# nnnagle/vq-vae

Measured on AMD Instinct MI355X. Metric: tiles/sec, higher is better.
Workload: dtype bf16

## Files before the change

### include/frl_hip.h

```cpp
#ifndef FRL_HIP_H
#define FRL_HIP_H

#include <stddef.h>
#include <stdint.h>

#ifdef __cplusplus
extern "C" {
#endif

typedef void* frl_stream_t;

enum { FRL_F32 = 0, FRL_BF16 = 1, FRL_F16 = 2  };
enum { FRL_ACT_NONE = 0, FRL_ACT_RELU = 1, FRL_ACT_SIGMOID = 2 };

int frl_version(void);
const char* frl_last_error(void);
int frl_device_arch(char* buf, int n);
int frl_kernel_timing_enable(int on);
int frl_kernel_timing_report(char* buf, int n);

size_t frl_pack_cache_table_bytes(void);
int frl_pack_cache_create(void* arena, size_t bytes);
int frl_pack_cache_destroy(int handle);
int frl_pack_cache_activate(int handle);
// ... 132 lines not shown
int frl_tcn_hot_fwd(const void* x, const void* drop_mask, const float* conv_w, const float* conv_b, const float* gn_w, const float* gn_b,
                    const float* gate_w, const float* gate_b, void* y, int64_t npix, int HW, int dilation, float eps, void* ws,
                    size_t ws_bytes, frl_stream_t stream);
int frl_tcn_hot_bwd_nodx_supported(int64_t npix, int HW);
int frl_tcn_hot_bwd(const void* x, const void* drop_mask, const void* dy, const float* conv_w, const float* conv_b, const float* gn_w,
                    const float* gn_b, const float* gate_w, const float* gate_b, void* dx, float* d_conv_w, float* d_conv_b,
                    float* d_gn_w, float* d_gn_b, float* d_gate_w, float* d_gate_b, int64_t npix, int HW, int dilation,
                    float eps, void* ws, size_t ws_bytes, frl_stream_t stream);
size_t frl_tcn_chain_fwd_workspace_bytes(void);
int frl_tcn_chain_static_tiles(int on);
int frl_tcn_chain_fwd(const void* x, const float* const* conv_w, const float* const* conv_b, const float* const* gn_w,
                      const float* const* gn_b, const float* const* gate_w, const float* const* gate_b, const float* head_w,
                      const float* head_b, void* y1, void* y2, void* y3, void* h, int64_t npix, int HW, int Ch, float eps, void* ws,
                      size_t ws_bytes, frl_stream_t stream);
int frl_tcn_chain_fwd_xt(const void* x, const float* const* conv_w, const float* const* conv_b, const float* const* gn_w,
                         const float* const* gn_b, const float* const* gate_w, const float* const* gate_b, const float* head_w,
                         const float* head_b, void* y1, void* y2, void* y3, void* h, void* xt, int64_t npix, int HW, int Ch, float eps,
                         void* ws, size_t ws_bytes, frl_stream_t stream);
int frl_tcn_hot_bwd_head_supported(int64_t npix, int HW, int Ch);
size_t frl_tcn_hot_bwd_head_workspace_bytes(int64_t npix);
int frl_tcn_hot_bwd_head(const void* x, const void* dh, const float* head_w, int Ch, const float* conv_w, const float* conv_b,
                         const float* gn_w, const float* gn_b, const float* gate_w, const float* gate_b, void* dx, float* d_conv_w,
                         float* d_conv_b, float* d_gn_w, float* d_gn_b, float* d_gate_w, float* d_gate_b, int64_t npix, int HW,
                         int dilation, float eps, void* ws, size_t ws_bytes, frl_stream_t stream);
int frl_tcn_hot_force_generic_tiles(int on);
int frl_tcn_hot_bwd4_share(int variant, int share);

size_t frl_adamw_workspace_bytes(void);
int frl_adamw_clip_step(const void* desc_host, int ntensors, const void* chunks, const int* chunk_tensor, int nchunks, float max_norm,
                        float lr, double beta1, double beta2, float eps, int step, float* norm_out, const float* ok, int* counters,
                        const float* lr_dev, int* tensor_steps, int nsteps, void* ws, size_t ws_bytes, frl_stream_t stream);
int frl_multi_tensor_scale_copy(const void* desc_host, int ntensors, const void* chunks, const int* chunk_tensor, int nchunks, float scale,
                                frl_stream_t stream);

int frl_film_modulate_fwd(const void* h, const void* gamma, const void* beta, void* out, int64_t B, int T, int64_t HW,
                          int C, int dtype, frl_stream_t stream);
int frl_film_modulate_bwd(const void* dout, const void* h, const void* gamma, void* dh, void* dgamma, void* dbeta,
                          int64_t B, int T, int64_t HW, int C, int dtype, frl_stream_t stream);
int frl_mean_time_fwd(const void* tile, void* out, int64_t B, int T, int64_t HWC, int dtype, frl_stream_t stream);
int frl_add(const void* a, const void* b, float scale_b, void* out, int64_t n, int dtype, frl_stream_t stream);

typedef struct FrlNormRec {
  float sub, div, mul, add, lo, hi;
  int flags;
  int pad;
} FrlNormRec;
int frl_normalize_tiles(const void* raw, int raw_dtype, const uint8_t* valid, const void* table, void* out, int out_dtype,
                        uint8_t* mask_out, int64_t rows, int F, frl_stream_t stream);
int frl_normalize_chunk_tiles(const void* chunk, int raw_dtype, int T, int CY, int CX, int F, const int32_t* desc, int ntiles,
                              int tile, const void* table, void* out, int out_dtype, uint8_t* mask_out, frl_stream_t stream);

int frl_host_parallel_copy(void* dst, const void* src, size_t nbytes, int nthreads);

size_t frl_mse_workspace_bytes(void);
int frl_mse_fwd(const void* pred, const void* target, const uint8_t* mask, int64_t P, int C, float* out, int dtype,
                void* ws, size_t ws_bytes, frl_stream_t stream);
int frl_mse_bwd(const void* pred, const void* target, const uint8_t* mask, const float* gscale, const float* stats,
                int64_t P, int C, void* dpred, int dtype, frl_stream_t stream);

int frl_decoder_mse_fused_supported(int Cz, int hidden, int F, int dtype);
size_t frl_decoder_mse_workspace_bytes(int64_t P, int Cz);
int frl_decoder_mse_fwd(const void* z, const float* w1, const float* b1, const float* w2, const float* b2, const void* target,
                        const uint8_t* mask, void* xhat, float* out, int64_t P, int Cz, void* ws, size_t ws_bytes,
                        frl_stream_t stream);
int frl_decoder_mse_bwd(const void* z, const float* w1, const float* b1, const float* w2, const float* b2, const void* target,
                        const uint8_t* mask, const float* gscale, const float* stats, void* dz, float* dw1, float* db1,
                        float* dw2, float* db2, int64_t P, int Cz, void* ws, size_t ws_bytes, frl_stream_t stream);
size_t frl_decoder_mse_onepass_bytes(int64_t P, int Cz);
int frl_decoder_mse_fwd_bwd(const void* z, const float* w1, const float* b1, const float* w2, const float* b2, const void* target,
                            const uint8_t* mask, const float* gscale, float* out, void* dz, void* buf, size_t buf_bytes, void* ctl,
                            int* nslab, int64_t P, int Cz, frl_stream_t stream);
int frl_decoder_mse_reduce(const void* buf, int nslab, float* dw1, float* db1, float* dw2, float* db2, int Cz, frl_stream_t stream);
int frl_decoder_mse_bwd_subgroups(int on);

size_t frl_vq_workspace_bytes(int64_t N, int K, int d);
int frl_vq_assign_fwd(const void* z, const float* E, int64_t N, int K, int d, int32_t* idx_out, void* zq_out,
                      float* stats_out, int32_t* counts_out, int dtype, void* ws, size_t ws_bytes, frl_stream_t stream);
size_t frl_vq_prepared_bytes(int K, int d);
int frl_vq_stream_tiles(int nt);
int frl_vq_prepare(const float* E, int64_t N, int K, int d, int dtype, void* prep, size_t prep_bytes, frl_stream_t stream);
int frl_vq_assign_fwd_prepared(const void* z, const float* E, void* prep , int64_t N, int K, int d,
                               int32_t* idx_out, void* zq_out, float* stats_out, int32_t* counts_out, int dtype, void* ws,
                               size_t ws_bytes, frl_stream_t stream);
int frl_vq_bwd(const void* g_out, const void* z, const void* zq , const float* E, const int32_t* idx, const int32_t* counts,
               const float* gscale, float beta, int64_t N, int K, int d, void* g_z_out, float* g_E_out, float* sums_out,
               int dtype, void* ws, size_t ws_bytes, frl_stream_t stream);
int frl_vq_ema_update(const float* sums, const int32_t* counts, int K, int d, float decay, float eps, float* ema_count,
                      float* ema_sum, float* E, const float* ok, frl_stream_t stream);
int frl_vq_revive_dead_codes(float* E, const int64_t* window_counts, int64_t min_count, const void* z, int64_t N, int K, int d,
                             uint64_t seed, float* m, float* v, int32_t* revived, int dtype, frl_stream_t stream);

int frl_gather_locations_fwd(const void* feat, int64_t sC, int64_t sH, int64_t sW, int C, int H, int W, const int64_t* coords, int64_t N,
                             void* out, int dtype, frl_stream_t stream);
int frl_segment_sum_rows(const float* vals, const int64_t* order, const int64_t* keys_sorted, int64_t M, int D, float* out, int64_t out_stride,
                         int accumulate, frl_stream_t stream);
int frl_infonce_fwd(const float* emb, int D, const int64_t* pairs, const float* weights, const unsigned char* is_pos, int64_t T,
                    const int64_t* seg, int64_t nseg, float temperature, int similarity, float* sims, float* logits, float* loss_a, float* coef,
                    float* loss, frl_stream_t stream);
int frl_infonce_pair_grads(const float* emb, int D, const int64_t* pairs, const float* sims, const float* coef, const float* gscale, int64_t T,
                           int64_t nseg, float temperature, int similarity, float* ga, float* gb, frl_stream_t stream);

size_t frl_vicreg_workspace_bytes(int64_t N, int D);
int frl_vicreg_fwd(const void* x, int64_t N, int D, int dtype, float variance_weight, float covariance_weight, float variance_target,
                   float eps, float* losses, float* cov, float* centre, void* ws, size_t ws_bytes, frl_stream_t stream);
int frl_vicreg_bwd(const void* x, const float* cov, const float* centre, const float* g3, int64_t N, int D, int dtype, float variance_weight,
                   float covariance_weight, float variance_target, float eps, void* dx, frl_stream_t stream);

int frl_soft_nbr_fwd(const float* d_ref, const float* d_learned, const unsigned char* mask, const float* weights, int64_t B, int M,
                     float inv_tau_ref, float inv_tau_learned, int min_valid, float* pairstat, float* coef, float* out2, double* stats,
                     frl_stream_t stream);
int frl_soft_nbr_bwd(const float* coef, const float* pairstat, const float* weights, const float* out2, const float* gup, int64_t B, int M,
                     float* grad, frl_stream_t stream);
int frl_soft_nbr_gathered_fwd(const float* ref, int C, const void* emb, int D, int emb_dtype, const int64_t* ref_rows_a, const int64_t* ref_rows_b,
                              const int64_t* emb_rows_a, const int64_t* emb_rows_b, const int64_t* lengths, const float* weights, int64_t B, int M,
                              int exclude_diagonal, float inv_tau_ref, float inv_tau_learned, int min_valid, float* pairstat, float* out2,
                              double* stats, frl_stream_t stream);
int frl_soft_nbr_gathered_bwd(const float* ref, int C, const void* emb, int D, int emb_dtype, const int64_t* ref_rows_a, const int64_t* ref_rows_b,
                              const int64_t* emb_rows_a, const int64_t* emb_rows_b, const int64_t* lengths, const float* weights, int64_t B, int M,
                              int exclude_diagonal, float inv_tau_ref, float inv_tau_learned, int min_valid, const float* pairstat,
                              const float* out2, const float* gup, float* grad_rows, frl_stream_t stream);

int frl_evt_soft_nbr_fwd(const void* emb, int emb_dtype, int64_t N, int D, const int32_t* idx, const float* S, const float* w, int K,
                         const int32_t* seg, const int32_t* seg_host, int nseg, float inv_tau_ref, float inv_tau_learned, int min_valid_anchors,
                         float* rowstat, float* segout, double* segstat, int32_t* index_flag, frl_stream_t stream);
int frl_evt_soft_nbr_bwd(const void* emb, int emb_dtype, int64_t N, int D, const int32_t* idx, const float* S, const float* w, int K,
                         const int32_t* seg, const int32_t* seg_host, int nseg, float inv_tau_ref, float inv_tau_learned, const float* rowstat,
                         const float* segout, const float* gup, const float* seg_weights, void* grad, frl_stream_t stream);

int frl_recovery_disc_fwd(const void* z, int dtype, const float* ysfc, int64_t N, int T, int D, float margin, float low_ysfc_max,
                          float high_ysfc_min, float* partial, float* out2, double* stats, frl_stream_t stream);
int frl_recovery_disc_bwd(const void* z, int dtype, const float* ysfc, int64_t N, int T, int D, float margin, float low_ysfc_max,
                          float high_ysfc_min, const float* out2, const float* gup, void* grad, frl_stream_t stream);
int frl_spread_rank_fwd(const float* d_i, const float* d_j, const unsigned char* mask, const float* ref_diff, int64_t B, int M, float margin,
                        float delta, float* pairstat, float* out2, double* stats, frl_stream_t stream);
int frl_spread_rank_bwd(const unsigned char* mask, const float* pairstat, const float* ref_diff, const float* gup, int64_t B, int M,
                        float margin, float delta, float* grad_i, float* grad_j, frl_stream_t stream);
int frl_spread_rank_gathered_fwd(const void* emb, int D, int emb_dtype, const int64_t* rows_i, const int64_t* rows_j, const int64_t* lengths,
                                 const float* ref_diff, int64_t B, int M, float margin, float delta, float* pairstat, float* out2,
                                 double* stats, frl_stream_t stream);
int frl_spread_rank_gathered_bwd(const void* emb, int D, int emb_dtype, const int64_t* rows_i, const int64_t* rows_j, const int64_t* lengths,
                                 const float* ref_diff, int64_t B, int M, float margin, float delta, const float* pairstat, const float* gup,
                                 float* grad_rows, frl_stream_t stream);

int frl_decode_codes(const int32_t* idx, const void* table, void* out, int64_t P, int K, int F, int dtype, int32_t* index_flag,
                     frl_stream_t stream);

size_t frl_mutual_knn_max_points(int D);
int frl_mutual_knn(const float* feat, int N, int D, const int32_t* patch_id, const float* coords, float pos_min_spatial, int k,
                   int32_t* knn_idx, uint8_t* mutual, frl_stream_t stream);

size_t frl_phase_pairs_max_points(int D);
int frl_phase_pairs(const float* spec, const float* ysfc, int N, int D, int T, const int32_t* seg_host, const int32_t* seg, int S, int k,
                    int min_overlap, int min_pairs, float sigma, uint64_t* masks, int32_t* knn_idx, int32_t* overlap, uint8_t* keep,
                    uint8_t* keep_overlap, float* weight, float* dist, uint8_t* anchor_ok, int32_t* counters, int32_t* flag,
                    frl_stream_t stream);

int frl_spatial_pairs_max_hw(void);
int frl_spatial_pack_mask(const uint8_t* mask, int S, int H, int W, uint32_t* bits, frl_stream_t stream);
int frl_spatial_knn(const uint32_t* bits, int S, int H, int W, const int32_t* anchors, int N, const int32_t* seg_host, const int32_t* seg,
                    const int32_t* offsets, int k, int32_t* pos_rc, uint8_t* pos_valid, int32_t* counters, int32_t* flag, frl_stream_t stream);
int frl_spatial_negatives(const uint32_t* bits, int S, int H, int W, const int32_t* anchors, int N, const int32_t* seg_host, const int32_t* seg,
                          int lo, int hi, int n_per_anchor, const int32_t* draws, int32_t* neg_rc, int32_t* neg_count, int32_t* counters,
                          int32_t* flag, frl_stream_t stream);
int frl_spatial_pair_index(int S, int H, int W, const int32_t* anchors, int N, const int32_t* seg_host, const int32_t* seg, const int32_t* pos_rc,
                           const uint8_t* pos_valid, int k, const int32_t* neg_rc, const int32_t* neg_count, int n_per_anchor, const float* feat,
                           int C, float tau, float min_w, uint32_t* bitmap, int32_t* wordpre, int32_t* unique_seg, int32_t* unique_rc,
                           int32_t* anchor_idx, int32_t* pos_idx, int32_t* neg_idx, float* pos_w, float* pos_d, float* neg_w, float* neg_d,
                           frl_stream_t stream);

// ... 68 lines not shown
```

### vq-vae_amd/csrc/frl_epi.hpp

```cpp
#pragma once
#include <stdint.h>
#include <hip/hip_runtime.h>

struct ThEpi {
  float *dWc, *dWg, *dbc, *dbg, *dgam, *dbet;
  __device__ void operator()(int64_t i, float s) const {
    if (i < 3 * 4096) {
      const int k = (int)(i / 4096), co = (int)((i % 4096) / 64), ci = (int)(i % 64);
      dWc[(co * 64 + ci) * 3 + k] = s;
    } else if (i < 4 * 4096) {
      dWg[i - 3 * 4096] = s;
    } else {
      const int j = (int)(i - 4 * 4096);
      if (j < 64) dbc[j] = s; else if (j < 128) dbg[j - 64] = s; else if (j < 192) dgam[j - 128] = s; else dbet[j - 192] = s;
    }
  }
};

struct C3Epi {
  int OCT, Cin9, oc_base, Cout; float* dW; float* dB;
  __device__ void operator()(int64_t i, float s) const {
    if (i < (int64_t)OCT * Cin9) {
      const int Cin = Cin9 / 9;
      const int tap = (int)(i / ((int64_t)OCT * Cin)), rem = (int)(i % ((int64_t)OCT * Cin));
      const int ocl = rem / Cin, ic = rem % Cin;
      if (oc_base + ocl < Cout) dW[(int64_t)(oc_base + ocl) * Cin9 + ic * 9 + tap] = s;
    } else if (dB != nullptr) {
      const int ocl = (int)(i - (int64_t)OCT * Cin9);
      if (oc_base + ocl < Cout) dB[oc_base + ocl] = s;
    }
  }
};

struct DecEpi {
  float *dW2, *dW1, *db2, *db1; int Cz, CZP, F, Hd;
  __device__ void operator()(int64_t i, float s) const {
    if (i < F * Hd) { dW2[i] = s; return; }
    i -= F * Hd;
    if (i < Hd * CZP) { const int hh = (int)(i / CZP), c = (int)(i % CZP); if (c < Cz) dW1[hh * Cz + c] = s; return; }
    i -= Hd * CZP;
    if (i < F) db2[i] = s; else db1[i - F] = s;
  }
};

struct EncEpi {
  float *dw2, *dw1, *db2, *dg2, *db1, *dg1;
  __device__ void operator()(int64_t i, float s) const {
    if (i < 64 * 128) { dw2[i] = s; return; }
    i -= 64 * 128;
    if (i < 128 * 64) { dw1[i] = s; return; }
    i -= 128 * 64;
    if (i < 64) db2[i] = s;
    else if (i < 128) dg2[i - 64] = s;
    else if (i < 256) db1[i - 128] = s;
    else dg1[i - 256] = s;
  }
};

struct FilmEpi {
  float *dw1g, *dw1b, *dw2g, *dw2b, *db1g, *db1b, *db2g, *db2b;
  __device__ void operator()(int64_t i, float s) const {
    if (i < 2048) { dw1g[i] = s; return; }
    if (i < 4096) { dw1b[i - 2048] = s; return; }
    if (i < 4480) { dw2g[i - 4096] = s; return; }
    if (i < 4864) { dw2b[i - 4480] = s; return; }
    if (i < 4896) { db1g[i - 4864] = s; return; }
    if (i < 4928) { db1b[i - 4896] = s; return; }
    if (i < 4940) { db2g[i - 4928] = s; return; }
    db2b[i - 4940] = s;
  }
};

struct ShEpi {
  float *dwb, *dwa, *dbb, *dba; int NB, NA, HID;
  __device__ void operator()(int64_t i, float s) const {
    if (i < NB * HID) { dwb[i] = s; return; }
    i -= NB * HID;
    if (i < NA * HID) { dwa[i] = s; return; }
    i -= NA * HID;
    if (i < NB) dbb[i] = s; else dba[i - NB] = s;
  }
};

struct WgradEpi {
  float* dW; int64_t dso, dsi; float* dB; int Cout, Cin, accumulate_bias;
  __device__ void operator()(int64_t i, float s) const {
    if (i < (int64_t)Cout * Cin) {
      const int oc = (int)(i / Cin), ic = (int)(i % Cin);
      dW[oc * dso + ic * dsi] = s;
    } else if (dB != nullptr) {
      const int oc = (int)(i - (int64_t)Cout * Cin);
      if (accumulate_bias) dB[oc] += s; else dB[oc] = s;
    }
  }
};

struct CodeEpi {
  const float* E; const int32_t* counts; const float* gscale; float ce_base; int d, bf; float* gE; float* sums_out;
  __device__ void operator()(int64_t i, float s) const {
    if (sums_out) sums_out[i] = s;
    if (gE) {
      const float ce = ce_base * (gscale ? gscale[1] : 1.f);
      const float ev = bf ? (float)(__bf16)E[i] : E[i];
      gE[i] = ce * ((float)counts[i / d] * ev - s);
    }
  }
};

struct CopyEpi {
  float* dst;
  __device__ void operator()(int64_t i, float s) const { dst[i] = s; }
};

template <class Epi> struct FrlEpiKind { static constexpr int id = 0; };
template <> struct FrlEpiKind<ThEpi> { static constexpr int id = 1; };
template <> struct FrlEpiKind<C3Epi> { static constexpr int id = 2; };
template <> struct FrlEpiKind<DecEpi> { static constexpr int id = 3; };
template <> struct FrlEpiKind<EncEpi> { static constexpr int id = 4; };
template <> struct FrlEpiKind<FilmEpi> { static constexpr int id = 5; };
template <> struct FrlEpiKind<ShEpi> { static constexpr int id = 6; };
template <> struct FrlEpiKind<WgradEpi> { static constexpr int id = 7; };
template <> struct FrlEpiKind<CodeEpi> { static constexpr int id = 8; };
```

### vq-vae_amd/csrc/frl_pack.hpp

```cpp
#pragma once
#include <hip/hip_runtime.h>
#include <stdint.h>
#include <stddef.h>

enum { FRL_PACK_PW = 0, FRL_PACK_C3 = 1, FRL_PACK_PW_REP = 2, FRL_PACK_PW_K4 = 3 };

struct FrlPackJob {
  const float* W;
  char* dst;
  long long so, si;
  int kind, dtype, NF;
  int Cout, Cin, MB;
  int tap_rev, nfrag;
};

static inline FrlPackJob frl_pack_job_pw(const float* W, size_t dst_off, int dtype, int NF, int Cout, int Cin, int MB, long long so, long long si) {
  FrlPackJob j;
  j.W = W; j.dst = (char*)dst_off; j.so = so; j.si = si; j.kind = FRL_PACK_PW; j.dtype = dtype; j.NF = NF;
  j.Cout = Cout; j.Cin = Cin; j.MB = MB; j.tap_rev = 0; j.nfrag = MB * NF * 64;
  return j;
}
static inline FrlPackJob frl_pack_job_c3(const float* W, size_t dst_off, int dtype, int NF, int Cout, int Cin, long long so, long long si, int tap_rev,
                                         int nfrag) {
  FrlPackJob j;
  j.W = W; j.dst = (char*)dst_off; j.so = so; j.si = si; j.kind = FRL_PACK_C3; j.dtype = dtype; j.NF = NF;
  j.Cout = Cout; j.Cin = Cin; j.MB = (Cout + 15) >> 4; j.tap_rev = tap_rev; j.nfrag = nfrag;
  return j;
}

void* frl_pack_cached(const FrlPackJob* jobs, int njobs, size_t bytes, bool* hit);
```

### vq-vae_amd/csrc/pack_cache.hip

```cpp
#include "frl_common.hpp"
#include "frl_host.hpp"
#include "frl_pack.hpp"
#include <map>
#include <mutex>
#include <string.h>
#include <vector>

#define PK_FRAGS_PER_BLOCK 512

__device__ __forceinline__ void pk_frag_pw(const FrlPackJob& j, int i) {
  const int lane = i & 63, fs = i >> 6;
  const int s = fs % j.NF, mb = fs / j.NF;
  const int r = lane & 15, kc = lane >> 4;
  const int qo = 4 * j.MB;
  const int oc = j.kind == FRL_PACK_PW_REP ? 4 * mb + (r & 3) : qo * (r >> 2) + 4 * mb + (r & 3);
  if (j.dtype == FRL_BF16) {
    const int q = j.NF * 8;
    bf16x8 v;
#pragma unroll
    for (int e = 0; e < 8; ++e) {
      const int ic = j.kind == FRL_PACK_PW_K4 ? (e < 4 ? 4 * kc + e : j.Cin) : q * kc + 8 * s + e;
      v[e] = (oc < j.Cout && ic < j.Cin) ? (bf16)j.W[oc * j.so + ic * j.si] : (bf16)0.f;
    }
    reinterpret_cast<bf16x8*>(j.dst)[i] = v;
  } else {
    const int q = j.NF;
    const int ic = q * kc + s;
    reinterpret_cast<float*>(j.dst)[i] = (oc < j.Cout && ic < j.Cin) ? j.W[oc * j.so + ic * j.si] : 0.f;
  }
}

__device__ __forceinline__ void pk_frag_c3(const FrlPackJob& j, int g) {
  const int FE = j.dtype == FRL_BF16 ? 8 : 1;
  const int q = j.NF * FE, CK = 4 * q;
  const int MB = (j.Cout + 15) >> 4, qo = 4 * MB;
  const int nck = (j.Cin + CK - 1) / CK;
  const int per_block = 9 * 4 * j.NF * 64;
  const int blk = g / per_block, i = g % per_block;
  const int oc0 = (blk / nck) * 4, ck = (blk % nck) * CK;
  const int ln = i & 63, fs = i >> 6;
  const int s = fs % j.NF, m = (fs / j.NF) & 3, tap = fs / (j.NF * 4);
  const int r = ln & 15, kq = ln >> 4;
  const int oc = qo * (r >> 2) + 4 * (oc0 + m) + (r & 3);
  const int tsrc = j.tap_rev ? 8 - tap : tap;
  const bool mok = (oc0 + m) < MB;
  if (j.dtype == FRL_BF16) {
    bf16x8 v;
#pragma unroll
    for (int e = 0; e < 8; ++e) {
      const int ic = ck + q * kq + 8 * s + e;
      v[e] = (mok && oc < j.Cout && ic < j.Cin) ? (bf16)j.W[oc * j.so + ic * j.si + tsrc] : (bf16)0.f;
    }
    reinterpret_cast<bf16x8*>(j.dst)[g] = v;
  } else {
    const int ic = ck + q * kq + s;
    reinterpret_cast<float*>(j.dst)[g] = (mok && oc < j.Cout && ic < j.Cin) ? j.W[oc * j.so + ic * j.si + tsrc] : 0.f;
  }
}

__global__ __launch_bounds__(256) void frl_pack_jobs_kernel(const FrlPackJob* __restrict__ jobs, const int2* __restrict__ blocks) {
  const int2 bk = blocks[blockIdx.x];
  const FrlPackJob j = jobs[bk.x];
  const int end = (bk.y + PK_FRAGS_PER_BLOCK) < j.nfrag ? (bk.y + PK_FRAGS_PER_BLOCK) : j.nfrag;
  for (int i = bk.y + threadIdx.x; i < end; i += 256) {
    if (j.kind == FRL_PACK_C3) pk_frag_c3(j, i); else pk_frag_pw(j, i);
  }
}

namespace {
struct Key {
  unsigned char bytes[8 * 72];
  size_t n;
  bool operator<(const Key& o) const { return n != o.n ? n < o.n : memcmp(bytes, o.bytes, n) < 0; }
};
struct Cache {
  char* arena = nullptr;
  size_t bytes = 0, used = 0, table_bytes = 0;
  std::map<Key, char*> images;
  std::vector<FrlPackJob> jobs;
  std::vector<int2> blocks;
  bool dirty = false;
};
std::mutex g_mu;
std::map<int, Cache> g_caches;
int g_next = 1;
int g_active = 0;
constexpr size_t PK_MAX_JOBS = 2048, PK_MAX_BLOCKS = 16384;
}

void* frl_pack_cached(const FrlPackJob* jobs, int njobs, size_t bytes, bool* hit) {
  *hit = false;
  if (g_active == 0 || njobs <= 0 || njobs > 8) return nullptr;
  std::lock_guard<std::mutex> lk(g_mu);
  auto it = g_caches.find(g_active);
  if (it == g_caches.end()) return nullptr;
  Cache& c = it->second;
  Key k;
  memset(&k, 0, sizeof(k));
  k.n = (size_t)njobs * sizeof(FrlPackJob);
  memcpy(k.bytes, jobs, k.n);
  auto im = c.images.find(k);
  if (im != c.images.end()) { *hit = true; return im->second; }
  const size_t need = (bytes + 255) / 256 * 256;
  int nblk = 0;
  for (int i = 0; i < njobs; ++i) nblk += (jobs[i].nfrag + PK_FRAGS_PER_BLOCK - 1) / PK_FRAGS_PER_BLOCK;
  if (c.used + need > c.bytes || c.jobs.size() + njobs > PK_MAX_JOBS || c.blocks.size() + nblk > PK_MAX_BLOCKS) return nullptr;
  char* img = c.arena + c.used;
  c.used += need;
  for (int i = 0; i < njobs; ++i) {
    FrlPackJob j = jobs[i];
    j.dst = img + (size_t)j.dst;
    const int ji = (int)c.jobs.size();
    c.jobs.push_back(j);
    for (int f = 0; f < j.nfrag; f += PK_FRAGS_PER_BLOCK) c.blocks.push_back(int2{ji, f});
  }
  c.images[k] = img;
  c.dirty = true;
  return img;
}

extern "C" {

size_t frl_pack_cache_table_bytes(void) { return PK_MAX_JOBS * sizeof(FrlPackJob) + PK_MAX_BLOCKS * sizeof(int2); }

int frl_pack_cache_create(void* arena, size_t bytes) {
  const size_t tb = (frl_pack_cache_table_bytes() + 255) / 256 * 256;
  if (arena == nullptr || bytes <= tb + 4096) return frl_fail(-4, "pack_cache_create: arena too small");
  std::lock_guard<std::mutex> lk(g_mu);
  Cache c;
  c.arena = (char*)arena;
  c.bytes = bytes;
  c.table_bytes = tb;
  c.used = tb;
  const int h = g_next++;
  g_caches[h] = c;
  return h;
}

int frl_pack_cache_destroy(int handle) {
  std::lock_guard<std::mutex> lk(g_mu);
  if (g_active == handle) g_active = 0;
  g_caches.erase(handle);
  return 0;
}

int frl_pack_cache_activate(int handle) {
  std::lock_guard<std::mutex> lk(g_mu);
  const int was = g_active;
  g_active = (handle != 0 && g_caches.count(handle)) ? handle : 0;
  return was;
}

int frl_pack_cache_images(int handle) {
  std::lock_guard<std::mutex> lk(g_mu);
  auto it = g_caches.find(handle);
  return it == g_caches.end() ? -1 : (int)it->second.images.size();
}

int frl_pack_cache_refresh(int handle, hipStream_t stream) {
  std::lock_guard<std::mutex> lk(g_mu);
  auto it = g_caches.find(handle);
  if (it == g_caches.end()) return frl_fail(-2, "pack_cache_refresh: unknown handle");
  Cache& c = it->second;
  if (c.jobs.empty()) return 0;
  FrlPackJob* jd = (FrlPackJob*)c.arena;
  int2* bd = (int2*)(c.arena + PK_MAX_JOBS * sizeof(FrlPackJob));
  if (c.dirty) {
    hipStreamCaptureStatus cs = hipStreamCaptureStatusNone;
    (void)hipStreamIsCapturing(stream, &cs);
    if (cs != hipStreamCaptureStatusNone) return frl_fail(-5, "pack_cache_refresh: images were registered during a stream capture (run the step eagerly first)");
    FRL_HIP(hipMemcpyAsync(jd, c.jobs.data(), c.jobs.size() * sizeof(FrlPackJob), hipMemcpyHostToDevice, stream));
    FRL_HIP(hipMemcpyAsync(bd, c.blocks.data(), c.blocks.size() * sizeof(int2), hipMemcpyHostToDevice, stream));
    FRL_HIP(hipStreamSynchronize(stream));
    c.dirty = false;
  }
  FRL_LAUNCH(frl_pack_jobs_kernel, dim3((unsigned)c.blocks.size()), dim3(256), 0, stream, (const FrlPackJob*)jd, (const int2*)bd);
  return frl_check_launch("pack_cache_refresh");
}

}
```

### vq-vae_amd/csrc/vq.hip

```cpp
#include "frl_common.hpp"
#include "frl_host.hpp"
#include "vq_common.hpp"
#include "vq_prepare.hpp"
#include "vq_assign_chunked.hpp"
#include "vq_assign_resident.hpp"
#include "vq_assign_stream.hpp"
#include "vq_bwd.hpp"
#include <stdlib.h>

static int vq_chunk(int K, int d_pad, size_t esize) {
  const size_t cap = 64 * 1024;
  int kc = VQ_MAX_CHUNK;
  while (kc > 16 && (size_t)kc * d_pad * esize > cap) kc >>= 1;
  const int kpad = (K + 15) / 16 * 16;
  if (kc > kpad) kc = kpad;
  return kc;
}
static int vq_waves(int64_t N, int d) { return (d <= 64 && N >= (int64_t)256 * 8 * 2 * 16) ? 8 : 4; }
static int vq_grid(int64_t N, int d) {
  const int nw = vq_waves(N, d), NT = nw == 8 ? 2 : 4;
  const int64_t nb = (N + nw * NT * 16 - 1) / (nw * NT * 16);
  const int cap = 512;
  return (int)(nb < cap ? (nb < 1 ? 1 : nb) : cap);
}
#define VQ_FIX_WAVES 1024
#define VQ_BWD_WGS 256

struct VqPrep { size_t ctl, en, pack, total; int Kc, kpad, npk; };
template <typename T, int NF>
static VqPrep vq_prep_layout(int64_t N, int K, int d) {
  VqPrep P;
  const int d_pad = NF * DT<T>::FE * 4;
  P.Kc = vq_chunk(K, d_pad, sizeof(T));
  P.kpad = (K + P.Kc - 1) / P.Kc * P.Kc;
  P.npk = (P.kpad / 16) * NF * 64;
  P.ctl = 0;
  P.en = (sizeof(VqCtl) + (size_t)K * 4 + 255) / 256 * 256;
  P.pack = P.en + ((size_t)P.kpad * 4 + 255) / 256 * 256;
  P.total = P.pack + (size_t)P.npk * sizeof(typename DT<T>::frag_t);
  return P;
}
static size_t vq_prep_bytes_max(int K) {
  return (sizeof(VqCtl) + (size_t)K * 4 + 255) / 256 * 256 + ((size_t)(K + VQ_MAX_CHUNK) * 4 + 255) / 256 * 256 +
         (size_t)((K + 15) / 16 + 64) * 16 * 128 * 4;
}

struct VqLayout { size_t hdr, counts_fix, partial, amb, amb_lim, prep, total; int grid; };
static VqLayout vq_layout(int64_t N, int K, int d) {
  VqLayout L;
  L.grid = vq_grid(N, d);
  size_t o = 0;
  L.hdr = o; o += 256;
  L.counts_fix = o; o += ((size_t)K * 4 + 255) / 256 * 256;
  L.partial = o; o += ((size_t)L.grid * 16 * 4 + 255) / 256 * 256;
  L.amb = o; o += ((size_t)N * 4 + 255) / 256 * 256;
  L.amb_lim = o; o += ((size_t)N * 4 + 255) / 256 * 256;
  L.prep = o; o += vq_prep_bytes_max(K);
  L.total = o;
  return L;
}

template <typename T, int NF>
static int launch_vq_prepare(const float* E, int64_t N, int K, int d, char* prep, hipStream_t st) {
  typedef typename DT<T>::frag_t frag_t;
  const VqPrep P = vq_prep_layout<T, NF>(N, K, d);
  const int npack_blocks = (P.npk + 255) / 256;
  const int kz = P.kpad > 64 ? P.kpad : 64;
  FRL_LAUNCH((vq_prepare_kernel<T, NF>), dim3(npack_blocks + (kz + 255) / 256), dim3(256), 0, st, E, K, d, (float*)(prep + P.en), P.kpad,
             (frag_t*)(prep + P.pack), P.npk, npack_blocks, (int*)(prep + P.ctl));
  return frl_check_launch("vq_prepare");
}

static int g_vq_stream_tiles = -1;
static int vq_stream_tiles();
#ifndef VQ_STREAM_DEFAULT
#define VQ_STREAM_DEFAULT 2
#endif
static int vq_stream_tiles() {
  if (g_vq_stream_tiles >= 0) return g_vq_stream_tiles;
  static const int env = [] { const char* e = getenv("FRL_VQ_STREAM"); return e ? atoi(e) : VQ_STREAM_DEFAULT; }();
  return env;
}
#ifndef VQ_RES_NT
#define VQ_RES_NT 4
#endif
template <typename... P, typename... A>
static int vq_launch_assign(void (*kern)(P...), int grid, int threads, size_t lds, hipStream_t st, A... args) {
  if (lds > 64 * 1024) FRL_HIP(hipFuncSetAttribute((const void*)kern, hipFuncAttributeMaxDynamicSharedMemorySize, (int)lds));
  FRL_LAUNCH_AS("vq_assign_kernel", kern, dim3(grid), dim3(threads), lds, st, args...);
  return 0;
}
template <typename T, int NF>
static int launch_vq(const void* z, const float* E, char* prep, int64_t N, int K, int d, int32_t* idx, void* zq, float* stats,
                     int32_t* counts, char* ws, hipStream_t st) {
  typedef typename DT<T>::frag_t frag_t;
  const VqLayout L = vq_layout(N, K, d);
  const VqPrep P = vq_prep_layout<T, NF>(N, K, d);
  const int nw = vq_waves(N, d);
  const int Kc = P.Kc;
  VqHeader* hdr = (VqHeader*)(ws + L.hdr);
  const bool resident = P.kpad == Kc;
  if (!resident) FRL_HIP(hipMemsetAsync(ws, 0, L.partial, st));
  if (prep == nullptr) {
    const int rc = launch_vq_prepare<T, NF>(E, N, K, d, ws + L.prep, st);
    if (rc) return rc;
    prep = ws + L.prep;
  }
  const float* en = (const float*)(prep + P.en);
  const frag_t* pk = (const frag_t*)(prep + P.pack);
  if constexpr (sizeof(T) == 2 && NF == 2) {
    const int stream_nt = vq_stream_tiles();
    int nt = stream_nt >= 4 ? 4 : (stream_nt >= 2 ? 2 : 1);
    while (nt > 1 && N % (VQS_NW * nt * 16) != 0) nt >>= 1;
    const int batch = VQS_NW * nt * 16;
    if (resident && stream_nt > 0 && d == 64 && (Kc & 15) == 0 && N % batch == 0 && N < ((int64_t)1 << 32)) {
      const int64_t nb = (N + batch - 1) / batch;
      const int grid_s = (int)(nb < 256 ? nb : 256);
      const size_t lds = (size_t)(Kc / 16) * NF * 64 * sizeof(frag_t) + (size_t)Kc * 4 + (size_t)((K + 3) & ~3) * 4 + 64 * 4 +
                         (size_t)VQ_FAST_ROWS * 16 + (size_t)VQS_NW * VQS_CAP * 8 + (size_t)VQS_CAND * 4 +
                         (size_t)VQS_NW * (VQS_CAP + 16) * VQS_ZP * sizeof(T);
      if (lds > 160 * 1024) return frl_fail(-3, "vq_assign: LDS budget exceeded");
      const auto kern = nt == 4 ? vq_assign_stream_kernel<4> : nt == 2 ? vq_assign_stream_kernel<2> : vq_assign_stream_kernel<1>;
      const int rc = vq_launch_assign(kern, grid_s, 64 * VQS_NW, lds, st, (const bf16*)z, en, N, K, Kc, idx, (bf16*)zq, (float*)(ws + L.partial),
                                      (const bf16x8*)pk, (VqCtl*)(prep + P.ctl), counts, stats, (unsigned*)(ws + L.amb), (float*)(ws + L.amb_lim));
      return rc ? rc : frl_check_launch("vq_assign");
    }
  }
  if (resident) {
    const int nwr = (nw == 8 && NF <= (sizeof(T) == 2 ? 2 : 4)) ? 8 : 4;
    const int batch = nwr * VQ_RES_NT * 16;
    const int64_t nb = (N + batch - 1) / batch;
    const int grid_r = (int)(nb < L.grid ? nb : L.grid);
    size_t lds = (size_t)(Kc / 16) * NF * 64 * sizeof(frag_t) + (size_t)Kc * 4 + (size_t)((K + 1) & ~1) * 4 + (size_t)VQ_FAST_ROWS * 12 +
                 (size_t)2 * batch * 4 + (size_t)nwr * 64 * 4 + 32 * 4 + (size_t)VQ_PZ_CAP * d * sizeof(T);
    const size_t fold = (size_t)2 * nwr * 64 * sizeof(double);
    if (lds < fold) lds = fold;
    if (lds > 160 * 1024) return frl_fail(-3, "vq_assign: LDS budget exceeded");
    auto kern = vq_assign_resident_kernel<T, NF, VQ_RES_NT, 4>;
    if constexpr (NF <= (sizeof(T) == 2 ? 2 : 4)) {
      if (nwr == 8) kern = vq_assign_resident_kernel<T, NF, VQ_RES_NT, 8>;
    }
    const int rc = vq_launch_assign(kern, grid_r, 64 * nwr, lds, st, (const T*)z, E, en, N, K, d, Kc, idx, (T*)zq, (float*)(ws + L.partial), pk,
                                    (VqCtl*)(prep + P.ctl), counts, stats);
    return rc ? rc : frl_check_launch("vq_assign");
  }
  const int Kc2 = Kc >= 32 ? Kc / 2 : Kc;
  const size_t lds = 2 * ((size_t)(Kc2 / 16) * NF * 64 * sizeof(frag_t) + (size_t)Kc2 * 4) + 64 + (K <= 2048 ? (size_t)K * 4 : 0);
  if (((Kc2 / 16) * NF * 64 * sizeof(frag_t)) % 1024 != 0 || (Kc2 & 63) != 0) return frl_fail(-3, "vq_assign: chunk is not a whole number of DMA pieces");
  const auto kern = nw == 8 ? vq_assign_kernel<T, NF, 2, 8> : vq_assign_kernel<T, NF, 4, 4>;
  const int rc = vq_launch_assign(kern, L.grid, 64 * nw, lds, st, (const T*)z, E, en, N, K, d, Kc2, idx, (T*)zq, (float*)(ws + L.partial),
                                  (int32_t*)(ws + L.counts_fix), hdr, (int32_t*)(ws + L.amb), (float*)(ws + L.amb_lim), pk);
  if (rc) return rc;
  FRL_LAUNCH_AS("vq_fixup_tile_kernel", (vq_fixup_tile_kernel<T, NF>), dim3(1024), dim3(64 * VQ_FIXT_WAVES), 0, st, (const T*)z, E, en, pk, K, P.kpad, d,
                (const int32_t*)(ws + L.amb), (const float*)(ws + L.amb_lim), hdr, idx, (T*)zq, (int32_t*)(ws + L.counts_fix));
  FRL_LAUNCH(vq_finalize_kernel, dim3(1), dim3(256), 0, st, (const float*)(ws + L.partial), L.grid * nw, (const VqHeader*)hdr,
             (const int32_t*)(ws + L.counts_fix), counts, K, N, d, stats);
  return frl_check_launch("vq_assign");
}

static int vq_bwd_chunk(int K, int d) {
  int kc = K;
  while ((size_t)kc * d * 4 > 96 * 1024 && kc > 1) kc = (kc + 1) / 2;
  return kc;
}

extern "C" {

int frl_vq_stream_tiles(int nt) {
  const int prev = g_vq_stream_tiles;
  g_vq_stream_tiles = nt < 0 ? -1 : nt;
  return prev;
}

size_t frl_vq_workspace_bytes(int64_t N, int K, int d) {
  const VqLayout L = vq_layout(N, K, d);
  const size_t bwd = (size_t)VQ_BWD_WGS * K * d * 4 + (size_t)K * d * 4;
  return L.total > bwd ? L.total : bwd;
}

#define VQ_DISPATCH(dtype, d, CALL)                                              \
  do {                                                                          \
    if ((dtype) == FRL_F32) {                                                   \
      if ((d) <= 16) return CALL(float, 4);                                     \
      if ((d) <= 32) return CALL(float, 8);                                     \
      if ((d) <= 64) return CALL(float, 16);                                    \
      return CALL(float, 32);                                                   \
    } else if ((dtype) == FRL_BF16) {                                           \
      if ((d) <= 32) return CALL(bf16, 1);                                      \
      if ((d) <= 64) return CALL(bf16, 2);                                      \
      return CALL(bf16, 4);                                                     \
    }                                                                           \
    return frl_fail(-2, "vq: bad dtype");                                       \
  } while (0)

size_t frl_vq_prepared_bytes(int K, int d) { return (K > 0 && d > 0 && d <= 128) ? vq_prep_bytes_max(K) : 0; }

int frl_vq_prepare(const float* E, int64_t N, int K, int d, int dtype, void* prep, size_t prep_bytes, hipStream_t stream) {
  if (N <= 0 || K <= 0 || d <= 0) return frl_fail(-2, "vq_prepare: empty input");
  if (d > 128) return frl_fail(-2, "vq_prepare: d > 128 unsupported");
  if (prep == nullptr || prep_bytes < frl_vq_prepared_bytes(K, d)) return frl_fail(-4, "vq_prepare: buffer too small");
#define VQ_CALL_PREP(T_, NF_) launch_vq_prepare<T_, NF_>(E, N, K, d, (char*)prep, stream)
  VQ_DISPATCH(dtype, d, VQ_CALL_PREP);
#undef VQ_CALL_PREP
}

int frl_vq_assign_fwd_prepared(const void* z, const float* E, void* prep, int64_t N, int K, int d, int32_t* idx_out, void* zq_out,
                               float* stats_out, int32_t* counts_out, int dtype, void* ws, size_t ws_bytes, hipStream_t stream) {
  if (N <= 0 || K <= 0 || d <= 0) return frl_fail(-2, "vq_assign: empty input");
  if (d > 128) return frl_fail(-2, "vq_assign: d > 128 unsupported");
  if (ws_bytes < frl_vq_workspace_bytes(N, K, d)) return frl_fail(-4, "vq_assign: workspace too small");
#define VQ_CALL_FWD(T_, NF_) launch_vq<T_, NF_>(z, E, (char*)prep, N, K, d, idx_out, zq_out, stats_out, counts_out, (char*)ws, stream)
  VQ_DISPATCH(dtype, d, VQ_CALL_FWD);
#undef VQ_CALL_FWD
}

int frl_vq_assign_fwd(const void* z, const float* E, int64_t N, int K, int d, int32_t* idx_out, void* zq_out,
                      float* stats_out, int32_t* counts_out, int dtype, void* ws, size_t ws_bytes, hipStream_t stream) {
  return frl_vq_assign_fwd_prepared(z, E, nullptr, N, K, d, idx_out, zq_out, stats_out, counts_out, dtype, ws, ws_bytes, stream);
}

int frl_vq_bwd(const void* g_out, const void* z, const void* zq, const float* E, const int32_t* idx, const int32_t* counts,
               const float* gscale, float beta, int64_t N, int K, int d, void* g_z_out, float* g_E_out,
               float* sums_out, int dtype, void* ws, size_t ws_bytes, hipStream_t stream) {
  if (N <= 0 || K <= 0 || d <= 0) return frl_fail(-2, "vq_bwd: empty input");
  if (dtype != FRL_F32 && dtype != FRL_BF16) return frl_fail(-2, "vq_bwd: bad dtype");
  if (dtype == FRL_BF16 && d > 128) return frl_fail(-2, "vq_bwd: d > 128 unsupported in bf16");
  if (ws_bytes < frl_vq_workspace_bytes(N, K, d)) return frl_fail(-4, "vq_bwd: workspace too small");
  const int Kc = vq_bwd_chunk(K, d);
  const size_t lds = (size_t)Kc * d * 4;
  if (dtype == FRL_F32 && lds > 96 * 1024) return frl_fail(-2, "vq_bwd: one code row exceeds the LDS chunk");
  const int64_t rows = (N + VQ_BWD_WGS - 1) / VQ_BWD_WGS;
  const float cz = beta * 2.f / ((float)N * (float)d), ce = 2.f / ((float)N * (float)d);
  float* slab = (float*)ws;
  if (dtype == FRL_F32) {
    auto kern = vq_bwd_kernel<float>;
    if (lds > 64 * 1024) FRL_HIP(hipFuncSetAttribute((const void*)kern, hipFuncAttributeMaxDynamicSharedMemorySize, (int)lds));
    FRL_LAUNCH_AS("vq_bwd_kernel", kern, dim3(VQ_BWD_WGS), dim3(256), lds, stream, (const float*)g_out, (const float*)z, E, idx, gscale,
                       cz, N, K, d, Kc, rows, (float*)g_z_out, slab);
    launch_slab_reduce_deferrable<float, CodeEpi>((const float*)slab, VQ_BWD_WGS, (int64_t)K * d, CodeEpi{E, counts, gscale, ce, d, 0, g_E_out, sums_out}, stream, sums_out == nullptr);
  } else if (dtype == FRL_BF16) {
    const int64_t rows64 = (rows + 63) / 64 * 64;
    if (d <= 32) {
      FRL_LAUNCH((vq_bwd_mfma_kernel<4, 2, 8>), dim3(VQ_BWD_WGS), dim3(512), (size_t)64 * 40 * 2 + 256, stream, (const bf16*)g_out, (const bf16*)z, (const bf16*)zq, E, idx,
                 gscale, cz, N, K, d, rows64, (bf16*)g_z_out, slab);
    } else if (d <= 64) {
      FRL_LAUNCH((vq_bwd_mfma_kernel<4, 4, 8>), dim3(VQ_BWD_WGS), dim3(512), (size_t)64 * 72 * 2 + 256, stream, (const bf16*)g_out, (const bf16*)z, (const bf16*)zq, E, idx,
                 gscale, cz, N, K, d, rows64, (bf16*)g_z_out, slab);
    } else {
      FRL_LAUNCH((vq_bwd_mfma_kernel<2, 8, 8>), dim3(VQ_BWD_WGS), dim3(512), (size_t)64 * 136 * 2 + 256, stream, (const bf16*)g_out, (const bf16*)z, (const bf16*)zq, E, idx,
                 gscale, cz, N, K, d, rows64, (bf16*)g_z_out, slab);
    }
    launch_slab_reduce_deferrable<float, CodeEpi>((const float*)slab, VQ_BWD_WGS, (int64_t)K * d, CodeEpi{E, counts, gscale, ce, d, 1, g_E_out, sums_out}, stream, sums_out == nullptr);
  } else return frl_fail(-2, "vq_bwd: bad dtype");
  return frl_check_launch("vq_bwd");
}

int frl_vq_ema_update(const float* sums, const int32_t* counts, int K, int d, float decay, float eps, float* ema_count,
                      float* ema_sum, float* E, const float* ok, hipStream_t stream) {
  FRL_LAUNCH(vq_ema_kernel, dim3(1), dim3(256), 0, stream, sums, counts, K, d, decay, eps, ema_count, ema_sum, E, ok);
  return frl_check_launch("vq_ema_update");
}

int frl_vq_revive_dead_codes(float* E, const int64_t* window_counts, int64_t min_count, const void* z, int64_t N, int K, int d,
                             uint64_t seed, float* m, float* v, int32_t* revived, int dtype, hipStream_t stream) {
  if (K <= 0 || d <= 0) return frl_fail(-2, "vq_revive_dead_codes: bad codebook shape");
  if (N <= 0) return frl_fail(-2, "vq_revive_dead_codes: no candidate rows");
  if (dtype == FRL_F32)
    FRL_LAUNCH((vq_revive_kernel<float>), dim3(K), dim3(64), 0, stream, E, (const long long*)window_counts, (long long)min_count,
               (const float*)z, (long long)N, K, d, (unsigned long long)seed, m, v, revived);
  else if (dtype == FRL_BF16)
    FRL_LAUNCH((vq_revive_kernel<bf16>), dim3(K), dim3(64), 0, stream, E, (const long long*)window_counts, (long long)min_count,
               (const bf16*)z, (long long)N, K, d, (unsigned long long)seed, m, v, revived);
  else return frl_fail(-2, "vq_revive_dead_codes: dtype must be FRL_F32 or FRL_BF16");
  return frl_check_launch("vq_revive_dead_codes");
}

}
```

### vq-vae_amd/csrc/vq_assign_chunked.hpp

```cpp
#pragma once
#include "vq_common.hpp"

template <typename T, int NF, int NT, int NW>
__global__ __launch_bounds__(NW * 64, (NW == 8 ? 4 : 2)) void vq_assign_kernel(
    const T* __restrict__ Z, const float* __restrict__ E, const float* __restrict__ en_g, int64_t N, int K, int d, int Kc,
    int32_t* __restrict__ idx_out, T* __restrict__ zq_out, float* __restrict__ partial , int32_t* __restrict__ counts_acc,
    VqHeader* __restrict__ hdr_w, int32_t* __restrict__ amb_list, float* __restrict__ amb_lim, const typename DT<T>::frag_t* __restrict__ pk) {
  typedef typename DT<T>::frag_t frag_t;
  constexpr int FE = DT<T>::FE;
  constexpr int q = NF * FE;
  extern __shared__ __attribute__((aligned(16))) char smem[];
  const int chunk_bytes = (Kc / 16) * NF * 64 * (int)sizeof(frag_t);
  const int buf_bytes = chunk_bytes + Kc * 4;
  float* cbw = reinterpret_cast<float*>(smem + 2 * buf_bytes);
  int* hist = reinterpret_cast<int*>(smem + 2 * buf_bytes + 64);
  const bool lds_hist = K <= 2048;
  const int tid = threadIdx.x, lane = tid & 63;
  const int wave = __builtin_amdgcn_readfirstlane(tid >> 6);
  const int vx = lane & 15, kc = lane >> 4;
  const int nchunks = (K + Kc - 1) / Kc;
  const bool fast = (d == 4 * q);
  float enmax;
  {
    float m = 0.f;
// ... 150 lines not shown
          } else {
#pragma unroll
            for (int s = 0; s < NF * FE; ++s) {
              if (q * kc + s < d) {
                const float ev = to_f32(from_f32<T>(er[s]));
                zo[s] = from_f32<T>(ev);
                const float df = lq_get<T, NF>(zt[t], s / FE, s % FE) - ev;
                sq_acc = fmaf(df, df, sq_acc);
              }
            }
          }
          if (kc == 0) atomicAdd(lds_hist ? &hist[code] : &counts_acc[code], 1);
        }
      }
    }
  }
  const float ws_ = wave_sum(sq_acc);
  if (lane == 0) partial[blockIdx.x * NW + wave] = ws_;
  if (lds_hist) {
    __syncthreads();
    vq_flush_hist<NW>(hist, counts_acc, K, tid);
  }
}

#define VQ_FIXT_WAVES 8
template <typename T, int NF>
__global__ __launch_bounds__(64 * VQ_FIXT_WAVES) void vq_fixup_tile_kernel(const T* __restrict__ Z, const float* __restrict__ E, const float* __restrict__ en_g,
                                                            const typename DT<T>::frag_t* __restrict__ pk, int K, int kpad, int d,
                                                            const int32_t* __restrict__ amb_list, const float* __restrict__ amb_lim,
                                                            VqHeader* __restrict__ hdr, int32_t* __restrict__ idx_out, T* __restrict__ zq_out,
                                                            int32_t* __restrict__ counts_fix) {
  constexpr int FE = DT<T>::FE;
  constexpr int q = NF * FE;
  __shared__ double mrg_d[VQ_FIXT_WAVES][16];
  __shared__ int mrg_k[VQ_FIXT_WAVES][16];
  __shared__ unsigned long long bins[VQ_SQ_BINS];
  __shared__ float row_sq[16];
  if (threadIdx.x < VQ_SQ_BINS) bins[threadIdx.x] = 0ull;
  const int lane = threadIdx.x & 63, wave = threadIdx.x >> 6;
  const int vx = lane & 15, kc = lane >> 4;
  const bool fast = (d == 4 * q);
  const int namb = hdr->namb;
  const int ntile = (namb + 15) >> 4, nmb = kpad >> 4;
  const int mb0 = (wave * nmb) / VQ_FIXT_WAVES, mb1 = ((wave + 1) * nmb) / VQ_FIXT_WAVES;
  for (int tile = blockIdx.x; tile < ntile; tile += gridDim.x) {
    const int li = tile * 16 + vx;
    const bool valid = li < namb;
    const int64_t row = amb_list[valid ? li : tile * 16];
    const float lm = amb_lim[valid ? li : tile * 16];
    LQTile<T, NF> zr;
    lq_load<T, NF>(zr, Z, row, d, kc, fast);
    const VqBest own = vq_resolve_inlane<T, NF>(zr, pk, en_g, mb0, mb1, K, lane, valid, lm, [&](int p0, int p1, double& d0, double& d1) {
      vq_exact_pair<T, 1>(Z, E, row, p0, p1, d, d0, d1);
    });
    double bestd = own.d;
    int bk = own.k;
    if (kc == 0) { mrg_d[wave][vx] = bestd; mrg_k[wave][vx] = bk; }
    __syncthreads();
    if (wave == 0) {
      bestd = mrg_d[0][vx]; bk = mrg_k[0][vx];
#pragma unroll
      for (int w = 1; w < VQ_FIXT_WAVES; ++w) {
        const double ob = mrg_d[w][vx];
        const int okk = mrg_k[w][vx];
        if (ob < bestd || (ob == bestd && okk < bk)) { bestd = ob; bk = okk; }
      }
      if ((unsigned)bk >= (unsigned)K) bk = 0;
      float rs = 0.f;
      if (valid) vq_write_row<T, NF>(zr, E, zq_out, row, bk, d, kc, rs);
      rs += __shfl_xor(rs, 16, 64);
      rs += __shfl_xor(rs, 32, 64);
      if (valid && kc == 0) { idx_out[row] = bk; atomicAdd(&counts_fix[bk], 1); }
      if (kc == 0) row_sq[vx] = valid ? rs : -1.f;
    }
    __syncthreads();
    if (wave == 1 && lane < 16 && !(row_sq[lane] == -1.f)) vq_sq_bins_add(bins, &hdr->sq_fix, row_sq[lane]);
  }
  __syncthreads();
  if (threadIdx.x < VQ_SQ_BINS && bins[threadIdx.x] != 0ull) atomicAdd(&hdr->sq_bins[threadIdx.x], bins[threadIdx.x]);
}

__global__ __launch_bounds__(256) void vq_finalize_kernel(const float* __restrict__ partial, int npartial, const VqHeader* __restrict__ hdr,
                                                          const int32_t* __restrict__ counts_acc, int32_t* __restrict__ counts, int K, int64_t N,
                                                          int d, float* __restrict__ stats) {
  __shared__ double red[256];
  double s = 0.0;
  for (int i = threadIdx.x; i < npartial; i += 256) s += (double)partial[i];
  red[threadIdx.x] = s;
  __syncthreads();
  for (int o = 128; o > 0; o >>= 1) { if (threadIdx.x < o) red[threadIdx.x] += red[threadIdx.x + o]; __syncthreads(); }
  const double sq = red[0] + (vq_sq_bins_value(hdr->sq_bins) + hdr->sq_fix);
  __syncthreads();
  double h = 0.0;
  for (int k = threadIdx.x; k < K; k += 256) {
    const int cnt = counts_acc[k];
    counts[k] = cnt;
    const double p = (double)cnt / (double)N;
    h += p * log(p + 1e-10);
  }
  red[threadIdx.x] = h;
  __syncthreads();
  for (int o = 128; o > 0; o >>= 1) { if (threadIdx.x < o) red[threadIdx.x] += red[threadIdx.x + o]; __syncthreads(); }
  if (threadIdx.x == 0) {
    stats[0] = (float)sq;
    stats[1] = (float)exp(-red[0]);
    stats[2] = (float)hdr->namb;
    stats[3] = (float)(sq / ((double)N * (double)d));
  }
}
```

### vq-vae_amd/csrc/vq_assign_resident.hpp

```cpp
#pragma once
#include "vq_common.hpp"

#define VQ_PZ_CAP 16

template <typename T, int NF, int NT, int NW>
__global__ __launch_bounds__(NW * 64, (NW == 8 ? 4 : 1)) void vq_assign_resident_kernel(
    const T* __restrict__ Z, const float* __restrict__ E, const float* __restrict__ en_g, int64_t N, int K, int d, int Kc,
    int32_t* __restrict__ idx_out, T* __restrict__ zq_out, float* __restrict__ partial ,
    const typename DT<T>::frag_t* __restrict__ pk, VqCtl* __restrict__ ctl, int32_t* __restrict__ counts_out, float* __restrict__ stats_out) {
  typedef typename DT<T>::frag_t frag_t;
  constexpr int FE = DT<T>::FE;
  constexpr int q = NF * FE;
  constexpr int BATCH = NW * NT * 16;
  constexpr int CAND_CAP = NW * 64;
  extern __shared__ __attribute__((aligned(16))) char smem[];
  frag_t* wl = reinterpret_cast<frag_t*>(smem);
  float* enl = reinterpret_cast<float*>(smem + (size_t)(Kc / 16) * NF * 64 * sizeof(frag_t));
  int* hist = reinterpret_cast<int*>(enl + Kc);
  unsigned long long* best = reinterpret_cast<unsigned long long*>(hist + ((K + 1) & ~1));
  int* bestk = reinterpret_cast<int*>(best + VQ_FAST_ROWS);
  int* park = bestk + VQ_FAST_ROWS;
  int* cand = park + 2 * BATCH;
  int* misc = cand + CAND_CAP;
  T* park_z = reinterpret_cast<T*>(misc + 32);
  int32_t* counts_acc = reinterpret_cast<int32_t*>(ctl + 1);
  const int tid = threadIdx.x, lane = tid & 63, wave = tid >> 6;
  const int vx = lane & 15, kc = lane >> 4;
  const bool fast = (d == 4 * q);
  const int nmb = Kc / 16;
#ifdef VQ_STAMPS
  __shared__ unsigned long long vq_ts[16][8];
  if (tid < 128) (&vq_ts[0][0])[tid] = 0ull;
  unsigned long long t_prev = __builtin_amdgcn_s_memtime();
  const unsigned long long t_begin = t_prev;
  const unsigned long long w_begin = wall_clock64();
#endif

  const int64_t nbatch = (N + BATCH - 1) / BATCH;
  LQTile<T, NF> zt[NT];
  auto load_batch = [&](int64_t b, int tid_) {
    const int64_t r0 = b * BATCH + (int64_t)(tid_ >> 6) * (NT * 16);
#pragma unroll
    for (int t = 0; t < NT; ++t) {
      int64_t row = r0 + t * 16 + (tid_ & 15);
      if (row >= N) row = N - 1;
      lq_load<T, NF>(zt[t], Z, row, d, (tid_ >> 4) & 3, fast);
    }
  };
  if ((int64_t)blockIdx.x < nbatch) load_batch(blockIdx.x, tid);
  copy_frags_lds<T>(wl, pk, nmb * NF * 64, tid, NW * 64);
  float enmax;
  {
    float m = 0.f;
    for (int i = tid; i < Kc; i += NW * 64) {
      const float v = i < K ? en_g[i] : 3.0e38f;
      enl[i] = v;
      if (i < K) m = fmaxf(m, v);
    }
#pragma unroll
    for (int off = 1; off < 64; off <<= 1) m = fmaxf(m, __shfl_xor(m, off, 64));
    if (lane == 0) misc[18 + wave] = __float_as_int(m);
  }
  for (int k = tid; k < K; k += NW * 64) hist[k] = 0;
  if (tid < VQ_FAST_ROWS) { best[tid] = ~0ull; bestk[tid] = 0x7fffffff; }
  if (tid == 0) misc[16] = 0;
  __syncthreads();
  {
    float m = 0.f;
#pragma unroll
    for (int w = 0; w < NW; ++w) m = fmaxf(m, __int_as_float(misc[18 + w]));
    enmax = m;
  }
  const float err_rel = (float)(4 * q + 8) * 1.1920929e-7f;
  const float thr_rel = (3.0517578125e-5f + 2.f * err_rel) * 1.001953125f;
  const float enroot = sqrtf(enmax);
  float sq_acc = 0.f;
  int n_resolved = 0;
  VQ_ST(2);

  for (int64_t batch = blockIdx.x; batch < nbatch; batch += gridDim.x) {
    const int64_t base = batch * BATCH;
    const int64_t v0 = base + (int64_t)wave * (NT * 16);
    if (batch != (int64_t)blockIdx.x) {
      int tidl = tid;
      asm volatile("" : "+v"(tidl));
      load_batch(batch, tidl);
    }
    float thr[NT];
    unsigned g1[NT], g2[NT];
    int gc[NT];
#pragma unroll
    for (int t = 0; t < NT; ++t) {
// ... 202 lines not shown
        }
        VQ_LDS_BARRIER();
        if (c < ncand && bits == best[li]) __hip_atomic_fetch_min(&bestk[li], code, __ATOMIC_RELAXED, __HIP_MEMORY_SCOPE_WORKGROUP);
        VQ_LDS_BARRIER();
        const int j = tidr & 15;
        for (int li2 = tidr >> 4; li2 < n; li2 += NW * 4) {
          int bk = bestk[li2];
          if ((unsigned)bk >= (unsigned)K) bk = 0;
          const int64_t row = base + park[2 * li2];
          for (int ch = j; ch < d; ch += 16) {
            float ev, zv;
            bool done_ = false;
            if constexpr (FE == 8) {
              if (zlds) {
                ev = -0.5f * (float)reinterpret_cast<const bf16x8*>(wl)[((bk >> 4) * NF + ((ch % q) >> 3)) * 64 + (bk & 15) + 16 * (ch / q)][ch & 7];
                zv = (float)reinterpret_cast<const bf16*>(park_z)[li2 * d + ch];
                done_ = true;
              }
            }
            if (!done_) {
              ev = to_f32(from_f32<T>(E[(int64_t)bk * d + ch]));
              zv = to_f32(Z[row * (int64_t)d + ch]);
            }
            zq_out[row * (int64_t)d + ch] = from_f32<T>(ev);
            const float df = zv - ev;
            sq_acc = fmaf(df, df, sq_acc);
          }
          if (j == 0) { idx_out[row] = bk; atomicAdd(&hist[bk], 1); }
        }
        VQ_LDS_BARRIER();
        if (tidr < VQ_FAST_ROWS && tidr < n) {
          int m1 = -1;
          asm volatile("" : "+v"(m1));
          best[tidr] = ((unsigned long long)(unsigned)m1 << 32) | (unsigned)m1;
          bestk[tidr] = 0x7fffffff;
        }
      }
    }
    if (!all_waves) {
      for (int t0 = wave * 16; t0 < n; t0 += NW * 16) {
        const int li = t0 + vx;
        const bool valid = li < n;
        const int64_t row = base + park[2 * (valid ? li : t0)];
        const float lm = __int_as_float(park[2 * (valid ? li : t0) + 1]);
        LQTile<T, NF> zr;
        lq_load<T, NF>(zr, Z, row, d, kc, fast);
        int bk = vq_resolve_inlane<T, NF>(zr, wl, enl, 0, nmb, K, lane, valid, lm, [&](int p0, int p1, double& d0, double& d1) {
          vq_exact_pair<T, 1>(Z, E, row, p0, p1, d, d0, d1);
        }).k;
        if ((unsigned)bk >= (unsigned)K) bk = 0;
        if (valid) {
          vq_write_row<T, NF>(zr, E, zq_out, row, bk, d, kc, sq_acc);
          if (kc == 0) { idx_out[row] = bk; atomicAdd(&hist[bk], 1); }
        }
      }
    }
    n_resolved += n;
    VQ_LDS_BARRIER();
    if (tid == 0) misc[16] = 0;
    VQ_ST(5);
  }
  int tidt = tid;
  asm volatile("" : "+v"(tidt));
  const float ws_ = wave_sum(sq_acc);
  if ((tidt & 63) == 0) partial[blockIdx.x * NW + (tidt >> 6)] = ws_;
  __syncthreads();
  vq_flush_hist<NW>(hist, counts_acc, K, tidt);
  if (tidt == 0 && n_resolved) atomicAdd(&ctl->namb, n_resolved);
  asm volatile("s_waitcnt vmcnt(0)" ::: "memory");
  __syncthreads();
  if (tidt == 0) {
    __builtin_amdgcn_fence(__ATOMIC_RELEASE, "agent");
    asm volatile("s_waitcnt vmcnt(0)" ::: "memory");
    const int ticket = __hip_atomic_fetch_add(&ctl->done, 1, __ATOMIC_RELAXED, __HIP_MEMORY_SCOPE_AGENT);
    misc[17] = (ticket == (int)gridDim.x - 1) ? 1 : 0;
    if (ticket == (int)gridDim.x - 1) {
      __builtin_amdgcn_fence(__ATOMIC_ACQUIRE, "agent");
      asm volatile("s_waitcnt vmcnt(0)" ::: "memory");
    }
  }
  __syncthreads();
  const bool last = misc[17] != 0;
  __syncthreads();
  if (last) vq_fold_stats<NW>(reinterpret_cast<double*>(smem), tidt, tidt & 63, tidt >> 6, partial, (int)gridDim.x * NW, ctl, K, N, d, counts_out, stats_out);
#ifdef VQ_STAMPS
  VQ_ST(6);
  __syncthreads();
  if (tid < 128) vq_dbg[(size_t)blockIdx.x * 128 + tid] = (&vq_ts[0][0])[tid];
  if (tid == 0) { vq_dbg[(size_t)gridDim.x * 128 + 2 * blockIdx.x] = __builtin_amdgcn_s_memtime() - t_begin; vq_dbg[(size_t)gridDim.x * 128 + 2 * blockIdx.x + 1] = wall_clock64() - w_begin; }
#endif
}
```

### vq-vae_amd/csrc/vq_assign_stream.hpp

```cpp
#pragma once
#include "vq_common.hpp"

#define VQS_NW 16
#define VQS_ZP 72
#define VQS_GRP 16

template <int NT, bool FULL>
__device__ __forceinline__ void vqs_score_group(const bf16x8* __restrict__ wl, const float* __restrict__ enl, int lane, int kc, int mb0, int cnt,
                                                const LQTile<bf16, 2> (&z)[NT], unsigned (&c1)[NT], unsigned (&c2)[NT]) {
  const unsigned maskv = ~VQ_IDX_MASK;
  const bf16x8* __restrict__ wb = wl + mb0 * 2 * 64 + lane;
  const float* __restrict__ eb = enl + mb0 * 16 + 4 * kc;
  auto block = [&](int mb, int j) {
    (void)mb;
    const f32x4 en4 = *reinterpret_cast<const f32x4*>(eb + j * 16);
    const bf16x8 a0 = wb[j * 2 * 64], a1 = wb[j * 2 * 64 + 64];
#pragma unroll
    for (int t = 0; t < NT; ++t) {
      f32x4 acc = mfma16(a0, z[t].f[0], en4);
      acc = mfma16(a1, z[t].f[1], acc);
#pragma unroll
      for (int r = 0; r < 4; r += 2) {
        const unsigned k0 = (__float_as_uint(acc[r]) & maskv) | (unsigned)(4 * j + r);
        const unsigned k1 = (__float_as_uint(acc[r + 1]) & maskv) | (unsigned)(4 * j + r + 1);
        unsigned m;
        asm("v_med3_f32 %0, %1, %2, %3" : "=v"(m) : "v"(c1[t]), "v"(k0), "v"(k1));
        asm("v_min_f32 %0, %1, %2" : "=v"(c2[t]) : "v"(c2[t]), "v"(m));
        asm("v_min3_f32 %0, %1, %2, %3" : "=v"(c1[t]) : "v"(c1[t]), "v"(k0), "v"(k1));
      }
    }
  };
  if constexpr (FULL) {
#pragma unroll
    for (int j = 0; j < VQS_GRP; ++j) block(mb0 + j, j);
  } else {
    for (int j = 0; j < cnt; ++j) block(mb0 + j, j);
  }
}

__device__ __forceinline__ void vqs_load_row(LQTile<bf16, 2>& t, const bf16* p) {
  asm volatile("global_load_dwordx4 %0, %1, off" : "=v"(t.f[0]) : "v"(p) : "memory");
  asm volatile("global_load_dwordx4 %0, %1, off offset:16" : "=v"(t.f[1]) : "v"(p) : "memory");
}
template <int NT, int CNT>
__device__ __forceinline__ void vqs_wait(LQTile<bf16, 2> (&b)[NT]) {
  asm volatile("s_waitcnt vmcnt(%2)" : "+v"(b[0].f[0]), "+v"(b[0].f[1]) : "n"(CNT) : "memory");
#pragma unroll
  for (int t = 1; t < NT; ++t) asm volatile("" : "+v"(b[t].f[0]), "+v"(b[t].f[1]) : : "memory");
}

__device__ __forceinline__ int vqs_resolve_inlane(const LQTile<bf16, 2>& zt, const bf16* __restrict__ zrow, const bf16x8* __restrict__ wl,
                                                  const float* __restrict__ enl, int nmb, int K, int lane, int kc, bool mine, float lm) {
  double bestd = 1.0e300;
  int bk = 0x7fffffff, p0 = -1, p1 = -1;
  auto flush = [&]() {
    if (p0 >= 0) {
      const double d0 = vq_exact_lds<2>(zrow, wl, p0, 64);
      if (d0 < bestd || (d0 == bestd && p0 < bk)) { bestd = d0; bk = p0; }
      if (p1 >= 0) {
        const double d1 = vq_exact_lds<2>(zrow, wl, p1, 64);
        if (d1 < bestd || (d1 == bestd && p1 < bk)) { bestd = d1; bk = p1; }
      }
    }
    p0 = p1 = -1;
  };
  for (int mb = 0; mb < nmb; ++mb) {
    f32x4 acc = *reinterpret_cast<const f32x4*>(enl + mb * 16 + 4 * kc);
    acc = mfma16(wl[(mb * 2 + 0) * 64 + lane], zt.f[0], acc);
    acc = mfma16(wl[(mb * 2 + 1) * 64 + lane], zt.f[1], acc);
#pragma unroll
    for (int r = 0; r < 4; ++r) {
      const int cd = mb * 16 + 4 * kc + r;
      const bool hit = mine && acc[r] <= lm && cd < K;
      if (__builtin_amdgcn_ballot_w64(hit && p1 >= 0) != 0ull) flush();
      if (hit) { if (p0 < 0) p0 = cd; else p1 = cd; }
    }
  }
  flush();
#pragma unroll
  for (int off = 16; off <= 32; off <<= 1) {
    const double ob = __shfl_xor(bestd, off, 64);
    const int okk = __shfl_xor(bk, off, 64);
    if (ob < bestd || (ob == bestd && okk < bk)) { bestd = ob; bk = okk; }
  }
  if ((unsigned)bk >= (unsigned)K) bk = 0;
  return bk;
}

#define VQS_CAP 8
#define VQS_CAND (VQS_NW * 64)
#ifdef VQS_NT_STORES
#define VQS_STORE(p, v) __builtin_nontemporal_store((v), (p))
#else
#define VQS_STORE(p, v) (*(p) = (v))
#endif
template <int NT>
__global__ __launch_bounds__(VQS_NW * 64, 1) void vq_assign_stream_kernel(
    const bf16* __restrict__ Z, const float* __restrict__ en_g, int64_t N, int K, int Kc, int32_t* __restrict__ idx_out,
    bf16* __restrict__ zq_out, float* __restrict__ partial , const bf16x8* __restrict__ pk, VqCtl* __restrict__ ctl,
    int32_t* __restrict__ counts_out, float* __restrict__ stats_out, unsigned* __restrict__ ovf_row , float* __restrict__ ovf_lim ) {
  constexpr int NF = 2, q = 16, d = 64, NW = VQS_NW;
  constexpr int BATCH = NW * NT * 16;
  static_assert(NW * VQS_CAP <= VQ_FAST_ROWS, "parked rows of a workgroup");
  extern __shared__ __attribute__((aligned(16))) char smem[];
  bf16x8* wl = reinterpret_cast<bf16x8*>(smem);
  float* enl = reinterpret_cast<float*>(smem + (size_t)(Kc / 16) * NF * 64 * sizeof(bf16x8));
  int* hist = reinterpret_cast<int*>(enl + Kc);
  int* misc = hist + ((K + 3) & ~3);
  unsigned long long* best = reinterpret_cast<unsigned long long*>(misc + 64);
  int* bestk = reinterpret_cast<int*>(best + VQ_FAST_ROWS);
  int* plist = bestk + VQ_FAST_ROWS;
  unsigned* prow = reinterpret_cast<unsigned*>(plist + VQ_FAST_ROWS);
  float* plim = reinterpret_cast<float*>(prow + NW * VQS_CAP);
  int* cand = reinterpret_cast<int*>(plim + NW * VQS_CAP);
  bf16* zdef = reinterpret_cast<bf16*>(cand + VQS_CAND);
  bf16* zpark = zdef + NW * VQS_CAP * VQS_ZP;
  int32_t* counts_acc = reinterpret_cast<int32_t*>(ctl + 1);
  const int tid = threadIdx.x, lane = tid & 63, wave = tid >> 6;
  const int vx = lane & 15, kc = lane >> 4;
  const int nmb = Kc / 16;
  const int64_t nbatch = N / BATCH;
#ifdef VQ_STAMPS
  __shared__ unsigned long long vq_ts[16][8];
  if (tid < 128) (&vq_ts[0][0])[tid] = 0ull;
  unsigned long long t_prev = __builtin_amdgcn_s_memtime();
  const unsigned long long t_begin = t_prev;
  const unsigned long long w_begin = wall_clock64();
#endif
  LQTile<bf16, NF> bufA[NT], bufB[NT];
  auto load_batch = [&](LQTile<bf16, NF> (&dst)[NT], int64_t b, bool real = true) {
    const int64_t r0 = b * BATCH + (int64_t)wave * (NT * 16);
#pragma unroll
    for (int t = 0; t < NT; ++t) vqs_load_row(dst[t], Z + (r0 + (real ? t * 16 + vx : 0)) * d + q * kc);
  };
  load_batch(bufA, blockIdx.x);
  const float env = tid < K ? en_g[tid] : 3.0e38f;
  for (int i0 = 0; i0 < nmb * NF * 64; i0 += 4 * NW * 64) {
    bf16x8 tmp[4];
#pragma unroll
    for (int u = 0; u < 4; ++u) { const int i = i0 + u * NW * 64 + tid; if (i < nmb * NF * 64) tmp[u] = pk[i]; }
#pragma unroll
    for (int u = 0; u < 4; ++u) { const int i = i0 + u * NW * 64 + tid; if (i < nmb * NF * 64) wl[i] = tmp[u]; }
  }
  float enmax;
  {
    float m = 0.f;
    if (tid < Kc) {
      enl[tid] = env;
      if (tid < K) m = env;
    }
#pragma unroll
    for (int off = 1; off < 64; off <<= 1) m = fmaxf(m, __shfl_xor(m, off, 64));
    if (lane == 0) misc[18 + wave] = __float_as_int(m);
  }
  for (int k = tid; k < K; k += NW * 64) hist[k] = 0;
  if (tid < VQ_FAST_ROWS) { best[tid] = ~0ull; bestk[tid] = 0x7fffffff; }
  if (tid < 2) misc[tid] = 0;
  __syncthreads();
  {
    float m = 0.f;
#pragma unroll
    for (int w = 0; w < NW; ++w) m = fmaxf(m, __int_as_float(misc[18 + w]));
    enmax = m;
  }
  const VqThr th = vq_thresholds(q, enmax);
  float sq_acc = 0.f;
  int n_resolved = 0, cnt_w = 0, ovf_cnt = 0;
  auto ovf_slot = [&](int k) -> int64_t {
    return ((int64_t)blockIdx.x + (int64_t)(k / (NT * 16)) * gridDim.x) * BATCH + (int64_t)wave * (NT * 16) + (k % (NT * 16));
  };
  bf16* zp = zpark + wave * 16 * VQS_ZP;
  int nstep = 0;
  VQ_ST(2);

  auto step = [&](LQTile<bf16, NF> (&cur)[NT], LQTile<bf16, NF> (&nxt)[NT], int64_t batch) {
    const int64_t v0 = batch * BATCH + (int64_t)wave * (NT * 16);
    { if (nstep == 0) __builtin_amdgcn_s_setprio(3); else if (nstep == 1) __builtin_amdgcn_s_setprio(2); else if (nstep == 2) __builtin_amdgcn_s_setprio(1); else __builtin_amdgcn_s_setprio(0); }
    ++nstep;
    vqs_wait<NT, 3 * NT>(cur);
    VQ_ST(0);
    const bool has_next = batch + (int64_t)gridDim.x < nbatch;
    load_batch(nxt, has_next ? batch + gridDim.x : batch, has_next);
    float thr[NT];
// ... 157 lines not shown
      for (int t0 = wave * 16; t0 < npark; t0 += NW * 16) {
        const int li = t0 + vx;
        const bool valid = li < npark;
        const int e = plist[valid ? li : t0];
        LQTile<bf16, NF> zr;
        zr.f[0] = *reinterpret_cast<const bf16x8*>(zdef + e * VQS_ZP + q * kc);
        zr.f[1] = *reinterpret_cast<const bf16x8*>(zdef + e * VQS_ZP + q * kc + 8);
        const int bk = vqs_resolve_inlane(zr, zdef + e * VQS_ZP, wl, enl, nmb, K, lane, kc, valid, plim[e]);
        if (valid) {
          const int64_t row = (int64_t)prow[e];
          bf16* zo = zq_out + row * (int64_t)d + q * kc;
#pragma unroll
          for (int s = 0; s < NF; ++s) {
            const bf16x8 pv = wl[((bk >> 4) * NF + s) * 64 + (bk & 15) + 16 * kc];
            bf16x8 ev;
#pragma unroll
            for (int e2 = 0; e2 < 8; ++e2) {
              const float f = -0.5f * (float)pv[e2];
              ev[e2] = (bf16)f;
              const float df = (float)zr.f[s][e2] - f;
              sq_acc = fmaf(df, df, sq_acc);
            }
            *reinterpret_cast<bf16x8*>(zo + 8 * s) = ev;
          }
          if (kc == 0) { idx_out[row] = bk; atomicAdd(&hist[bk], 1); }
        }
      }
    }
  }
  for (int t0 = 0; t0 < ovf_cnt; t0 += 16) {
    const int kq = t0 + vx;
    const bool valid = kq < ovf_cnt;
    const int64_t sl_ = ovf_slot(valid ? kq : t0);
    const int64_t row = (int64_t)__hip_atomic_load(&ovf_row[sl_], __ATOMIC_RELAXED, __HIP_MEMORY_SCOPE_AGENT);
    const float lm = __hip_atomic_load(&ovf_lim[sl_], __ATOMIC_RELAXED, __HIP_MEMORY_SCOPE_AGENT);
    LQTile<bf16, NF> zr;
    zr.f[0] = *reinterpret_cast<const bf16x8*>(Z + row * d + q * kc);
    zr.f[1] = *reinterpret_cast<const bf16x8*>(Z + row * d + q * kc + 8);
    *reinterpret_cast<bf16x8*>(zp + vx * VQS_ZP + q * kc) = zr.f[0];
    *reinterpret_cast<bf16x8*>(zp + vx * VQS_ZP + q * kc + 8) = zr.f[1];
    asm volatile("s_waitcnt lgkmcnt(0)" ::: "memory");
    const int bk = vqs_resolve_inlane(zr, zp + vx * VQS_ZP, wl, enl, nmb, K, lane, kc, valid, lm);
    if (valid) {
      bf16* zo = zq_out + row * (int64_t)d + q * kc;
#pragma unroll
      for (int s = 0; s < NF; ++s) {
        const bf16x8 pv = wl[((bk >> 4) * NF + s) * 64 + (bk & 15) + 16 * kc];
        bf16x8 ev;
#pragma unroll
        for (int e2 = 0; e2 < 8; ++e2) {
          const float f = -0.5f * (float)pv[e2];
          ev[e2] = (bf16)f;
          const float df = (float)zr.f[s][e2] - f;
          sq_acc = fmaf(df, df, sq_acc);
        }
        *reinterpret_cast<bf16x8*>(zo + 8 * s) = ev;
      }
      if (kc == 0) { idx_out[row] = bk; atomicAdd(&hist[bk], 1); }
    }
    asm volatile("s_waitcnt lgkmcnt(0)" ::: "memory");
  }
  VQ_ST(5);
  const float ws_ = wave_sum(sq_acc);
  if (lane == 0) {
    __hip_atomic_store(&partial[blockIdx.x * NW + wave], ws_, __ATOMIC_RELAXED, __HIP_MEMORY_SCOPE_AGENT);
    if (n_resolved) atomicAdd(&misc[0], n_resolved);
  }
  __syncthreads();
  vq_flush_hist<NW>(hist, counts_acc, K, tid);
  if (tid == 0 && misc[0]) atomicAdd(&ctl->namb, misc[0]);
  asm volatile("s_waitcnt vmcnt(0)" ::: "memory");
  __syncthreads();
  if (tid == 0) {
    const int ticket = __hip_atomic_fetch_add(&ctl->done, 1, __ATOMIC_RELAXED, __HIP_MEMORY_SCOPE_AGENT);
    misc[17] = (ticket == (int)gridDim.x - 1) ? 1 : 0;
    if (ticket == (int)gridDim.x - 1) {
      __builtin_amdgcn_fence(__ATOMIC_ACQUIRE, "agent");
      asm volatile("s_waitcnt vmcnt(0)" ::: "memory");
    }
  }
  __syncthreads();
  const bool last = misc[17] != 0;
  __syncthreads();
  if (last) vq_fold_stats<NW>(reinterpret_cast<double*>(smem), tid, lane, wave, partial, (int)gridDim.x * NW, ctl, K, N, d, counts_out, stats_out);
#ifdef VQ_STAMPS
  VQ_ST(6);
  __syncthreads();
  if (tid < 128) vq_dbg[(size_t)blockIdx.x * 128 + tid] = (&vq_ts[0][0])[tid];
  if (tid == 0) { vq_dbg[(size_t)gridDim.x * 128 + 2 * blockIdx.x] = __builtin_amdgcn_s_memtime() - t_begin; vq_dbg[(size_t)gridDim.x * 128 + 2 * blockIdx.x + 1] = wall_clock64() - w_begin; }
#endif
}
```

### vq-vae_amd/csrc/vq_common.hpp

```cpp
#pragma once
#include "frl_common.hpp"
#include "frl_reduce.hpp"
#include <math.h>

#define VQ_IDX_BITS 7
#define VQ_IDX_MASK 127u
#define VQ_MAX_CHUNK 512
#define VQ_FAST_ROWS 128

#define VQ_SQ_BINS 9
struct VqHeader {
  unsigned enmax_bits;
  int namb;
  double sq_fix;
  int done;
  int pad;
  unsigned long long sq_bins[VQ_SQ_BINS];
};
static_assert(sizeof(VqHeader) <= 256, "the workspace keeps 256 bytes for the header");
struct VqCtl { int done; int namb; int pad[62]; };

#ifdef VQ_STAMPS
__device__ unsigned long long* vq_dbg;
#define VQ_ST(i) do { const unsigned long long t_now = __builtin_amdgcn_s_memtime(); if (lane == 0) vq_ts[wave][i] += t_now - t_prev; t_prev = t_now; } while (0)
// ... 72 lines not shown
  const float err_rel = (float)(4 * q + 8) * 1.1920929e-7f;
  const float thr_rel = (3.0517578125e-5f + 2.f * err_rel) * 1.001953125f;
  return VqThr{thr_rel, sqrtf(enmax)};
}
template <typename T, int NF>
__device__ __forceinline__ float vq_row_threshold(const LQTile<T, NF>& z, VqThr th) {
  float zn = 0.f;
#pragma unroll
  for (int s = 0; s < NF; ++s)
#pragma unroll
    for (int e = 0; e < DT<T>::FE; ++e) { const float v = lq_get<T, NF>(z, s, e); zn = fmaf(v, v, zn); }
  zn += __shfl_xor(zn, 16, 64);
  zn += __shfl_xor(zn, 32, 64);
  const float sroot = sqrtf(zn) + th.enroot;
  return sroot * sroot * th.thr_rel + 1e-37f;
}

template <typename T, int NF>
__device__ __forceinline__ void vq_write_row(const LQTile<T, NF>& z, const float* E, T* zq_out, int64_t row, int code,
                                             int d, int kc, float& sq_acc) {
  constexpr int FE = DT<T>::FE, q = NF * FE;
  const float* er = E + (int64_t)code * d + q * kc;
  T* zo = zq_out + row * (int64_t)d + q * kc;
#pragma unroll
  for (int s = 0; s < NF * FE; ++s) {
    if (q * kc + s < d) {
      const float ev = to_f32(from_f32<T>(er[s]));
      zo[s] = from_f32<T>(ev);
      const float df = lq_get<T, NF>(z, s / FE, s % FE) - ev;
      sq_acc = fmaf(df, df, sq_acc);
    }
  }
}

struct VqBest { double d; int k; };
template <typename T, int NF, typename Exact>
__device__ __forceinline__ VqBest vq_resolve_inlane(const LQTile<T, NF>& z, const typename DT<T>::frag_t* __restrict__ frags,
                                                    const float* __restrict__ norms, int mb0, int mb1, int K, int lane, bool mine, float lm,
                                                    Exact exact) {
  const int kc = lane >> 4;
  double bestd = 1.0e300;
  int bk = 0x7fffffff, p0 = -1, p1 = -1;
  auto flush = [&]() {
    if (p0 >= 0) {
      double d0, d1;
      exact(p0, p1, d0, d1);
      if (d0 < bestd || (d0 == bestd && p0 < bk)) { bestd = d0; bk = p0; }
      if (p1 >= 0 && (d1 < bestd || (d1 == bestd && p1 < bk))) { bestd = d1; bk = p1; }
    }
    p0 = p1 = -1;
  };
  for (int mb = mb0; mb < mb1; ++mb) {
    f32x4 acc = *reinterpret_cast<const f32x4*>(norms + mb * 16 + 4 * kc);
#pragma unroll
    for (int s = 0; s < NF; ++s) acc = mfma16(frags[(size_t)(mb * NF + s) * 64 + lane], z.f[s], acc);
#pragma unroll
    for (int r = 0; r < 4; ++r) {
      const int code = mb * 16 + 4 * kc + r;
      const bool hit = mine && acc[r] <= lm && code < K;
      if (__builtin_amdgcn_ballot_w64(hit && p1 >= 0) != 0ull) flush();
      if (hit) { if (p0 < 0) p0 = code; else p1 = code; }
    }
  }
  flush();
#pragma unroll
  for (int off = 16; off <= 32; off <<= 1) {
    const double ob = __shfl_xor(bestd, off, 64);
    const int okk = __shfl_xor(bk, off, 64);
    if (ob < bestd || (ob == bestd && okk < bk)) { bestd = ob; bk = okk; }
  }
  return VqBest{bestd, bk};
}

template <int NW>
__device__ __forceinline__ void vq_flush_hist(const int* __restrict__ hist, int32_t* __restrict__ counts_acc, int K, int tid) {
  for (int k = tid; k < K; k += NW * 64) {
    const int h = hist[k];
    if (h) atomicAdd(&counts_acc[k], h);
  }
}

template <int NW>
__device__ __forceinline__ void vq_fold_stats(double* red, int tid, int lane, int wave, const float* partial, int npartial, VqCtl* ctl, int K, int64_t N, int d,
                                              int32_t* __restrict__ counts_out, float* __restrict__ stats_out) {
  int32_t* counts_acc = reinterpret_cast<int32_t*>(ctl + 1);
  double sp = 0.0;
  for (int i = tid; i < npartial; i += NW * 64) sp += (double)__hip_atomic_load(&partial[i], __ATOMIC_RELAXED, __HIP_MEMORY_SCOPE_AGENT);
  double hp = 0.0;
  for (int k = tid; k < K; k += NW * 64) {
    const int c = __hip_atomic_load(&counts_acc[k], __ATOMIC_RELAXED, __HIP_MEMORY_SCOPE_AGENT);
    counts_out[k] = c;
    __hip_atomic_store(&counts_acc[k], 0, __ATOMIC_RELAXED, __HIP_MEMORY_SCOPE_AGENT);
    const double p = (double)c / (double)N;
    hp += p * log(p + 1e-10);
  }
  sp = wave_sum_d(sp);
  hp = wave_sum_d(hp);
  if (lane == 0) { red[wave] = sp; red[NW + wave] = hp; }
  __syncthreads();
  if (tid == 0) {
    for (int w = 1; w < NW; ++w) { red[0] += red[w]; red[NW] += red[NW + w]; }
    stats_out[0] = (float)red[0];
    stats_out[1] = (float)exp(-red[NW]);
    stats_out[2] = (float)__hip_atomic_load(&ctl->namb, __ATOMIC_RELAXED, __HIP_MEMORY_SCOPE_AGENT);
    stats_out[3] = (float)(red[0] / ((double)N * (double)d));
    __hip_atomic_store(&ctl->namb, 0, __ATOMIC_RELAXED, __HIP_MEMORY_SCOPE_AGENT);
    __hip_atomic_store(&ctl->done, 0, __ATOMIC_RELAXED, __HIP_MEMORY_SCOPE_AGENT);
  }
}

__device__ __forceinline__ void vq_sq_bins_add(unsigned long long* bins, double* nonfinite, float v) {
  const unsigned u = __float_as_uint(v);
  const unsigned ex = (u >> 23) & 0xffu;
  if (ex == 0xffu || (u >> 31)) { atomicAdd(nonfinite, (double)v); return; }
  const unsigned m = ex ? ((u & 0x7fffffu) | 0x800000u) : (u & 0x7fffffu);
  if (m == 0u) return;
  const unsigned e = ex ? ex - 1u : 0u;
  const unsigned long long w = (unsigned long long)m << (e & 31u);
  atomicAdd(&bins[e >> 5], w & 0xffffffffull);
  if (w >> 32) atomicAdd(&bins[(e >> 5) + 1], w >> 32);
}
__device__ __forceinline__ double vq_sq_bins_value(const unsigned long long* bins) {
  double s = 0.0;
#pragma unroll
  for (int b = VQ_SQ_BINS - 1; b >= 0; --b) s = s * 4294967296.0 + (double)bins[b];
  return s * 0x1p-149;
}
```

### vq-vae_amd/csrc/vq_prepare.hpp

```cpp
#pragma once
#include "vq_common.hpp"

template <typename T, int NF>
__global__ void vq_prepare_kernel(const float* __restrict__ E, int K, int d, float* __restrict__ en, int kpad,
                                  typename DT<T>::frag_t* __restrict__ pk, int total, int npack_blocks, int* __restrict__ ctl) {
  constexpr int FE = DT<T>::FE;
  constexpr int q = NF * FE;
  if ((int)blockIdx.x >= npack_blocks) {
    const int k = ((int)blockIdx.x - npack_blocks) * blockDim.x + threadIdx.x;
    if (k >= kpad) return;
    if (k < 64) ctl[k] = 0;
    if (k < K) ctl[64 + k] = 0;
    float s = 3.0e38f;
    if (k < K) {
      s = 0.f;
      for (int j = 0; j < d; ++j) {
        const float v = to_f32(from_f32<T>(E[(int64_t)k * d + j]));
        s = fmaf(v, v, s);
      }
    }
    en[k] = s;
    return;
  }
  const int i = blockIdx.x * blockDim.x + threadIdx.x;
  if (i >= total) return;
  const int ln = i & 63, fs = i >> 6;
  const int s = fs % NF, mb = fs / NF;
  const int code = mb * 16 + (ln & 15), kq = ln >> 4;
  if constexpr (FE == 8) {
    bf16x8 v;
#pragma unroll
    for (int e = 0; e < 8; ++e) {
      const int ch = q * kq + 8 * s + e;
      v[e] = (code < K && ch < d) ? (bf16)(-2.f * (float)(bf16)E[(int64_t)code * d + ch]) : (bf16)0.f;
    }
    pk[i] = v;
  } else {
    const int ch = q * kq + s;
    pk[i] = (code < K && ch < d) ? -2.f * E[(int64_t)code * d + ch] : 0.f;
  }
}
```

### vq-vae_amd/frl_hip/_lib.py

```python
from __future__ import annotations

import ctypes
import os
from ctypes import c_char_p, c_float, c_int, c_int64, c_size_t, c_void_p

_HERE = os.path.dirname(os.path.abspath(__file__))
LIB_PATH = os.path.join(_HERE, "libfrlhip_%s.so" % os.environ["FRL_HIP_LIB_TAG"] if os.environ.get("FRL_HIP_LIB_TAG") else "libfrlhip.so")

F32, BF16, F16 = 0, 1, 2
ACT_NONE, ACT_RELU, ACT_SIGMOID = 0, 1, 2

_lib = None


class FrlHipError(RuntimeError):
    pass


P, I, L, F, S, D = c_void_p, c_int, c_int64, c_float, c_size_t, ctypes.c_double
SIGNATURES = {
    "frl_version": (c_int, []),
    "frl_last_error": (c_char_p, []),
    "frl_device_arch": (c_int, [c_char_p, I]),
    "frl_kernel_timing_enable": (c_int, [I]),
    "frl_kernel_timing_report": (c_int, [c_char_p, I]),
    "frl_pack_cache_table_bytes": (S, []),
    "frl_pack_cache_create": (c_int, [P, S]),
    "frl_pack_cache_destroy": (c_int, [I]),
    "frl_pack_cache_activate": (c_int, [I]),
    "frl_pack_cache_images": (c_int, [I]),
    "frl_pack_cache_refresh": (c_int, [I, P]),
    "frl_conv_workspace_bytes": (S, [I, I, I]),
    "frl_conv1x1_fwd": (c_int, [P, P, P, P, L, I, I, I, I, P, S, P]),
    "frl_conv1x1_bwd_data": (c_int, [P, P, I, P, P, L, I, I, I, P, S, P]),
    "frl_conv1x1_bwd_data_add": (c_int, [P, P, I, P, P, P, L, I, I, I, P, S, P]),
    "frl_wgrad_set_max_workgroups": (c_int, [I]),
    "frl_wgrad_thin": (c_int, [I]),
    "frl_conv3x3_wgrad_force_generic": (c_int, [I]),
    "frl_conv3x3_tile32": (c_int, [I]),
    "frl_conv1x1_bwd_weight_workspace_bytes": (S, [L, I, I]),
    "frl_conv1x1_bwd_weight": (c_int, [P, P, I, P, P, P, L, I, I, I, P, S, P]),
    "frl_conv_tap_bwd_weight": (c_int, [P, P, I, P, P, L, L, P, L, I, I, I, I, I, I, P, S, I, P]),
    "frl_vq_workspace_bytes": (S, [L, I, I]),
    "frl_vq_assign_fwd": (c_int, [P, P, L, I, I, P, P, P, P, I, P, S, P]),
    "frl_vq_prepared_bytes": (S, [I, I]),
    "frl_vq_prepare": (c_int, [P, L, I, I, I, P, S, P]),
    "frl_vq_stream_tiles": (c_int, [I]),
    "frl_vq_assign_fwd_prepared": (c_int, [P, P, P, L, I, I, P, P, P, P, I, P, S, P]),
    "frl_vq_bwd": (c_int, [P, P, P, P, P, P, P, F, L, I, I, P, P, P, I, P, S, P]),
    "frl_vq_ema_update": (c_int, [P, P, I, I, F, F, P, P, P, P, P]),
    "frl_vq_revive_dead_codes": (c_int, [P, P, L, P, L, I, I, ctypes.c_uint64, P, P, P, I, P]),
    "frl_groupnorm_fwd": (c_int, [P, P, P, P, P, P, I, I, I, I, F, I, I, P]),
    "frl_groupnorm_bwd_workspace_bytes": (S, [I, I, I]),
    "frl_groupnorm_bwd": (c_int, [P, P, P, P, P, P, P, P, P, I, I, I, I, I, I, P, S, P]),
    "frl_scalar_combine": (c_int, [P, P, I, P, P, P]),
    "frl_scalar_fanout": (c_int, [P, P, I, P, P]),
    "frl_scalar_combine_dev": (c_int, [P, P, P, I, P, P, P]),
    "frl_scalar_combine_aux": (c_int, [P, P, P, P, I, P, P, P, P]),
    "frl_scalar_fanout_dev": (c_int, [P, P, P, I, P, P]),
    "frl_scalar_fanout_guard": (c_int, [P, P, P, P, I, P, P, P]),
    "frl_encoder2_supported": (c_int, [I, I, I, I, I, I, I]),
    "frl_encoder2_workspace_bytes": (S, [I]),
    "frl_encoder2_fwd": (c_int, [P, P, P, P, P, P, P, P, P, I, I, F, P, S, P]),
    "frl_encoder2_bwd": (c_int, [P, P, P, P, P, P, P, P, P, P, P, P, P, P, P, I, I, P, S, P]),
    "frl_decoder_mse_fused_supported": (c_int, [I, I, I, I]),
    "frl_decoder_mse_workspace_bytes": (S, [L, I]),
    "frl_decoder_mse_fwd": (c_int, [P, P, P, P, P, P, P, P, P, L, I, P, S, P]),
    "frl_decoder_mse_bwd": (c_int, [P, P, P, P, P, P, P, P, P, P, P, P, P, P, L, I, P, S, P]),
    "frl_decoder_mse_onepass_bytes": (S, [L, I]),
    "frl_decoder_mse_fwd_bwd": (c_int, [P, P, P, P, P, P, P, P, P, P, P, S, P, P, L, I, P]),
    "frl_decoder_mse_reduce": (c_int, [P, I, P, P, P, P, I, P]),
    "frl_mse_workspace_bytes": (S, []),
    "frl_mse_fwd": (c_int, [P, P, P, L, I, P, I, P, S, P]),
    "frl_mse_bwd": (c_int, [P, P, P, P, P, L, I, P, I, P]),
    "frl_film_modulate_fwd": (c_int, [P, P, P, P, L, I, L, I, I, P]),
    "frl_film_modulate_bwd": (c_int, [P, P, P, P, P, P, L, I, L, I, I, P]),
    "frl_film_fused_supported": (c_int, [I, I, I, I]),
    "frl_film_fused_workspace_bytes": (S, []),
    "frl_film_fused_fwd": (c_int, [P] * 13 + [I, I, I, P, S, P]),
    "frl_film_fused_bwd": (c_int, [P] * 20 + [I, I, I, P, S, P]),
    "frl_gate_blend_fwd": (c_int, [P, P, P, F, P, P, L, I, P]),
    "frl_gate_blend_bwd": (c_int, [P, P, P, P, F, P, P, L, I, P]),
    "frl_mean_time_fwd": (c_int, [P, P, L, I, L, I, P]),
    "frl_add": (c_int, [P, P, F, P, L, I, P]),
    "frl_normalize_tiles": (c_int, [P, I, P, P, P, I, P, L, I, P]),
    "frl_gather_locations_fwd": (c_int, [P, L, L, L, I, I, I, P, L, P, I, P]),
    "frl_segment_sum_rows": (c_int, [P, P, P, L, I, P, L, I, P]),
    "frl_infonce_fwd": (c_int, [P, I, P, P, P, L, P, L, F, I, P, P, P, P, P, P]),
    "frl_infonce_pair_grads": (c_int, [P, I, P, P, P, P, L, L, F, I, P, P, P]),
    "frl_mutual_knn_max_points": (S, [I]),
    "frl_mutual_knn": (c_int, [P, I, I, P, P, F, I, P, P, P]),
    "frl_phase_pairs_max_points": (S, [I]),
    "frl_phase_pairs": (c_int, [P, P, I, I, I, P, P, I, I, I, I, F] + [P] * 11),
    "frl_spatial_pairs_max_hw": (c_int, []),
    "frl_spatial_pack_mask": (c_int, [P, I, I, I, P, P]),
    "frl_spatial_knn": (c_int, [P, I, I, I, P, I, P, P, P, I, P, P, P, P, P]),
    "frl_spatial_negatives": (c_int, [P, I, I, I, P, I, P, P, I, I, I, P, P, P, P, P, P]),
    "frl_spatial_pair_index": (c_int, [I, I, I, P, I, P, P, P, P, I, P, P, I, P, I, F, F] + [P] * 12),
    "frl_anchor_grid_max": (c_int, [I, I, I, I, I]),
    "frl_anchor_grid": (c_int, [P, I, I, I, I, I, I, P, I, P, P, P, P]),
    "frl_anchor_supplement": (c_int, [P, I, I, I, P, P, I, P, P, P, P, P, P]),
    "frl_anchor_inverse_frequency": (c_int, [P, P, I, I, I, P, I, P, P, P]),
    "frl_spectral_negatives": (c_int, [P, L, I, P, I, I, P, L, F, F, P, P, P, P, P]),
    "frl_pair_sims_workspace_bytes": (S, [L]),
    "frl_pair_sims": (c_int, [P, L, I, P, L, P, P, P, P, S, P]),
    "frl_type_baseline_workspace_bytes": (S, [I, I]),
    "frl_type_baseline": (c_int, [P, P, I, I, I, I, I, P, P, P, P, S, P]),
    "frl_leakage_workspace_bytes": (S, [L, I, I]),
    "frl_leakage_fwd": (c_int, [P, I, P, I, L, I, I, P, P, P, P, S, P]),
    "frl_leakage_bwd": (c_int, [P, I, P, P, P, P, L, I, I, P, I, P]),
    "frl_gmm_workspace_bytes": (S, [L, I, I, I]),
    "frl_gmm_pivot": (c_int, [P, L, I, P, P, S, P]),
    "frl_gmm_em_step": (c_int, [P, P, L, I, I, P, P, P, P, I, I, P, P, S, P]),
    "frl_gmm_m_step": (c_int, [L, I, I, P, P, P, P, P, D, D, I, P, I, P, I, P, S, P]),
    "frl_gmm_score": (c_int, [P, L, I, I, P, P, P, P, P, P, P, P]),
    "frl_phase_summary": (c_int, [P, P, L, I, I, F, F, P, P, P]),
    "frl_probe_workspace_bytes": (S, [I, I, I]),
    "frl_probe_pivot": (c_int, [P, I, I, P, I, I, P, I, I, P, I, I, L, P, P, S, P]),
    "frl_probe_accumulate": (c_int, [P, I, I, P, I, I, P, I, I, P, I, I, L, P, I, P, P, P, S, P]),
    "frl_probe_evaluate": (c_int, [P, I, I, P, I, I, P, I, I, P, I, I, L, P, P, P, I, P, P, P, P, S, P]),
    "frl_strata_workspace_bytes": (S, [I, I, I, I]),
    "frl_strata_contingency": (c_int, [P, I, P, I, P, I, P, I, I, I, L, I, I, P, P, P, P]),
    "frl_strata_moments": (c_int, [P, P, I, P, I, P, I, I, I, I, I, L, I, P, I, I, P, P, P, P, P, P, S, P]),
    "frl_quantile_workspace_bytes": (S, [I, I, I]),
    "frl_quantile_append": (c_int, [P, P, I, P, I, P, I, P, I, I, I, L, I, I, I, P, P, L, P, P, P, P, P, P]),
    "frl_quantile_select": (c_int, [P, P, L, P, P, P, L, I, I, P, I, I, P, P, P, P, P, S, P]),
    "frl_host_parallel_copy": (c_int, [P, P, S, I]),
    "frl_normalize_chunk_tiles": (c_int, [P, I, I, I, I, I, P, I, I, P, P, I, P, P]),
    "frl_conv3x3_fwd": (c_int, [P, P, P, P, I, I, I, I, I, I, I, P, S, P]),
    "frl_conv3x3_fwd_gate_blend": (c_int, [P, P, P, P, P, P, P, I, I, I, I, I, I, P, S, P]),
    "frl_conv3x3_bwd_data": (c_int, [P, P, I, P, P, I, I, I, I, I, I, P, S, P]),
    "frl_conv3x3_bwd_data_fused": (c_int, [P, P, I, P, P, P, P, P, I, I, I, I, I, I, P, S, P]),
# ... 89 lines not shown
```

### vq-vae_amd/frl_hip/functional.py

```python
from __future__ import annotations

from typing import Optional

import torch
from torch.autograd import Function
from torch.autograd.function import once_differentiable

from . import ops
from .ops import ACT_NONE, ACT_RELU, ACT_SIGMOID


def _c(t: Optional[torch.Tensor]):
    return None if t is None else (t if t.is_contiguous() else t.contiguous())


def _wanted(ctx, first: int, grads):
    out = []
    for i, g in enumerate(grads):
        if g is not None and not ctx.needs_input_grad[first + i]:
            ops.discard(g)
            g = None
        out.append(g)
    return tuple(out)


class Conv1x1Fn(Function):

    @staticmethod
    def forward(ctx, x, w, bias, act):
        y = ops.conv1x1_fwd(x, w, bias, act)
        ctx.act = act
        ctx.has_bias = bias is not None
        ctx.save_for_backward(x, w, y if act != ACT_NONE else None)
        return y

    @staticmethod
    @once_differentiable
    def backward(ctx, dy):
        x, w, y = ctx.saved_tensors
        dy = _c(dy)
        dx = ops.conv1x1_bwd_data(dy, w, y, ctx.act) if ctx.needs_input_grad[0] else None
        dw = db = None
        if ctx.needs_input_grad[1] or (ctx.has_bias and ctx.needs_input_grad[2]):
            dw, db = ops.conv1x1_bwd_weight(dy, x, y, ctx.act, want_bias=ctx.has_bias and ctx.needs_input_grad[2])
            dw, = _wanted(ctx, 1, (dw.reshape(w.shape),))
        return dx, dw, db, None


class Conv3x3Fn(Function):

    @staticmethod
    def forward(ctx, x, w, bias, act):
        y = ops.conv3x3_fwd(x, w, bias, act)
        ctx.act = act
        ctx.has_bias = bias is not None
        ctx.save_for_backward(x, w, y if act != ACT_NONE else None)
        return y

    @staticmethod
    @once_differentiable
    def backward(ctx, dy):
        x, w, y = ctx.saved_tensors
        dy = _c(dy)
        dx = ops.conv3x3_bwd_data(dy, w, y, ctx.act) if ctx.needs_input_grad[0] else None
        dw = db = None
        if ctx.needs_input_grad[1] or (ctx.has_bias and ctx.needs_input_grad[2]):
            dw, db = ops.conv3x3_bwd_weight(dy, x, y, ctx.act, want_bias=ctx.has_bias and ctx.needs_input_grad[2])
            dw, = _wanted(ctx, 1, (dw,))
        return dx, dw, db, None


class GroupNormFn(Function):

    @staticmethod
    def forward(ctx, x, gamma, beta, groups, eps, relu):
        y, mean, rstd = ops.groupnorm_fwd(x, gamma, beta, groups, eps, relu)
        ctx.groups, ctx.relu = groups, relu
        ctx.save_for_backward(x, gamma, beta, mean, rstd)
        return y

    @staticmethod
    @once_differentiable
    def backward(ctx, dy):
        x, gamma, beta, mean, rstd = ctx.saved_tensors
        dx, dg, db = ops.groupnorm_bwd(_c(dy), x, gamma, beta, mean, rstd, ctx.groups, ctx.relu)
        return _wanted(ctx, 0, (dx, dg, db)) + (None, None, None)


class Encoder2Fn(Function):

    @staticmethod
    def forward(ctx, x, w1, g1, b1, w2, g2, b2, eps):
        z, stats = ops.encoder2_fwd(x, w1, g1, b1, w2, g2, b2, eps)
        ctx.save_for_backward(x, w1, g1, b1, w2, g2, b2, stats)
        return z

    @staticmethod
    @once_differentiable
    def backward(ctx, dz):
        x, w1, g1, b1, w2, g2, b2, stats = ctx.saved_tensors
        grads = ops.encoder2_bwd(x, _c(dz), w1, g1, b1, w2, g2, b2, stats)
        return (None,) + _wanted(ctx, 1, grads) + (None,)


class ScalarCombineFn(Function):

    @staticmethod
    def forward(ctx, coefs, mults, aux_coefs, promises, *terms):
        res = ops.scalar_combine([t.detach() for t in terms], coefs, mults, aux_coefs)
        ctx.coefs = tuple(float(c) for c in coefs)
        ctx.mults = mults
        ctx.promises = promises
        ctx.mark_non_differentiable(*res[1:])
        return res if aux_coefs is not None else res + (None,)

    @staticmethod
    @once_differentiable
    def backward(ctx, g, g_ok, g_aux):
        gg = ops.scalar_fanout(g.reshape(1).float().contiguous(), ctx.coefs, ctx.mults, ctx.promises)
        return (None, None, None, None) + tuple(gg[i] for i in range(len(ctx.coefs)))


def scalar_combine(terms, coefs, mults=None, aux_coefs=None):
    fits = all(torch.is_tensor(t) and t.is_cuda and t.dtype == torch.float32 and t.numel() == 1 for t in terms) and 1 <= len(terms) <= 8
    if not fits:
        tot = None
        for i, (t, c) in enumerate(zip(terms, coefs)):
            v = t if c == 1.0 else c * t
            if mults is not None and mults[i] is not None:
                v = v * mults[i].reshape(()).to(v.device)
            tot = v if tot is None else tot + v
        if aux_coefs is None:
            return tot, None
        aux = sum(float(c) * t.detach() for t, c in zip(terms, aux_coefs))
        return tot, None, aux
    promises = []
    for t in terms:
        pr = getattr(t, "_frl_promise", None)
        promises.append(None if pr is None else pr[0])
        if pr is not None:
            pr[1]["guarded"] = True
    loss, ok, aux = ScalarCombineFn.apply(tuple(coefs), None if mults is None else tuple(mults), None if aux_coefs is None else tuple(aux_coefs),
                                          tuple(promises) if any(p is not None for p in promises) else None, *[t.reshape(()) for t in terms])
    return (loss, ok) if aux_coefs is None else (loss, ok, aux)


class SobelFn(Function):
    @staticmethod
    def forward(ctx, x):
        return ops.sobel_fwd(x)

    @staticmethod
    @once_differentiable
    def backward(ctx, dg):
        return ops.sobel_bwd(_c(dg))


class EdgeSmoothFn(Function):

    @staticmethod
    def forward(ctx, x, a_logit, b_logit, rank, dil):
        sm, res, a_soft, b_soft = ops.edge_smooth_fwd(x, a_logit, b_logit, rank, dil)
        ctx.rank, ctx.dil = rank, dil
        ctx.save_for_backward(x, a_soft, b_soft)
        return sm, res

    @staticmethod
    @once_differentiable
    def backward(ctx, d_sm, d_res):
        x, a_soft, b_soft = ctx.saved_tensors
        d_sm, d_res = _c(d_sm), _c(d_res)
        d_tot = ops.add(d_sm, d_res, -1.0)
        dx, da, db = ops.edge_smooth_bwd(d_tot, x, a_soft, b_soft, ctx.rank, ctx.dil, dx_add=d_res)
        return dx, da, db, None, None


class GateBlendFn(Function):

    @staticmethod
    def forward(ctx, smoothed, residual, gate_raw, min_gate):
        out, gate = ops.gate_blend_fwd(smoothed, residual, gate_raw, min_gate)
        ctx.min_gate = min_gate
        ctx.set_materialize_grads(False)
        ctx.save_for_backward(residual, gate_raw)
        return out, gate

    @staticmethod
    @once_differentiable
    def backward(ctx, dout, dgate):
        residual, gate_raw = ctx.saved_tensors
        if dout is None:
            dout = torch.zeros_like(residual)
        dout = _c(dout)
        dres, dgraw = ops.gate_blend_bwd(dout, _c(dgate), residual, gate_raw, ctx.min_gate)
        return dout if ctx.needs_input_grad[0] else None, dres, dgraw, None


class SpatialSmoothFn(Function):

    @staticmethod
    def forward(ctx, x, w_mb, b_mb, w_a, b_a, w_b, b_b, w_g0, b_g0, w_g2, b_g2, rank, dil, min_gate):
# ... 81 lines not shown
        ctx.cfg = (dilation, groups, eps)
        ctx.drop_mask = drop_mask
        ctx.save_for_backward(x, conv_w, conv_b, gn_w, gn_b, gate_w, gate_b, proj_w, proj_b)
        return y

    @staticmethod
    @once_differentiable
    def backward(ctx, dy):
        x, conv_w, conv_b, gn_w, gn_b, gate_w, gate_b, proj_w, proj_b = ctx.saved_tensors
        dilation, groups, eps = ctx.cfg
        pw = None if proj_w is None else proj_w.reshape(proj_w.shape[0], proj_w.shape[1])
        g = ops.tcn_block_bwd(x, _c(dy), conv_w, conv_b, gn_w, gn_b, gate_w, gate_b, pw, proj_b, dilation, groups, eps,
                              drop_mask=ctx.drop_mask, want_dx=ctx.needs_input_grad[0])
        dpw = g["proj_w"].reshape(proj_w.shape) if proj_w is not None else None
        return (g["dx"] if ctx.needs_input_grad[0] else None,) + _wanted(ctx, 1, (g["conv_w"], g["conv_b"], g["gn_w"], g["gn_b"], g["gate_w"],
                                                                                g["gate_b"], dpw, g.get("proj_b"))) + (None, None, None, None)


class TcnChainHeadFn(Function):

    @staticmethod
    def forward(ctx, x, *args):
        params, (head_w, head_b, groups, eps) = args[:18], args[18:22]
        want_xtype = len(args) > 22 and bool(args[22])
        blocks = [tuple(params[6 * i:6 * i + 6]) + (d, groups, False) for i, d in enumerate((1, 2, 4))]
        y1, y2, y3, h, *xt = ops.tcn_chain_fwd(x, blocks, head_w, head_b, eps, want_xtype=want_xtype)
        ctx.cfg = (groups, eps)
        ctx.n_tail = len(args) - 20
        ctx.save_for_backward(x, y1, y2, y3, head_w, *params)
        if want_xtype:
            ctx.mark_non_differentiable(xt[0])
            ctx.set_materialize_grads(False)
            return h, xt[0]
        return h

    @staticmethod
    @once_differentiable
    def backward(ctx, dh, _dxt=None):
        if dh is None:
            return (None,) * (21 + ctx.n_tail)
        x, y1, y2, y3, head_w, *params = ctx.saved_tensors
        groups, eps = ctx.cfg
        dh = _c(dh)
        w2 = head_w.reshape(head_w.shape[0], head_w.shape[1])
        dw_h = db_h = None
        if ctx.needs_input_grad[19] or ctx.needs_input_grad[20]:
            dw_h, db_h = ops.conv1x1_bwd_weight(dh, y3, None, ACT_NONE, want_bias=ctx.needs_input_grad[20])
            dw_h, = _wanted(ctx, 19, (dw_h.reshape(head_w.shape),))
        head_in_kernel = groups == 8 and ops.tcn_block_bwd_head_supported(y2, dh, w2, 4)
        dy = None if head_in_kernel else ops.conv1x1_bwd_data(dh, w2, None, ACT_NONE)
        grads = [None] * 18
        for i, (xin, dil) in reversed(list(enumerate(zip((x, y1, y2), (1, 2, 4))))):
            cw, cb, gw, gb, tw, tb = params[6 * i:6 * i + 6]
            if i == 2 and head_in_kernel:
                g = ops.tcn_block_bwd_head(xin, dh, w2, cw, cb, gw, gb, tw, tb, dil, eps)
            else:
                g = ops.tcn_block_bwd(xin, dy, cw, cb, gw, gb, tw, tb, None, None, dil, groups, eps, want_dx=(i > 0 or ctx.needs_input_grad[0]))
            grads[6 * i:6 * i + 6] = [g["conv_w"], g["conv_b"], g["gn_w"], g["gn_b"], g["gate_w"], g["gate_b"]]
            dy = g["dx"]
        return (dy if ctx.needs_input_grad[0] else None,) + _wanted(ctx, 1, grads) + (dw_h, db_h) + (None,) * ctx.n_tail


class FilmFn(Function):

    @staticmethod
    def forward(ctx, h, gamma, beta):
        ctx.save_for_backward(h, gamma)
        return ops.film_modulate_fwd(h, gamma, beta)

    @staticmethod
    @once_differentiable
    def backward(ctx, dout):
        h, gamma = ctx.saved_tensors
        return ops.film_modulate_bwd(_c(dout), h, gamma)


class FilmFusedFn(Function):

    @staticmethod
    def forward(ctx, h, z_type, *params):
        z, gamma, beta = ops.film_fused_fwd(z_type, h, params)
        ctx.save_for_backward(h, z_type, *params)
        ctx.mark_non_differentiable(gamma, beta)
        return z, gamma, beta

    @staticmethod
    @once_differentiable
    def backward(ctx, dz, _dg, _db):
        h, z_type, *params = ctx.saved_tensors
        dh, grads = ops.film_fused_bwd(z_type, h, _c(dz), params)
        return (dh if ctx.needs_input_grad[0] else None, None) + _wanted(ctx, 2, grads)


class ChannelScaleFn(Function):

    @staticmethod
    def forward(ctx, x, scale):
        b, c = scale.shape
        ctx.save_for_backward(scale)
        zero = torch.zeros_like(scale)
        ctx.zero = zero
        return ops.film_modulate_fwd(x.reshape(b, -1, 1, c), scale.reshape(b, 1, c), zero.reshape(b, 1, c)).reshape(x.shape)

    @staticmethod
    @once_differentiable
    def backward(ctx, dy):
        (scale,) = ctx.saved_tensors
        b, c = scale.shape
        dy = _c(dy)
        return ops.film_modulate_fwd(dy.reshape(b, -1, 1, c), scale.reshape(b, 1, c), ctx.zero.reshape(b, 1, c)).reshape(dy.shape), None


class VQFn(Function):

    @staticmethod
    def forward(ctx, z, codebook, prep=None):
        idx, zq, stats, counts = ops.vq_assign(z, codebook, prep)
        d = z.shape[-1]
        n = z.numel() // d
        ctx.set_materialize_grads(False)
        ctx.save_for_backward(z, codebook, idx, counts, zq)
        st = stats.clone()
        ctx.mark_non_differentiable(idx, counts, stats)
        return zq, st[3], st.narrow(0, 3, 1).reshape(()), st[1], idx, counts, stats

    @staticmethod
    @once_differentiable
    def backward(ctx, g_zq, g_cb, g_cm, g_perp, g_idx, g_counts, g_stats):
        z, codebook, idx, counts, zq = ctx.saved_tensors
        if g_cm is not None and g_cb is not None:
            gs = torch.stack([g_cm.reshape(()).float(), g_cb.reshape(()).float()])
        else:
            gs = torch.zeros(2, dtype=torch.float32, device=z.device)
            if g_cm is not None:
                gs[0] = g_cm
            if g_cb is not None:
                gs[1] = g_cb
        gz, ge, _ = ops.vq_bwd(_c(g_zq), z, codebook, idx, counts, gs, 1.0,
                               want_gz=ctx.needs_input_grad[0], want_ge=ctx.needs_input_grad[1], zq=zq)
        return gz, ge, None


class MseFn(Function):

    @staticmethod
    def forward(ctx, pred, target, mask):
        stats = ops.mse_fwd(pred, target, mask)
        ctx.save_for_backward(pred, target, mask, stats)
        return stats[0].clone()

    @staticmethod
    @once_differentiable
    def backward(ctx, g):
        pred, target, mask, stats = ctx.saved_tensors
        return ops.mse_bwd(pred, target, mask, g.reshape(1).float().contiguous(), stats), None, None


class DecoderMseFn(Function):

    @staticmethod
    def forward(ctx, z, w1, b1, w2, b2, target, mask, want_xhat, onepass=None):
        ctx.set_materialize_grads(False)
        ctx.onepass = onepass
        if onepass is not None:
            stats, dz, slabs = ops.decoder_mse_fwd_bwd(z, w1, b1, w2, b2, target, mask, onepass[0])
            ctx.held = (dz, slabs)
            ctx.save_for_backward(w1, b1, w2, b2)
            return stats.narrow(0, 0, 1).reshape(()), None
        stats, xhat = ops.decoder_mse_fwd(z, w1, b1, w2, b2, target, mask, want_xhat)
        ctx.save_for_backward(z, w1, b1, w2, b2, target, mask, stats)
        if xhat is not None:
            ctx.mark_non_differentiable(xhat)
        return stats.narrow(0, 0, 1).reshape(()), xhat

    @staticmethod
    @once_differentiable
    def backward(ctx, g, g_xhat):
        if ctx.onepass is not None:
            held, ctx.held = ctx.held, None
            if held is None:
                raise RuntimeError("decoder_mse: the gradients of a one-pass loss (grad_scale=) are handed out once; a second backward "
                                   "through it needs the two-kernel path (grad_scale=None)")
            if g is None:
                return (None,) * 9
            grad_scale, state = ctx.onepass
            if not state["guarded"]:
                ops.scalar_fanout(g.reshape(1).float().contiguous(), (1.0,), None, (grad_scale,))
            dz, slabs = held
            w1, b1, w2, b2 = ctx.saved_tensors
            gw = (None,) * 4
            if any(ctx.needs_input_grad[1:5]):
                dw1, db1, dw2, db2 = ops.decoder_mse_reduce(slabs, w1, b1, w2, b2)
                gw = _wanted(ctx, 1, (dw1.reshape(w1.shape), db1, dw2.reshape(w2.shape), db2))
            del held, slabs
            return (dz if ctx.needs_input_grad[0] else None,) + gw + (None, None, None, None)
        z, w1, b1, w2, b2, target, mask, stats = ctx.saved_tensors
        if g is None:
            return (None,) * 9
        dz, dw1, db1, dw2, db2 = ops.decoder_mse_bwd(z, w1, b1, w2, b2, target, mask, g.reshape(1).float().contiguous(), stats)
        return _wanted(ctx, 0, (dz, dw1.reshape(w1.shape), db1, dw2.reshape(w2.shape), db2)) + (None, None, None, None)


def decoder_mse(z, w1, b1, w2, b2, target, mask=None, want_xhat=False, grad_scale=None):
    if mask is not None:
        mask = mask.reshape(-1).to(torch.uint8).contiguous()
    if (grad_scale is not None and not want_xhat and torch.is_grad_enabled()
            and any(torch.is_tensor(t) and t.requires_grad for t in (z, w1, b1, w2, b2))):
        state = {"guarded": False}
        loss, xhat = DecoderMseFn.apply(z, w1, b1, w2, b2, target, mask, False, (grad_scale, state))
        loss._frl_promise = (grad_scale, state)
        return loss, xhat
    return DecoderMseFn.apply(z, w1, b1, w2, b2, target, mask, want_xhat)
# ... 23 lines not shown
```

### vq-vae_amd/frl_hip/models/vqvae.py

```python
from __future__ import annotations

from typing import Dict, Optional

import torch
import torch.distributed as dist
import torch.nn as nn

from .. import functional as Fh
from .. import ops
from ..losses.variance_covariance import variance_covariance_loss
from .blocks import Conv2DHead
from .representation import RepresentationModel


class VectorQuantizer(nn.Module):

    def __init__(self, codebook_size: int = 256, emb_dim: int = 64, beta: float = 0.25, quantizer: str = "st",
                 ema_decay: float = 0.99, ema_eps: float = 1e-5):
        super().__init__()
        if quantizer not in ("st", "ema"):
            raise ValueError("quantizer must be 'st' or 'ema' (scripts/train_vqvae.py:412)")
        self.codebook_size, self.emb_dim, self.beta = codebook_size, emb_dim, beta
        self.quantizer, self.ema_decay, self.ema_eps = quantizer, ema_decay, ema_eps
        self.codebook = nn.Parameter(torch.empty(codebook_size, emb_dim).uniform_(-1.0 / codebook_size, 1.0 / codebook_size),
# ... 20 lines not shown
        self.last_counts = counts
        self.last_stats = stats
        if self.quantizer == "ema":
            vq_loss = Fh.scalar_combine([l_cm], [self.beta])[0]
            if self.training:
                with torch.no_grad():
                    _, _, sums = ops.vq_bwd(None, z_rows.detach(), self.codebook.detach(), idx, counts, None, 0.0,
                                            want_gz=False, want_ge=False, want_sums=True)
                self._pending_ema = (sums, counts)
                if not self.defer_ema:
                    self.apply_ema()
        elif raw_terms:
            vq_loss = ((l_cb, 1.0), (l_cm, float(self.beta)))
        else:
            vq_loss = Fh.scalar_combine([l_cb, l_cm], [1.0, self.beta])[0]
        return zq, vq_loss, perp, idx

    @torch.no_grad()
    def apply_ema(self, ok: Optional[torch.Tensor] = None) -> None:
        if self._pending_ema is None:
            return
        sums, counts = self._pending_ema
        self._pending_ema = None
        if dist.is_available() and dist.is_initialized() and dist.get_world_size() > 1:
            counts = counts.clone()
            dist.all_reduce(sums)
            dist.all_reduce(counts)
        ops.vq_ema_update(sums, counts, self.ema_count, self.ema_sum, self.codebook.data, self.ema_decay, self.ema_eps, ok)
        if self._prepared is not None:
            self._prepared = ((None, None, self._prepared[0][2]), self._prepared[1])
        if self.defer_ema:
            torch.autograd.graph.increment_version(self.codebook)

    def drop_ema(self) -> None:
        self._pending_ema = None


class VQVAE(RepresentationModel):

    def __init__(self, in_features: Optional[int] = None, codebook_size: int = 256, emb_dim: int = 64, beta: float = 0.25,
                 hidden: int = 128, quantizer: str = "st", ema_decay: float = 0.99, ema_eps: float = 1e-5,
                 phase: bool = True, phase_codebook_size: int = 0, lambda_recon: float = 1.0, lambda_vq: float = 1.0,
                 cont_dim: Optional[int] = None, cat_vocab_sizes=None, naip_bands: Optional[int] = None, cat_emb_dim: int = 8,
                 lambda_vcr: float = 0.0, vcr_variance_weight: float = 1.0, vcr_covariance_weight: float = 1.0,
                 vcr_variance_target: float = 1.0, **repr_kwargs):
        if cont_dim is not None:
            if in_features is not None and int(in_features) != int(cont_dim):
                raise ValueError(f"cont_dim ({cont_dim}) and in_features ({in_features}) name the same axis and disagree")
            in_features = int(cont_dim)
        if in_features is None:
            in_features = 64
        if cat_vocab_sizes:
            raise ValueError("cat_vocab_sizes is not empty: categorical inputs are not part of the (time, y, x, feature) tile VQ-VAE "
                             f"(got {sorted(dict(cat_vocab_sizes))}); pass an empty mapping")
        self_legacy = dict(cat_vocab_sizes=dict(cat_vocab_sizes or {}), naip_bands=None if naip_bands is None else int(naip_bands),
                           cat_emb_dim=int(cat_emb_dim))
        repr_kwargs.setdefault("z_type_dim", emb_dim)
        if repr_kwargs["z_type_dim"] != emb_dim:
            raise ValueError("emb_dim must equal z_type_dim (the quantizer acts on z_type)")
        if "type_encoder_channels" not in repr_kwargs and emb_dim != 64:
            repr_kwargs["type_encoder_channels"] = (128, emb_dim)
        super().__init__(type_in_channels=in_features, phase_in_channels=in_features, **repr_kwargs)
        self.in_features, self.phase, self.lambda_recon, self.lambda_vq = in_features, phase, lambda_recon, lambda_vq
        self.cont_dim, self.legacy_inputs = in_features, self_legacy
        if lambda_vcr < 0:
            raise ValueError("lambda_vcr must be >= 0")
        self.lambda_vcr = float(lambda_vcr)
        self.vcr_variance_weight, self.vcr_covariance_weight = float(vcr_variance_weight), float(vcr_covariance_weight)
        self.vcr_variance_target = float(vcr_variance_target)
        self.quant = VectorQuantizer(codebook_size, emb_dim, beta, quantizer, ema_decay, ema_eps)
        self.decoder_type = Conv2DHead(emb_dim, [hidden], in_features)
        if phase:
            self.decoder_phase = Conv2DHead(self.z_phase_dim, [hidden], in_features)
            if phase_codebook_size:
                self.quant_phase = VectorQuantizer(phase_codebook_size, self.z_phase_dim, beta, quantizer, ema_decay, ema_eps)
        self.lambda_vq_dev: Optional[torch.Tensor] = None
        self.codebook_manager = None
        self._manager_takes_rows = False
        self.defer_codebook_hooks = False
        self._pending_manager = None
        self.fused_decoder = True
        self.onepass_decoder = True
        self.chain_xtype = True
        self._grad_scale_dev = {}
        self.concurrent_phase = True
        self._side_stream = None

    def phase_stream(self, device):
        if self._side_stream is None:
            self._side_stream = torch.cuda.Stream(device=device)
        return self._side_stream

    def attach_codebook_manager(self, manager) -> None:
        import inspect
        self.codebook_manager = manager
        upd = getattr(manager, "update", None)
        self._manager_takes_rows = upd is not None and len(inspect.signature(upd).parameters) >= 2

    def _grad_scale(self, device) -> torch.Tensor:
        key = (str(device), float(self.lambda_recon))
        t = self._grad_scale_dev.get(key)
        if t is None:
            t = self._grad_scale_dev[key] = torch.full((1,), float(self.lambda_recon), dtype=torch.float32, device=device)
        return t

    def _vcr_term(self, z: torch.Tensor):
        total, _, _ = variance_covariance_loss(z.reshape(-1, z.shape[-1]), self.vcr_variance_weight, self.vcr_covariance_weight,
                                               self.vcr_variance_target)
        return (total, self.lambda_vcr)

    def _decode_loss(self, dec: Conv2DHead, z: torch.Tensor, target: torch.Tensor, mask, want_recon: bool, onepass: bool = False):
        l0, l2 = dec.layers[0], dec.layers[-1]
        if (len(dec.layers) == 3 and self.fused_decoder
                and ops.decoder_mse_supported(z.shape[-1], l0.out_channels, l2.out_channels, z)):
            w1 = l0.weight.reshape(l0.out_channels, l0.in_channels)
            w2 = l2.weight.reshape(l2.out_channels, l2.in_channels)
            gs = self._grad_scale(z.device) if (onepass and self.onepass_decoder and not want_recon) else None
            return Fh.decoder_mse(z, w1, l0.bias, w2, l2.bias, target, mask, want_recon, grad_scale=gs)
        xhat = dec(z)
        return Fh.mse_loss(xhat, target, mask), xhat

    def _phase_branch(self, tile, z_type_detached, mask, return_recon, onepass: bool = False, h=None) -> Dict[str, torch.Tensor]:
        b, t, hh, ww, f = tile.shape
        out: Dict[str, torch.Tensor] = {}
        z_phase = self.forward_phase_nhwc(tile, z_type_detached, h=h)
        zp_in = z_phase
        terms = []
        if hasattr(self, "quant_phase"):
            zpq, pvq, pperp, pidx = self.quant_phase(z_phase.reshape(-1, z_phase.shape[-1]))
            zp_in = zpq.reshape(z_phase.shape)
            terms.append(self._vq_term(pvq))
            out.update(idx_phase=pidx, vq_loss_phase=pvq, perplexity_phase=pperp)
        if mask is None or mask.dim() == 4:
            pmask = mask
        else:
            pmask = mask.unsqueeze(1).expand(b, t, hh, ww).contiguous()
        l_phase, xhat_phase = self._decode_loss(self.decoder_phase, zp_in, tile, pmask, return_recon, onepass)
        terms.append((l_phase, self.lambda_recon))
        if self.lambda_vcr > 0 and self.training:
            terms.append(self._vcr_term(z_phase))
            out["vcr_loss_phase"] = terms[-1][0].detach()
        out.update(z_phase=z_phase, l_phase=l_phase, loss_terms=terms)
        if xhat_phase is not None:
            out["xhat_phase"] = xhat_phase
        return out

    def forward_tiles(self, tile: torch.Tensor, mask: Optional[torch.Tensor] = None,
                      return_recon: bool = False, differentiable_vq_loss: bool = False) -> Dict[str, torch.Tensor]:
        self._require_gpu(tile)
        tile = self._rows(tile)
        b, t, hh, ww, f = tile.shape
        concurrent = self.phase and self.concurrent_phase and tile.is_cuda
        pre = None
        if self.phase and self.chain_xtype and tile.is_cuda and not differentiable_vq_loss:
            if concurrent:
                main, side = torch.cuda.current_stream(), self.phase_stream(tile.device)
                side.wait_stream(main)
                tile.record_stream(side)
                with torch.cuda.stream(side):
                    pre = self.phase_chain_xtype(tile)
                if pre is not None:
                    main.wait_stream(side)
                    pre[1].record_stream(main)
            else:
                pre = self.phase_chain_xtype(tile)
        if pre is not None:
# ... 183 lines not shown
```

### vq-vae_amd/frl_hip/ops.py

```python
from __future__ import annotations

import ctypes
from typing import Optional, Tuple

import torch

from . import _lib
from ._lib import ACT_NONE, ACT_RELU, ACT_SIGMOID, BF16, F32, check

_WS = {}

_TIMING = {"on": False, "events": {}}


def set_timing(on: bool) -> None:
    _TIMING["on"] = bool(on)
    _TIMING["events"] = {}


def timing_summary():
    torch.cuda.synchronize()
    return {k: (len(v), sum(a.elapsed_time(b) for a, b in v)) for k, v in _TIMING["events"].items()}


def kernel_timing(on: bool) -> None:
    _lib.load().frl_kernel_timing_enable(1 if on else 0)


def kernel_timing_report():
    buf = ctypes.create_string_buffer(1 << 16)
    _lib.load().frl_kernel_timing_report(buf, len(buf))
    out = {}
    for line in buf.value.decode().splitlines():
        name, calls, ms = line.rsplit("\t", 2)
        out[name] = (int(calls), float(ms))
    return out


_INDEX_FLAG = {}


def sanitize_indices(idx: torch.Tensor, n: int, what: str) -> torch.Tensor:
    import os
    bad = ((idx < -n) | (idx >= n)).any()
    flag = _INDEX_FLAG.get(idx.device)
    if flag is None:
        flag = _INDEX_FLAG[idx.device] = torch.zeros(1, dtype=torch.int32, device=idx.device)
    flag |= bad.to(torch.int32)
    if os.environ.get("FRL_HIP_CHECK_INDICES", "0") == "1" and bool(bad.item()):
        raise IndexError(f"{what}: index out of range for {n} rows")
    return torch.where(idx < 0, idx + n, idx).clamp_(0, max(n - 1, 0))


def index_errors(device=None, reset: bool = True) -> bool:
    hit = False
    for dev, flag in _INDEX_FLAG.items():
        if device is None or torch.device(device) == dev:
            hit |= bool(flag.item())
            if reset:
                flag.zero_()
    return hit


class PackCache:

    def __init__(self, device, nbytes: int = 64 << 20):
        lib = _lib.load()
        self.arena = torch.empty(int(nbytes) + lib.frl_pack_cache_table_bytes(), dtype=torch.uint8, device=device)
        self.handle = lib.frl_pack_cache_create(ctypes.c_void_p(self.arena.data_ptr()), self.arena.numel())
        if self.handle <= 0:
            check(self.handle, "frl_pack_cache_create")
        self._prev = 0

    def __enter__(self):
        self._prev = _lib.load().frl_pack_cache_activate(self.handle)
        return self

    def __exit__(self, *a):
        _lib.load().frl_pack_cache_activate(self._prev)
        return False

    def refresh(self) -> None:
        check(_lib.load().frl_pack_cache_refresh(self.handle, _stream()), "frl_pack_cache_refresh")

    @property
    def images(self) -> int:
        return _lib.load().frl_pack_cache_images(self.handle)

    def close(self) -> None:
        if self.handle > 0:
            _lib.load().frl_pack_cache_destroy(self.handle)
            self.handle = 0

    def __del__(self):
        try:
            self.close()
        except Exception:
            pass


class span:

    def __init__(self, name):
        self.name = name

    def __enter__(self):
        if _TIMING["on"]:
            self.e0, self.e1 = torch.cuda.Event(enable_timing=True), torch.cuda.Event(enable_timing=True)
            self.e0.record()
        return self

    def __exit__(self, *a):
        if _TIMING["on"]:
            self.e1.record()
            _TIMING["events"].setdefault(self.name, []).append((self.e0, self.e1))
        return False


def _timed(name):
    def deco(fn):
        def wrapper(*a, **kw):
            if not _TIMING["on"]:
                return fn(*a, **kw)
            e0, e1 = torch.cuda.Event(enable_timing=True), torch.cuda.Event(enable_timing=True)
            e0.record()
            out = fn(*a, **kw)
            e1.record()
            _TIMING["events"].setdefault(name, []).append((e0, e1))
            return out
        wrapper.__name__ = fn.__name__
        wrapper.__doc__ = fn.__doc__
        return wrapper
    return deco


def _dt(t: torch.Tensor) -> int:
    if t.dtype == torch.float32:
        return F32
    if t.dtype == torch.bfloat16:
        return BF16
    raise TypeError(f"frl_hip supports float32 and bfloat16 activations, got {t.dtype}")


def _p(t: Optional[torch.Tensor]):
    return ctypes.c_void_p(0 if t is None else t.data_ptr())


def _stream():
    return ctypes.c_void_p(torch.cuda.current_stream().cuda_stream)


def _chk_rows(t: torch.Tensor, c: int, name: str):
    if not t.is_cuda:
        raise _lib.FrlHipError(f"{name}: tensor must live on the GPU (no CPU fallback)")
    if not t.is_contiguous() or t.shape[-1] != c:
        raise ValueError(f"{name}: expected contiguous [..., {c}] rows, got {tuple(t.shape)} stride {t.stride()}")


def _chk_like(t: torch.Tensor, ref: torch.Tensor, name: str):
    if t.shape != ref.shape or t.dtype != ref.dtype or t.device != ref.device or not t.is_contiguous():
        raise ValueError(f"{name}: expected a contiguous {tuple(ref.shape)} {ref.dtype} tensor on {ref.device}, got "
                         f"{tuple(t.shape)} {t.dtype} stride {t.stride()}")


def _f32(t: Optional[torch.Tensor], name: str):
    if t is None:
# ... 119 lines not shown
    ws = _WS.get(key)
    if ws is None or ws.numel() < nbytes:
        ws = torch.empty(max(nbytes, 1 << 20), dtype=torch.uint8, device=device)
        _WS[key] = ws
    return ws


@_timed("conv1x1_fwd")
def conv1x1_fwd(x: torch.Tensor, w: torch.Tensor, bias: Optional[torch.Tensor], act: int = ACT_NONE) -> torch.Tensor:
    cout, cin = w.shape[0], w.shape[1]
    _chk_rows(x, cin, "conv1x1_fwd.x")
    w = _f32(w.reshape(cout, cin), "w")
    y = torch.empty(x.shape[:-1] + (cout,), dtype=x.dtype, device=x.device)
    p = x.numel() // cin
    lib = _lib.load()
    ws = workspace(lib.frl_conv_workspace_bytes(cin, cout, 1), x.device)
    check(lib.frl_conv1x1_fwd(_p(x), _p(w), _p(_f32(bias, "bias")), _p(y), p, cin, cout, act, _dt(x), _p(ws), ws.numel(),
                              _stream()), "frl_conv1x1_fwd")
    return y


@_timed("conv1x1_bwd_data")
def conv1x1_bwd_data(dy: torch.Tensor, w: torch.Tensor, y: Optional[torch.Tensor] = None, act: int = ACT_NONE,
                     add: Optional[torch.Tensor] = None) -> torch.Tensor:
    cout, cin = w.shape[0], w.shape[1]
    _chk_rows(dy, cout, "conv1x1_bwd_data.dy")
    w = _f32(w.reshape(cout, cin), "w")
    dx = torch.empty(dy.shape[:-1] + (cin,), dtype=dy.dtype, device=dy.device)
    p = dy.numel() // cout
    lib = _lib.load()
    ws = workspace(lib.frl_conv_workspace_bytes(cin, cout, 1), dy.device)
    if add is not None:
        _chk_like(add, dx, "conv1x1_bwd_data.add")
        check(lib.frl_conv1x1_bwd_data_add(_p(dy), _p(y), act, _p(w), _p(dx), _p(add), p, cin, cout, _dt(dy), _p(ws), ws.numel(),
                                           _stream()), "frl_conv1x1_bwd_data_add")
        return dx
    check(lib.frl_conv1x1_bwd_data(_p(dy), _p(y), act, _p(w), _p(dx), p, cin, cout, _dt(dy), _p(ws), ws.numel(), _stream()),
          "frl_conv1x1_bwd_data")
    return dx


def _conv1x1_bwd_weight_impl(dy: torch.Tensor, x: torch.Tensor, y: Optional[torch.Tensor] = None, act: int = ACT_NONE,
                       want_bias: bool = True, scalar_frags: bool = False) -> Tuple[torch.Tensor, Optional[torch.Tensor]]:
    cout, cin = dy.shape[-1], x.shape[-1]
    _chk_rows(dy, cout, "bwd_weight.dy")
    _chk_rows(x, cin, "bwd_weight.x")
    p = dy.numel() // cout
    lib = _lib.load()
    nbytes = lib.frl_conv1x1_bwd_weight_workspace_bytes(p, cin, cout)
    ws = workspace(nbytes, dy.device)
    dw = grad_empty((cout, cin), dy.device)
    db = grad_empty((cout,), dy.device) if want_bias else None
    check(lib.frl_conv_tap_bwd_weight(_p(dy), _p(y), act, _p(x), _p(dw), cin, 1, _p(db), p, cin, cout, 1, 1, 0,
                                      _dt(dy), _p(ws), ws.numel(), 1 if scalar_frags else 0, _stream()),
          "frl_conv_tap_bwd_weight")
    return dw, db


conv1x1_bwd_weight = _timed("conv1x1_bwd_weight")(_conv1x1_bwd_weight_impl)


def wgrad_thin(on: bool) -> bool:
    return bool(_lib.load().frl_wgrad_thin(1 if on else 0))


def vq_stream_tiles(nt: int) -> int:
    return int(_lib.load().frl_vq_stream_tiles(int(nt)))


@_timed("vq_prepare")
def vq_prepare(codebook: torch.Tensor, n_rows: int, dtype: torch.dtype, out: Optional[torch.Tensor] = None) -> torch.Tensor:
    k, d = codebook.shape
    cb = _f32(codebook, "codebook")
    lib = _lib.load()
    nbytes = lib.frl_vq_prepared_bytes(k, d)
    if out is None or out.numel() < nbytes or out.device != cb.device:
        out = torch.empty(nbytes, dtype=torch.uint8, device=cb.device)
    check(lib.frl_vq_prepare(_p(cb), int(n_rows), k, d, BF16 if dtype == torch.bfloat16 else F32, _p(out), out.numel(), _stream()),
          "frl_vq_prepare")
    return out


@_timed("vq_assign")
def vq_assign(z: torch.Tensor, codebook: torch.Tensor, prep: Optional[torch.Tensor] = None):
    k, d = codebook.shape
    _chk_rows(z, d, "vq_assign.z")
    cb = _f32(codebook, "codebook")
    n = z.numel() // d
    lib = _lib.load()
    ws = workspace(lib.frl_vq_workspace_bytes(n, k, d), z.device)
    idx = torch.empty(n, dtype=torch.int32, device=z.device)
    zq = torch.empty_like(z)
    stats = torch.empty(4, dtype=torch.float32, device=z.device)
    counts = torch.empty(k, dtype=torch.int32, device=z.device)
    if prep is not None and (prep.dtype != torch.uint8 or prep.device != z.device or prep.numel() < lib.frl_vq_prepared_bytes(k, d)):
        raise ValueError("vq_assign: prep is not a prepared-codebook image for this codebook")
    check(lib.frl_vq_assign_fwd_prepared(_p(z), _p(cb), _p(prep), n, k, d, _p(idx), _p(zq), _p(stats), _p(counts), _dt(z), _p(ws),
                                         ws.numel(), _stream()), "frl_vq_assign_fwd")
    return idx, zq, stats, counts


@_timed("vq_bwd")
def vq_bwd(g_out: Optional[torch.Tensor], z: torch.Tensor, codebook: torch.Tensor, idx: torch.Tensor,
           counts: torch.Tensor, gscale: Optional[torch.Tensor], beta: float, want_gz: bool = True,
           want_ge: bool = True, want_sums: bool = False, zq: Optional[torch.Tensor] = None):
    if codebook.dim() != 2:
        raise ValueError(f"vq_bwd: codebook must be [K, d], got {tuple(codebook.shape)}")
    k, d = codebook.shape
    if not z.is_cuda:
        raise ValueError("vq_bwd.z: tensor must live on the GPU (no CPU fallback)")
    if z.dim() < 1 or z.shape[-1] != d or not z.is_contiguous():
        raise ValueError(f"vq_bwd.z: expected contiguous [..., {d}] rows, got {tuple(z.shape)} stride {z.stride()}")
    n = z.numel() // d
    if g_out is not None:
        _chk_like(g_out, z, "vq_bwd.g_out")
    if zq is not None:
        _chk_like(zq, z, "vq_bwd.zq")
    for t, m, name in ((idx, n, "idx"), (counts, k, "counts")):
        if t.dtype != torch.int32 or t.numel() != m or not t.is_contiguous() or t.device != z.device:
            raise ValueError(f"vq_bwd.{name}: expected a contiguous int32 tensor of {m} elements on {z.device}, got "
                             f"{tuple(t.shape)} {t.dtype} on {t.device}")
    if gscale is not None and (gscale.dtype != torch.float32 or gscale.device != z.device or gscale.numel() < 2
                               or not gscale.is_contiguous()):
        raise ValueError("vq_bwd.gscale: expected a contiguous float32 tensor of at least 2 elements on the device of z")
    if codebook.device != z.device:
        raise ValueError("vq_bwd: codebook and z live on different devices")
    lib = _lib.load()
    ws = workspace(lib.frl_vq_workspace_bytes(n, k, d), z.device)
    gz = torch.empty_like(z) if want_gz else None
    ge = grad_empty((k, d), z.device) if want_ge else None
    sums = torch.empty(k, d, dtype=torch.float32, device=z.device) if want_sums else None
    cb32 = _f32(codebook, "codebook")
    if _DEFER["on"]:
        _DEFER["keep"] += [t for t in (counts, gscale, cb32) if t is not None]
    check(lib.frl_vq_bwd(_p(g_out), _p(z), _p(zq), _p(cb32), _p(idx), _p(counts), _p(gscale), float(beta),
                         n, k, d, _p(gz), _p(ge), _p(sums), _dt(z), _p(ws), ws.numel(), _stream()), "frl_vq_bwd")
    return gz, ge, sums


def vq_ema_update(sums, counts, ema_count, ema_sum, codebook, decay: float, eps: float, ok: Optional[torch.Tensor] = None):
    k, d = codebook.shape
    if ok is not None and (ok.dtype != torch.float32 or not ok.is_cuda or ok.numel() < 1):
        raise ValueError("vq_ema_update: ok must be a float32 CUDA tensor")
    check(_lib.load().frl_vq_ema_update(_p(sums), _p(counts), k, d, float(decay), float(eps), _p(ema_count),
                                        _p(ema_sum), _p(codebook), _p(ok), _stream()), "frl_vq_ema_update")


def _mult_ptrs(mults, n):
    if mults is None or all(m is None for m in mults):
        return None
    for m in mults:
        if m is not None and (m.dtype != torch.float32 or m.numel() != 1 or not m.is_cuda):
            raise ValueError("scalar_combine: multipliers are float32 CUDA scalars")
    return (ctypes.c_void_p * n)(*[0 if m is None else m.data_ptr() for m in mults])


def scalar_combine(terms, coefs, mults=None, aux_coefs=None):
    n = len(terms)
    dev = terms[0].device
    for t in terms:
        if t.dtype != torch.float32 or t.numel() != 1 or not t.is_cuda:
            raise ValueError("scalar_combine: terms are float32 CUDA scalars")
    ptrs = (ctypes.c_void_p * n)(*[t.data_ptr() for t in terms])
    cf = (ctypes.c_float * n)(*[float(c) for c in coefs])
    out = torch.empty((), dtype=torch.float32, device=dev)
    ok = torch.empty(1, dtype=torch.float32, device=dev)
    if aux_coefs is None:
        check(_lib.load().frl_scalar_combine_dev(ptrs, cf, _mult_ptrs(mults, n), n, _p(out), _p(ok), _stream()), "frl_scalar_combine")
        return out, ok
    ac = (ctypes.c_float * n)(*[float(c) for c in aux_coefs])
    aux = torch.empty((), dtype=torch.float32, device=dev)
    check(_lib.load().frl_scalar_combine_aux(ptrs, cf, _mult_ptrs(mults, n), ac, n, _p(out), _p(ok), _p(aux), _stream()), "frl_scalar_combine_aux")
    return out, ok, aux


def scalar_fanout(g, coefs, mults=None, promises=None):
    n = len(coefs)
    cf = (ctypes.c_float * n)(*[float(c) for c in coefs])
    out = torch.empty(n, dtype=torch.float32, device=g.device)
    if promises is None or all(p is None for p in promises):
        check(_lib.load().frl_scalar_fanout_dev(_p(g), cf, _mult_ptrs(mults, n), n, _p(out), _stream()), "frl_scalar_fanout")
        return out
    for p in promises:
        if p is not None and (p.dtype != torch.float32 or p.numel() != 1 or p.device != g.device):
            raise ValueError("scalar_fanout: promises are float32 scalars on the gradient's device")
    pp = (ctypes.c_void_p * n)(*[0 if p is None else p.data_ptr() for p in promises])
    check(_lib.load().frl_scalar_fanout_guard(_p(g), cf, _mult_ptrs(mults, n), pp, n, _p(out), _p(_grad_scale_flag(g.device)), _stream()),
          "frl_scalar_fanout_guard")
    return out


_GRAD_SCALE_FLAG = {}


def _grad_scale_flag(device) -> torch.Tensor:
    device = torch.device(device)
    if device.index is None:
        device = torch.device(device.type, torch.cuda.current_device())
    flag = _GRAD_SCALE_FLAG.get(device)
    if flag is None:
        flag = _GRAD_SCALE_FLAG[device] = torch.zeros(1, dtype=torch.int32, device=device)
    return flag


def grad_scale_errors(device=None, reset: bool = True) -> bool:
    hit = False
    for dev, flag in _GRAD_SCALE_FLAG.items():
        if device is None or torch.device(device) == dev:
            hit |= bool(flag.item())
            if reset:
                flag.zero_()
    return hit


def check_grad_scale(device=None) -> None:
    if grad_scale_errors(device):
        raise RuntimeError("decoder_mse: a loss whose gradients were computed in the forward for a promised upstream gradient (grad_scale) "
# ... 504 lines not shown
def conv3x3_bwd_data(dy, w, y=None, act: int = ACT_NONE, add=None, sub_from=None, out_y=None, out_act: int = ACT_NONE):
    b, h, wd, cout = dy.shape
    cin = w.shape[1]
    dx = torch.empty(b, h, wd, cin, dtype=dy.dtype, device=dy.device)
    lib = _lib.load()
    ws = workspace(lib.frl_conv_workspace_bytes(cin, cout, 9), dy.device)
    if out_y is not None:
        if add is not None or sub_from is not None:
            raise ValueError("conv3x3_bwd_data: out_y does not combine with add / sub_from")
        _chk_like(out_y, dx, "conv3x3_bwd_data.out_y")
        check(lib.frl_conv3x3_bwd_data_outmask(_p(dy), _p(y), act, _p(_f32(w, "w")), _p(dx), _p(out_y), out_act, b, h, wd, cin, cout, _dt(dy),
                                               _p(ws), ws.numel(), _stream()), "frl_conv3x3_bwd_data_outmask")
        return dx
    if add is not None or sub_from is not None:
        out2 = None
        if add is not None:
            _chk_like(add, dx, "conv3x3_bwd_data.add")
        if sub_from is not None:
            _chk_like(sub_from, dx, "conv3x3_bwd_data.sub_from")
            out2 = torch.empty_like(dx)
        check(lib.frl_conv3x3_bwd_data_fused(_p(dy), _p(y), act, _p(_f32(w, "w")), _p(dx), _p(add), _p(sub_from), _p(out2), b, h, wd,
                                             cin, cout, _dt(dy), _p(ws), ws.numel(), _stream()), "frl_conv3x3_bwd_data_fused")
        return dx if sub_from is None else (dx, out2)
    check(lib.frl_conv3x3_bwd_data(_p(dy), _p(y), act, _p(_f32(w, "w")), _p(dx), b, h, wd, cin, cout, _dt(dy), _p(ws),
                                   ws.numel(), _stream()), "frl_conv3x3_bwd_data")
    return dx


@_timed("conv3x3_bwd_weight")
def conv3x3_bwd_weight(dy, x, y=None, act: int = ACT_NONE, scalar_frags: bool = False, want_bias: bool = True):
    b, h, wd, cout = dy.shape
    cin = x.shape[-1]
    lib = _lib.load()
    ws = workspace(lib.frl_conv3x3_bwd_weight_workspace_bytes(b, h, wd, cin, cout), dy.device)
    dw = grad_empty((cout, cin, 3, 3), dy.device)
    db = grad_empty((cout,), dy.device) if want_bias else None
    check(lib.frl_conv3x3_bwd_weight(_p(dy), _p(y), act, _p(x), _p(dw), _p(db), b, h, wd, cin, cout, _dt(dy), _p(ws),
                                     ws.numel(), 1 if scalar_frags else 0, _stream()), "frl_conv3x3_bwd_weight")
    return dw, db


@_timed("sobel_fwd")
def sobel_fwd(x):
    b, h, w, c = x.shape
    g = torch.empty(b, h, w, 2 * c, dtype=x.dtype, device=x.device)
    check(_lib.load().frl_sobel_fwd(_p(x), _p(g), b, h, w, c, _dt(x), _stream()), "frl_sobel_fwd")
    return g


@_timed("sobel_bwd")
def sobel_bwd(dg, add=None):
    b, h, w, c2 = dg.shape
    dx = torch.empty(b, h, w, c2 // 2, dtype=dg.dtype, device=dg.device)
    if add is not None:
        _chk_like(add, dx, "sobel_bwd.add")
        check(_lib.load().frl_sobel_bwd_add(_p(dg), _p(dx), _p(add), b, h, w, c2 // 2, _dt(dg), _stream()), "frl_sobel_bwd_add")
        return dx
    check(_lib.load().frl_sobel_bwd(_p(dg), _p(dx), b, h, w, c2 // 2, _dt(dg), _stream()), "frl_sobel_bwd")
    return dx


@_timed("edge_smooth_fwd")
def edge_smooth_fwd(x, a_logit, b_logit, rank: int, coarse_dilation: int):
    b, h, w, c = x.shape
    sm, res = torch.empty_like(x), torch.empty_like(x)
    a_soft, b_soft = torch.empty_like(a_logit), torch.empty_like(b_logit)
    check(_lib.load().frl_edge_smooth_stencil_fwd(_p(x), _p(a_logit), _p(b_logit), _p(sm), _p(res), _p(a_soft), _p(b_soft),
                                                  b, h, w, c, rank, coarse_dilation, _dt(x), _stream()),
          "frl_edge_smooth_stencil_fwd")
    return sm, res, a_soft, b_soft


@_timed("edge_smooth_bwd")
def edge_smooth_bwd(d_smoothed, x, a_soft, b_soft, rank: int, coarse_dilation: int, dx_add: Optional[torch.Tensor] = None):
    b, h, w, c = x.shape
    dx = torch.empty_like(x)
    da, db = torch.empty_like(a_soft), torch.empty_like(b_soft)
    if dx_add is not None and (dx_add.shape != x.shape or dx_add.dtype != x.dtype or not dx_add.is_contiguous()):
        raise ValueError("edge_smooth_bwd: dx_add must match x")
    check(_lib.load().frl_edge_smooth_stencil_bwd(_p(d_smoothed), _p(x), _p(a_soft), _p(b_soft), _p(dx), _p(da), _p(db), _p(dx_add),
                                                  b, h, w, c, rank, coarse_dilation, _dt(x), _stream()),
          "frl_edge_smooth_stencil_bwd")
    return dx, da, db


def fusion_enabled(name: str) -> bool:
    import os
    return name not in os.environ.get("FRL_HIP_DISABLE", "").split(",")


def smooth_heads_supported(x: torch.Tensor, hidden: int, rank: int, wa, ba, wb, bb) -> bool:
    if ba is None or bb is None or x.dim() != 4 or not x.is_cuda or not fusion_enabled("heads"):
        return False
    if tuple(wa.shape[:2]) != (8 * rank, hidden) or tuple(wb.shape[:2]) != (x.shape[-1] * rank, hidden):
        return False
    return bool(_lib.load().frl_smooth_heads_supported(x.shape[-1], hidden, rank, _dt(x)))


@_timed("smooth_heads_fwd")
def smooth_heads_fwd(x, feat, wa, ba, wb, bb, coarse_dilation: int):
    b, h, w, c = x.shape
    _chk_rows(x, c, "smooth_heads_fwd.x")
    _chk_like(feat, x, "smooth_heads_fwd.feat")
    lib = _lib.load()
    ws = workspace(lib.frl_smooth_heads_workspace_bytes(b * h * w), x.device)
    sm, res = torch.empty_like(x), torch.empty_like(x)
    check(lib.frl_smooth_heads_fwd(_p(x), _p(feat), _p(_f32(wa, "wa")), _p(_f32(ba, "ba")), _p(_f32(wb, "wb")), _p(_f32(bb, "bb")), _p(sm), _p(res),
                                   b, h, w, coarse_dilation, _p(ws), ws.numel(), _stream()), "frl_smooth_heads_fwd")
    return sm, res


@_timed("smooth_heads_bwd")
def smooth_heads_bwd(d_smoothed, x, feat, wa, ba, wb, bb, coarse_dilation: int, dx_add: Optional[torch.Tensor] = None, dfeat_relu: bool = False):
    b, h, w, c = x.shape
    for t, n in ((d_smoothed, "d_smoothed"), (feat, "feat")):
        _chk_like(t, x, f"smooth_heads_bwd.{n}")
    if dx_add is not None:
        _chk_like(dx_add, x, "smooth_heads_bwd.dx_add")
    lib = _lib.load()
    npix = b * h * w
    ws = workspace(lib.frl_smooth_heads_workspace_bytes(npix), x.device)
    scratch = torch.empty(lib.frl_smooth_heads_bwd_scratch_bytes(npix), dtype=torch.uint8, device=x.device)
    dx, dfeat = torch.empty_like(x), torch.empty_like(feat)
    dwa, dba, dwb, dbb = (grad_empty(t.shape, x.device) for t in (wa, ba, wb, bb))
    check(lib.frl_smooth_heads_bwd_masked(_p(d_smoothed), _p(x), _p(feat), _p(_f32(wa, "wa")), _p(_f32(ba, "ba")), _p(_f32(wb, "wb")),
                                          _p(_f32(bb, "bb")), _p(dx_add), _p(dx), _p(dfeat), _p(dwa), _p(dba), _p(dwb), _p(dbb), _p(scratch),
                                          scratch.numel(), b, h, w, coarse_dilation, int(dfeat_relu), _p(ws), ws.numel(), _stream()),
          "frl_smooth_heads_bwd_masked")
    return dx, dfeat, dwa, dba, dwb, dbb


def tcn_hot_supported(x: torch.Tensor, cin: int, cout: int, groups: int, dilation: int, has_projection: bool) -> bool:
    return bool(_lib.load().frl_tcn_hot_supported(x.shape[1], cin, cout, groups, dilation, int(has_projection), _dt(x)))


def _check_drop_mask(drop_mask, x, hot: bool):
    if drop_mask is None:
        return
    if not hot:
        raise NotImplementedError("the generic TCN kernels take no Dropout1d mask (only the hot configuration: bf16, 64 channels, T = 5, "
                                  "8 groups, dilation 1/2/4); GatedResidualBlock routes other shapes through its two-input formulation")
    b, t, c = x.shape[0], x.shape[1], x.shape[-1]
    if drop_mask.dtype != x.dtype or not drop_mask.is_contiguous() or drop_mask.numel() != x.numel() // t:
        raise ValueError("drop_mask must be a contiguous [B, HW.., C] tensor of x's dtype")


@_timed("tcn_block_fwd")
def tcn_block_fwd(x, conv_w, conv_b, gn_w, gn_b, gate_w, gate_b, proj_w, proj_b, dilation: int, groups: int,
                  eps: float = 1e-5, allow_hot: bool = True, drop_mask=None):
    b, t, cin = x.shape[0], x.shape[1], x.shape[-1]
    cout = conv_w.shape[0]
    hw = x.numel() // (b * t * cin)
    y = torch.empty(x.shape[:-1] + (cout,), dtype=x.dtype, device=x.device)
    lib = _lib.load()
    hot = bool(allow_hot and lib.frl_tcn_hot_supported(t, cin, cout, groups, dilation, int(proj_w is not None), _dt(x)))
    _check_drop_mask(drop_mask, x, hot)
    if hot:
        ws = workspace(lib.frl_tcn_hot_fwd_workspace_bytes(), x.device)
        check(lib.frl_tcn_hot_fwd(_p(x), _p(drop_mask), _p(_f32(conv_w, "conv_w")), _p(conv_b), _p(gn_w), _p(gn_b),
                                  _p(_f32(gate_w.reshape(cout, cout), "gate_w")), _p(gate_b), _p(y), b * hw, hw, dilation, float(eps),
                                  _p(ws), ws.numel(), _stream()), "frl_tcn_hot_fwd")
        return y
    ws = workspace(lib.frl_conv_workspace_bytes(max(cin, cout), cout, 6), x.device)
    check(lib.frl_tcn_block_fwd(_p(x), _p(_f32(conv_w, "conv_w")), _p(conv_b), _p(gn_w), _p(gn_b),
                                _p(_f32(gate_w.reshape(cout, cout), "gate_w")), _p(gate_b), _p(proj_w), _p(proj_b),
                                _p(y), b * hw, hw, t, cin, cout, dilation, groups, float(eps), _dt(x), _p(ws), ws.numel(),
# ... 1201 lines not shown
```

### vq-vae_amd/frl_hip/training/trainer.py

```python
from __future__ import annotations

from typing import Dict, Optional

import torch
import torch.distributed as dist

from ..parallel import BucketedGradAllReduce
from .schedules import LambdaVQSchedule, beta_schedule, cosine_lr


class VQVAETrainer:
    def __init__(self, model, lr: float = 1e-4, min_lr: float = 1e-6, weight_decay: float = 0.01, max_norm: float = 1.0,
                 total_steps: int = 1000, betas=(0.9, 0.95), check_finite: bool = True, fused_optimizer: bool = True,
                 beta_schedule_cfg: Optional[dict] = None, lambda_vq_schedule: Optional[LambdaVQSchedule] = None,
                 pack_cache: bool = True, defer_reductions: bool = True):
        self.model = model
        self.defer_reductions = bool(defer_reductions)
        named = [(n, p) for n, p in model.named_parameters() if p.requires_grad]
        cb = [p for n, p in named if "quant" in n and "codebook" in n]
        rest = [p for n, p in named if not ("quant" in n and "codebook" in n)]
        groups = [{"params": rest, "weight_decay": weight_decay}]
        if cb:
            groups.append({"params": cb, "weight_decay": 0.0})
        on_gpu = bool(rest) and rest[0].is_cuda
# ... 142 lines not shown
            with torch.cuda.stream(side):
                for _ in range(2):
                    self._step_body(static_tile, static_mask)
            torch.cuda.current_stream(dev).wait_stream(side)
            graph = torch.cuda.CUDAGraph()
            with torch.cuda.graph(graph, pool=getattr(self, "_graph_pool", None)):
                out = self._step_body(static_tile, static_mask)
            if getattr(self, "_graph_pool", None) is None:
                self._graph_pool = graph.pool()
            mgr_z, mgr_ok = (getattr(mgr, "_z", None), getattr(mgr, "_z_ok", None)) if mgr is not None else (None, None)
            self._restore(snap)
        finally:
            if saved_after is not None:
                mgr.after_step = saved_after
        return dict(key=key, graph=graph, tile=static_tile, mask=static_mask, out=out, mgr_z=mgr_z, mgr_ok=mgr_ok)

    def _snapshot(self):
        m, o = self.model, self.opt
        st = dict(params=[p.detach().clone() for p in o.params], m=[t.clone() for t in o.exp_avg], v=[t.clone() for t in o.exp_avg_sq],
                  counters=o.counters.clone(), tensor_steps=o.tensor_steps.clone(), step_count=o.step_count,
                  buffers=[b.detach().clone() for b in m.buffers()])
        mgr = getattr(m, "codebook_manager", None)
        if mgr is not None and hasattr(mgr, "window"):
            st["window"] = None if mgr.window is None else mgr.window.clone()
            st["revived"] = None if getattr(mgr, "revived", None) is None else mgr.revived.clone()
        return st

    def _restore(self, st):
        m, o = self.model, self.opt
        with torch.no_grad():
            for p, q in zip(o.params, st["params"]):
                p.copy_(q)
            for a, b in zip(o.exp_avg, st["m"]):
                a.copy_(b)
            for a, b in zip(o.exp_avg_sq, st["v"]):
                a.copy_(b)
            o.counters.copy_(st["counters"])
            o.tensor_steps.copy_(st["tensor_steps"])
            for b, q in zip(m.buffers(), st["buffers"]):
                b.copy_(q)
        o.step_count = st["step_count"]
        o._key = None
        self._images_refresh()
        mgr = getattr(m, "codebook_manager", None)
        if mgr is not None and "window" in st and mgr.window is not None:
            if st["window"] is None:
                mgr.window.zero_()
            else:
                mgr.window.copy_(st["window"])
            if getattr(mgr, "revived", None) is not None:
                if st["revived"] is None:
                    mgr.revived.zero_()
                else:
                    mgr.revived.copy_(st["revived"])
        if hasattr(m, "_quantizers"):
            for qz in m._quantizers():
                qz.drop_ema()
                if qz._prepared is not None:
                    dtype = qz._prepared[0][2]
                    qz._prepared = ((None, None, dtype), qz._prepared[1])
                    qz.prepared(dtype, 1 << 20)

    def _images_current(self) -> None:
        if self.pack_cache is None:
            return
        vers = [p._version for p in self.params]
        if vers != self._pack_versions:
            self.pack_cache.refresh()
            self._pack_versions = vers

    def _images_refresh(self) -> None:
        if self.pack_cache is not None:
            self.pack_cache.refresh()
            self._pack_versions = [p._version for p in self.params]

    @staticmethod
    def _finite_flag(out):
        ok = out.get("loss_ok")
        if ok is not None:
            return ok
        return (out["loss"].detach().float() * 0.0 == 0.0).float().reshape(1)

    def _backward(self, loss):
        if self.defer_reductions and self.hip_opt and not (self.reducer is not None and self.reducer.active):
            from .. import ops
            with ops.deferred_reductions(self.opt.params):
                loss.backward()
        else:
            loss.backward()

    def _step_body(self, tile, mask):
        self.model.train()
        self.opt.zero_grad(set_to_none=True)
        dp = self.reducer is not None and self.reducer.active
        if dp:
            self.reducer.reset()

        def fwd_bwd():
            out_ = self.model.forward_tiles(tile, mask)
            ok_ = self._finite_flag(out_)
            if dp:
                self.reducer.flag_src = 1.0 - ok_
            self._backward(out_["loss"])
            return out_, ok_

        if self.pack_cache is not None:
            with self.pack_cache:
                out, ok = fwd_bwd()
        else:
            out, ok = fwd_bwd()
        grads = None
        if dp:
            self.reducer.finish(scatter=False)
            fg = self.reducer.flat_grads()
            grads = [fg[id(p)] if p.grad is not None else None for p in self.opt.params]
            ok = (self.reducer.flag_result() == 0).float()
        out["grad_norm"] = self.opt.step(self.max_norm, grads, ok)
        self._images_refresh()
        if getattr(self.model, "defer_codebook_hooks", False):
            self.model.commit_codebook_hooks(ok)
        if hasattr(self.model, "_quantizers"):
            for qz in self.model._quantizers():
                if qz._prepared is not None:
                    qz.prepared(qz._prepared[0][2], 1 << 20)
        return out

    @torch.no_grad()
    def evaluate(self, batches, max_batches: Optional[int] = None) -> Dict:
        m = self.model
        quants = m._quantizers() if hasattr(m, "_quantizers") else []
        saved_q = [(q.last_counts, q.last_stats) for q in quants]
        was_training, conc = m.training, getattr(m, "concurrent_phase", None)
        acc = counts = counts_p = None
        n_batches = 0
        m.eval()
        if conc is not None:
            m.concurrent_phase = False
        try:
            for i, batch in enumerate(batches):
                if max_batches is not None and i >= max_batches:
                    break
                tile, mask = (batch["tile"], batch.get("mask")) if isinstance(batch, dict) else (batch, None)
                out = m.forward_tiles(tile, mask)
                terms = [out["loss"], out["l_type"], out.get("l_phase"), out.get("vq_loss")]
                dev = out["loss"].device
                vals = torch.stack([torch.zeros((), dtype=torch.float64, device=dev) if v is None else v.detach().reshape(()).double()
                                    for v in terms])
                ok = torch.isfinite(vals[0]).reshape(1)
                row = torch.cat([torch.where(ok, vals, torch.zeros_like(vals)), ok.double(), torch.ones(1, dtype=torch.float64, device=dev)])
                acc = row if acc is None else acc + row
                c = quants[0].last_counts.to(torch.int64)
                counts = c if counts is None else counts + c
                if len(quants) > 1 and out.get("idx_phase") is not None:
                    cp = quants[1].last_counts.to(torch.int64)
                    counts_p = cp if counts_p is None else counts_p + cp
                n_batches += 1
        finally:
            m.train(was_training)
            if conc is not None:
                m.concurrent_phase = conc
            for q, (lc, ls) in zip(quants, saved_q):
                q.last_counts, q.last_stats = lc, ls

        res: Dict = dict(loss=0.0, l_type=0.0, l_phase=0.0, vq_loss=0.0, batches=0, skipped=0)
        if n_batches == 0:
            return res
        parts = [acc] + [x.double() for x in (counts, counts_p) if x is not None]
        host = torch.cat(parts).cpu().split([t.numel() for t in parts])
        self.check_promises()
        a = host[0]
        n_ok = int(a[4].item())
        for j, name in enumerate(("loss", "l_type", "l_phase", "vq_loss")):
            res[name] = float(a[j].item()) / n_ok if n_ok else 0.0
        res.update(batches=n_ok, skipped=n_batches - n_ok)

        def usage(cnt_host: torch.Tensor, cnt_dev: torch.Tensor, suffix: str):
            p = cnt_host / max(float(cnt_host.sum().item()), 1.0)
            nz = p[p > 0]
            res["counts" + suffix] = cnt_dev
            res["perplexity" + suffix] = float(torch.exp(-(nz * nz.log()).sum()).item()) if nz.numel() else 0.0
            res["codes_used" + suffix] = int((cnt_host > 0).sum().item())

        usage(host[1], counts, "")
        if counts_p is not None:
            usage(host[2], counts_p, "_phase")
        res["sums"] = dict(terms=acc[:4], finite_batches=acc[4], batches=acc[5], counts=counts,
                           **({"counts_phase": counts_p} if counts_p is not None else {}))
        return res

    def step(self, tile: torch.Tensor, mask: Optional[torch.Tensor] = None) -> Dict[str, torch.Tensor]:
        lr_now = cosine_lr(self.step_idx, self.total_steps, self.lr, self.min_lr)
        for g in self.opt.param_groups:
            g["lr"] = lr_now
        if self.opt_lr_dev_sync():
            pass
        self._set_lambda_vq()
        self.model.train()
        self.opt.zero_grad(set_to_none=True)
        self._images_current()
        if self.pack_cache is not None:
            self.pack_cache.__enter__()
        try:
            return self._step_eager(tile, mask, lr_now)
        finally:
            if self.pack_cache is not None:
                self.pack_cache.__exit__(None, None, None)

    def _step_eager(self, tile, mask, lr_now):
        out = self.model.forward_tiles(tile, mask)
        loss = out["loss"]
        ok = None
        if self.check_finite:
            if self.hip_opt:
                ok = self._finite_flag(out)
                if self.reducer is not None and self.reducer.active:
                    self.reducer.flag_src = 1.0 - ok
            elif not self._all_finite(loss):
                self.skipped += 1
                if self.reducer is not None:
                    self.reducer.reset()
                if hasattr(self.model, "drop_codebook_hooks"):
                    self.model.drop_codebook_hooks()
                self.step_idx += 1
                out["lr"] = lr_now
                return out
        self._backward(loss)
        if self.reducer is not None:
            self.reducer.finish(scatter=not self.hip_opt)
        if self.hip_opt:
            grads = None
            if self.reducer is not None and self.reducer.active:
                fg = self.reducer.flat_grads()
                grads = [fg[id(p)] if p.grad is not None else None for p in self.opt.params]
                if ok is not None:
                    ok = (self.reducer.flag_result() == 0).float()
            out["grad_norm"] = self.opt.step(self.max_norm, grads, ok)
            self._images_refresh()
            if getattr(self.model, "defer_codebook_hooks", False):
                self.model.commit_codebook_hooks(ok)
        else:
            out["grad_norm"] = torch.nn.utils.clip_grad_norm_(self.params, self.max_norm)
            self.opt.step()
            if getattr(self.model, "defer_codebook_hooks", False):
                self.model.commit_codebook_hooks(None)
        mgr = getattr(self.model, "codebook_manager", None)
        if mgr is not None and hasattr(mgr, "after_step"):
            mgr.after_step(self.model.quant, self.opt)
        if self.hip_opt and hasattr(self.model, "_quantizers"):
            for qz in self.model._quantizers():
                if qz._prepared is not None:
                    qz.prepared(qz._prepared[0][2], 1 << 20)
        self.step_idx += 1
        out["lr"] = lr_now
        return out
```

Measured before the change: 112,100.

## Fold VQ codebook prep into pack cache and add lean launch path

Registers the VQ codebook preparation (fragment packing and norms) as a job in the shared pack-cache refresh kernel, so it runs in the batched refresh launch instead of separate prepare launches. Adds a stats-copy output to VQ assign and a scalar-pointer variant of VQ backward, so separate gscale construction and copies can be dropped. Seeds backward with a cached unit gradient to avoid allocating one each step. All of this is gated by a lean mode that depends on a model attribute. The intent is to cut per-step kernel launches and host overhead, at the cost of extra cache bookkeeping and more complex invalidation of the prepared codebook.

Result: faster. 113,900 (median of 6 runs) (+1.6%).

```diff
diff --git a/include/frl_hip.h b/include/frl_hip.h
--- a/include/frl_hip.h
+++ b/include/frl_hip.h
@@ -238,9 +238,16 @@
 int frl_vq_assign_fwd_prepared(const void* z, const float* E, void* prep , int64_t N, int K, int d,
                                int32_t* idx_out, void* zq_out, float* stats_out, int32_t* counts_out, int dtype, void* ws,
                                size_t ws_bytes, frl_stream_t stream);
+int frl_vq_assign_fwd_stats2(const void* z, const float* E, void* prep, int64_t N, int K, int d, int32_t* idx_out, void* zq_out,
+                             float* stats_out, float* stats_copy, int32_t* counts_out, int dtype, void* ws, size_t ws_bytes,
+                             frl_stream_t stream);
+int frl_pack_cache_add_vq(int handle, const float* E, int K, int d, int dtype, void* prep, size_t prep_bytes);
 int frl_vq_bwd(const void* g_out, const void* z, const void* zq , const float* E, const int32_t* idx, const int32_t* counts,
                const float* gscale, float beta, int64_t N, int K, int d, void* g_z_out, float* g_E_out, float* sums_out,
                int dtype, void* ws, size_t ws_bytes, frl_stream_t stream);
+int frl_vq_bwd_scalars(const void* g_out, const void* z, const void* zq , const float* E, const int32_t* idx,
+                       const int32_t* counts, const float* g_commit, const float* g_codebook, float beta, int64_t N, int K, int d,
+                       void* g_z_out, float* g_E_out, float* sums_out, int dtype, void* ws, size_t ws_bytes, frl_stream_t stream);
 int frl_vq_ema_update(const float* sums, const int32_t* counts, int K, int d, float decay, float eps, float* ema_count,
                       float* ema_sum, float* E, const float* ok, frl_stream_t stream);
 int frl_vq_revive_dead_codes(float* E, const int64_t* window_counts, int64_t min_count, const void* z, int64_t N, int K, int d,
diff --git a/vq-vae_amd/csrc/frl_epi.hpp b/vq-vae_amd/csrc/frl_epi.hpp
--- a/vq-vae_amd/csrc/frl_epi.hpp
+++ b/vq-vae_amd/csrc/frl_epi.hpp
@@ -96,11 +96,11 @@
 };
 
 struct CodeEpi {
-  const float* E; const int32_t* counts; const float* gscale; float ce_base; int d, bf; float* gE; float* sums_out;
+  const float* E; const int32_t* counts; const float* g_cb; float ce_base; int d, bf; float* gE; float* sums_out;
   __device__ void operator()(int64_t i, float s) const {
     if (sums_out) sums_out[i] = s;
     if (gE) {
-      const float ce = ce_base * (gscale ? gscale[1] : 1.f);
+      const float ce = ce_base * (g_cb ? g_cb[0] : 1.f);
       const float ev = bf ? (float)(__bf16)E[i] : E[i];
       gE[i] = ce * ((float)counts[i / d] * ev - s);
     }
diff --git a/vq-vae_amd/csrc/frl_pack.hpp b/vq-vae_amd/csrc/frl_pack.hpp
--- a/vq-vae_amd/csrc/frl_pack.hpp
+++ b/vq-vae_amd/csrc/frl_pack.hpp
@@ -3,7 +3,7 @@
 #include <stdint.h>
 #include <stddef.h>
 
-enum { FRL_PACK_PW = 0, FRL_PACK_C3 = 1, FRL_PACK_PW_REP = 2, FRL_PACK_PW_K4 = 3 };
+enum { FRL_PACK_PW = 0, FRL_PACK_C3 = 1, FRL_PACK_PW_REP = 2, FRL_PACK_PW_K4 = 3, FRL_PACK_VQ = 4 };
 
 struct FrlPackJob {
   const float* W;
@@ -29,3 +29,5 @@
 }
 
 void* frl_pack_cached(const FrlPackJob* jobs, int njobs, size_t bytes, bool* hit);
+
+int frl_pack_cache_add_job(int handle, const FrlPackJob& job);
diff --git a/vq-vae_amd/csrc/pack_cache.hip b/vq-vae_amd/csrc/pack_cache.hip
--- a/vq-vae_amd/csrc/pack_cache.hip
+++ b/vq-vae_amd/csrc/pack_cache.hip
@@ -1,12 +1,14 @@
 #include "frl_common.hpp"
 #include "frl_host.hpp"
 #include "frl_pack.hpp"
+#include "vq_prepare.hpp"
 #include <map>
 #include <mutex>
 #include <string.h>
 #include <vector>
 
 #define PK_FRAGS_PER_BLOCK 512
+#define PK_NORMS_PER_BLOCK 256
 
 __device__ __forceinline__ void pk_frag_pw(const FrlPackJob& j, int i) {
   const int lane = i & 63, fs = i >> 6;
@@ -58,16 +60,55 @@
   }
 }
 
+__device__ __forceinline__ void pk_item_vq(const FrlPackJob& j, int i) {
+  const int K = j.Cout, d = j.Cin, npk = j.tap_rev;
+  if (i >= npk) {
+    float* en = reinterpret_cast<float*>(j.dst + j.so);
+    int* ctl = reinterpret_cast<int*>(j.dst);
+    if (j.dtype == FRL_BF16) vq_prepare_norm<bf16>(j.W, K, d, en, j.MB, ctl, i - npk);
+    else vq_prepare_norm<float>(j.W, K, d, en, j.MB, ctl, i - npk);
+    return;
+  }
+  if (j.dtype == FRL_BF16) {
+    bf16x8* pk = reinterpret_cast<bf16x8*>(j.dst + j.si);
+    switch (j.NF) {
+      case 1: vq_prepare_frag<bf16, 1>(j.W, K, d, pk, i); break;
+      case 2: vq_prepare_frag<bf16, 2>(j.W, K, d, pk, i); break;
+      default: vq_prepare_frag<bf16, 4>(j.W, K, d, pk, i); break;
+    }
+  } else {
+    float* pk = reinterpret_cast<float*>(j.dst + j.si);
+    switch (j.NF) {
+      case 4: vq_prepare_frag<float, 4>(j.W, K, d, pk, i); break;
+      case 8: vq_prepare_frag<float, 8>(j.W, K, d, pk, i); break;
+      case 16: vq_prepare_frag<float, 16>(j.W, K, d, pk, i); break;
+      default: vq_prepare_frag<float, 32>(j.W, K, d, pk, i); break;
+    }
+  }
+}
+
 __global__ __launch_bounds__(256) void frl_pack_jobs_kernel(const FrlPackJob* __restrict__ jobs, const int2* __restrict__ blocks) {
   const int2 bk = blocks[blockIdx.x];
   const FrlPackJob j = jobs[bk.x];
-  const int end = (bk.y + PK_FRAGS_PER_BLOCK) < j.nfrag ? (bk.y + PK_FRAGS_PER_BLOCK) : j.nfrag;
+  int span = PK_FRAGS_PER_BLOCK, limit = j.nfrag;
+  if (j.kind == FRL_PACK_VQ) {
+    if (bk.y >= j.tap_rev) span = PK_NORMS_PER_BLOCK; else limit = j.tap_rev;
+  }
+  const int end = (bk.y + span) < limit ? (bk.y + span) : limit;
   for (int i = bk.y + threadIdx.x; i < end; i += 256) {
-    if (j.kind == FRL_PACK_C3) pk_frag_c3(j, i); else pk_frag_pw(j, i);
+    if (j.kind == FRL_PACK_C3) pk_frag_c3(j, i);
+    else if (j.kind == FRL_PACK_VQ) pk_item_vq(j, i);
+    else pk_frag_pw(j, i);
   }
 }
 
 namespace {
+template <typename F>
+void pk_blocks_of(const FrlPackJob& j, F&& put) {
+  const int nf = j.kind == FRL_PACK_VQ ? j.tap_rev : j.nfrag;
+  for (int f = 0; f < nf; f += PK_FRAGS_PER_BLOCK) put(f);
+  for (int f = nf; f < j.nfrag; f += PK_NORMS_PER_BLOCK) put(f);
+}
 struct Key {
   unsigned char bytes[8 * 72];
   size_t n;
@@ -119,6 +160,23 @@
   return img;
 }
 
+int frl_pack_cache_add_job(int handle, const FrlPackJob& job) {
+  std::lock_guard<std::mutex> lk(g_mu);
+  auto it = g_caches.find(handle);
+  if (it == g_caches.end()) return frl_fail(-2, "pack_cache_add_job: unknown handle");
+  Cache& c = it->second;
+  for (const FrlPackJob& j : c.jobs)
+    if (memcmp(&j, &job, sizeof(FrlPackJob)) == 0) return 0;
+  int nblk = 0;
+  pk_blocks_of(job, [&](int) { ++nblk; });
+  if (c.jobs.size() + 1 > PK_MAX_JOBS || c.blocks.size() + nblk > PK_MAX_BLOCKS) return frl_fail(-4, "pack_cache_add_job: job tables full");
+  const int ji = (int)c.jobs.size();
+  c.jobs.push_back(job);
+  pk_blocks_of(job, [&](int f) { c.blocks.push_back(int2{ji, f}); });
+  c.dirty = true;
+  return 0;
+}
+
 extern "C" {
 
 size_t frl_pack_cache_table_bytes(void) { return PK_MAX_JOBS * sizeof(FrlPackJob) + PK_MAX_BLOCKS * sizeof(int2); }
diff --git a/vq-vae_amd/csrc/vq.hip b/vq-vae_amd/csrc/vq.hip
--- a/vq-vae_amd/csrc/vq.hip
+++ b/vq-vae_amd/csrc/vq.hip
@@ -6,6 +6,7 @@
 #include "vq_assign_resident.hpp"
 #include "vq_assign_stream.hpp"
 #include "vq_bwd.hpp"
+#include "frl_pack.hpp"
 #include <stdlib.h>
 
 static int vq_chunk(int K, int d_pad, size_t esize) {
@@ -92,7 +93,7 @@
 }
 template <typename T, int NF>
 static int launch_vq(const void* z, const float* E, char* prep, int64_t N, int K, int d, int32_t* idx, void* zq, float* stats,
-                     int32_t* counts, char* ws, hipStream_t st) {
+                     float* stats_copy, int32_t* counts, char* ws, hipStream_t st) {
   typedef typename DT<T>::frag_t frag_t;
   const VqLayout L = vq_layout(N, K, d);
   const VqPrep P = vq_prep_layout<T, NF>(N, K, d);
@@ -122,7 +123,8 @@
       if (lds > 160 * 1024) return frl_fail(-3, "vq_assign: LDS budget exceeded");
       const auto kern = nt == 4 ? vq_assign_stream_kernel<4> : nt == 2 ? vq_assign_stream_kernel<2> : vq_assign_stream_kernel<1>;
       const int rc = vq_launch_assign(kern, grid_s, 64 * VQS_NW, lds, st, (const bf16*)z, en, N, K, Kc, idx, (bf16*)zq, (float*)(ws + L.partial),
-                                      (const bf16x8*)pk, (VqCtl*)(prep + P.ctl), counts, stats, (unsigned*)(ws + L.amb), (float*)(ws + L.amb_lim));
+                                      (const bf16x8*)pk, (VqCtl*)(prep + P.ctl), counts, stats, (unsigned*)(ws + L.amb), (float*)(ws + L.amb_lim),
+                                      stats_copy);
       return rc ? rc : frl_check_launch("vq_assign");
     }
   }
@@ -141,7 +143,7 @@
       if (nwr == 8) kern = vq_assign_resident_kernel<T, NF, VQ_RES_NT, 8>;
     }
     const int rc = vq_launch_assign(kern, grid_r, 64 * nwr, lds, st, (const T*)z, E, en, N, K, d, Kc, idx, (T*)zq, (float*)(ws + L.partial), pk,
-                                    (VqCtl*)(prep + P.ctl), counts, stats);
+                                    (VqCtl*)(prep + P.ctl), counts, stats, stats_copy);
     return rc ? rc : frl_check_launch("vq_assign");
   }
   const int Kc2 = Kc >= 32 ? Kc / 2 : Kc;
@@ -154,7 +156,7 @@
   FRL_LAUNCH_AS("vq_fixup_tile_kernel", (vq_fixup_tile_kernel<T, NF>), dim3(1024), dim3(64 * VQ_FIXT_WAVES), 0, st, (const T*)z, E, en, pk, K, P.kpad, d,
                 (const int32_t*)(ws + L.amb), (const float*)(ws + L.amb_lim), hdr, idx, (T*)zq, (int32_t*)(ws + L.counts_fix));
   FRL_LAUNCH(vq_finalize_kernel, dim3(1), dim3(256), 0, st, (const float*)(ws + L.partial), L.grid * nw, (const VqHeader*)hdr,
-             (const int32_t*)(ws + L.counts_fix), counts, K, N, d, stats);
+             (const int32_t*)(ws + L.counts_fix), counts, K, N, d, stats, stats_copy);
   return frl_check_launch("vq_assign");
 }
 
@@ -162,6 +164,53 @@
   int kc = K;
   while ((size_t)kc * d * 4 > 96 * 1024 && kc > 1) kc = (kc + 1) / 2;
   return kc;
+}
+
+extern "C" size_t frl_vq_workspace_bytes(int64_t N, int K, int d);
+static int vq_bwd_impl(const void* g_out, const void* z, const void* zq, const float* E, const int32_t* idx, const int32_t* counts,
+                       const float* g_cm, const float* g_cb, float cz_factor, float ce_factor, float beta, int64_t N, int K, int d, void* g_z_out,
+                       float* g_E_out, float* sums_out, int dtype, void* ws, size_t ws_bytes, hipStream_t stream) {
+  if (N <= 0 || K <= 0 || d <= 0) return frl_fail(-2, "vq_bwd: empty input");
+  if (dtype != FRL_F32 && dtype != FRL_BF16) return frl_fail(-2, "vq_bwd: bad dtype");
+  if (dtype == FRL_BF16 && d > 128) return frl_fail(-2, "vq_bwd: d > 128 unsupported in bf16");
+  if (ws_bytes < frl_vq_workspace_bytes(N, K, d)) return frl_fail(-4, "vq_bwd: workspace too small");
+  const int Kc = vq_bwd_chunk(K, d);
+  const size_t lds = (size_t)Kc * d * 4;
+  if (dtype == FRL_F32 && lds > 96 * 1024) return frl_fail(-2, "vq_bwd: one code row exceeds the LDS chunk");
+  const int64_t rows = (N + VQ_BWD_WGS - 1) / VQ_BWD_WGS;
+  const float cz = beta * 2.f / ((float)N * (float)d) * cz_factor, ce = 2.f / ((float)N * (float)d) * ce_factor;
+  float* slab = (float*)ws;
+  if (dtype == FRL_F32) {
+    auto kern = vq_bwd_kernel<float>;
+    if (lds > 64 * 1024) FRL_HIP(hipFuncSetAttribute((const void*)kern, hipFuncAttributeMaxDynamicSharedMemorySize, (int)lds));
+    FRL_LAUNCH_AS("vq_bwd_kernel", kern, dim3(VQ_BWD_WGS), dim3(256), lds, stream, (const float*)g_out, (const float*)z, E, idx, g_cm,
+                       cz, N, K, d, Kc, rows, (float*)g_z_out, slab);
+    launch_slab_reduce_deferrable<float, CodeEpi>((const float*)slab, VQ_BWD_WGS, (int64_t)K * d, CodeEpi{E, counts, g_cb, ce, d, 0, g_E_out, sums_out}, stream, sums_out == nullptr);
+  } else if (dtype == FRL_BF16) {
+    const int64_t rows64 = (rows + 63) / 64 * 64;
+    if (d <= 32) {
+      FRL_LAUNCH((vq_bwd_mfma_kernel<4, 2, 8>), dim3(VQ_BWD_WGS), dim3(512), (size_t)64 * 40 * 2 + 256, stream, (const bf16*)g_out, (const bf16*)z, (const bf16*)zq, E, idx,
+                 g_cm, cz, N, K, d, rows64, (bf16*)g_z_out, slab);
+    } else if (d <= 64) {
+      FRL_LAUNCH((vq_bwd_mfma_kernel<4, 4, 8>), dim3(VQ_BWD_WGS), dim3(512), (size_t)64 * 72 * 2 + 256, stream, (const bf16*)g_out, (const bf16*)z, (const bf16*)zq, E, idx,
+                 g_cm, cz, N, K, d, rows64, (bf16*)g_z_out, slab);
+    } else {
+      FRL_LAUNCH((vq_bwd_mfma_kernel<2, 8, 8>), dim3(VQ_BWD_WGS), dim3(512), (size_t)64 * 136 * 2 + 256, stream, (const bf16*)g_out, (const bf16*)z, (const bf16*)zq, E, idx,
+                 g_cm, cz, N, K, d, rows64, (bf16*)g_z_out, slab);
+    }
+    launch_slab_reduce_deferrable<float, CodeEpi>((const float*)slab, VQ_BWD_WGS, (int64_t)K * d, CodeEpi{E, counts, g_cb, ce, d, 1, g_E_out, sums_out}, stream, sums_out == nullptr);
+  } else return frl_fail(-2, "vq_bwd: bad dtype");
+  return frl_check_launch("vq_bwd");
+}
+
+template <typename T, int NF>
+static int vq_pack_job(int handle, const float* E, int K, int d, int dtype, char* prep) {
+  const VqPrep P = vq_prep_layout<T, NF>(0, K, d);
+  const int kz = P.kpad > 64 ? P.kpad : 64;
+  FrlPackJob j;
+  j.W = E; j.dst = prep; j.so = (long long)P.en; j.si = (long long)P.pack; j.kind = FRL_PACK_VQ; j.dtype = dtype; j.NF = NF;
+  j.Cout = K; j.Cin = d; j.MB = P.kpad; j.tap_rev = P.npk; j.nfrag = P.npk + kz;
+  return frl_pack_cache_add_job(handle, j);
 }
 
 extern "C" {
@@ -204,14 +253,27 @@
 #undef VQ_CALL_PREP
 }
 
-int frl_vq_assign_fwd_prepared(const void* z, const float* E, void* prep, int64_t N, int K, int d, int32_t* idx_out, void* zq_out,
-                               float* stats_out, int32_t* counts_out, int dtype, void* ws, size_t ws_bytes, hipStream_t stream) {
+int frl_pack_cache_add_vq(int handle, const float* E, int K, int d, int dtype, void* prep, size_t prep_bytes) {
+  if (K <= 0 || d <= 0 || d > 128 || E == nullptr) return frl_fail(-2, "pack_cache_add_vq: bad codebook shape");
+  if (prep == nullptr || prep_bytes < frl_vq_prepared_bytes(K, d)) return frl_fail(-4, "pack_cache_add_vq: buffer too small");
+#define VQ_CALL_JOB(T_, NF_) vq_pack_job<T_, NF_>(handle, E, K, d, dtype, (char*)prep)
+  VQ_DISPATCH(dtype, d, VQ_CALL_JOB);
+#undef VQ_CALL_JOB
+}
+
+int frl_vq_assign_fwd_stats2(const void* z, const float* E, void* prep, int64_t N, int K, int d, int32_t* idx_out, void* zq_out,
+                             float* stats_out, float* stats_copy, int32_t* counts_out, int dtype, void* ws, size_t ws_bytes, hipStream_t stream) {
   if (N <= 0 || K <= 0 || d <= 0) return frl_fail(-2, "vq_assign: empty input");
   if (d > 128) return frl_fail(-2, "vq_assign: d > 128 unsupported");
   if (ws_bytes < frl_vq_workspace_bytes(N, K, d)) return frl_fail(-4, "vq_assign: workspace too small");
-#define VQ_CALL_FWD(T_, NF_) launch_vq<T_, NF_>(z, E, (char*)prep, N, K, d, idx_out, zq_out, stats_out, counts_out, (char*)ws, stream)
+#define VQ_CALL_FWD(T_, NF_) launch_vq<T_, NF_>(z, E, (char*)prep, N, K, d, idx_out, zq_out, stats_out, stats_copy, counts_out, (char*)ws, stream)
   VQ_DISPATCH(dtype, d, VQ_CALL_FWD);
 #undef VQ_CALL_FWD
+}
+
+int frl_vq_assign_fwd_prepared(const void* z, const float* E, void* prep, int64_t N, int K, int d, int32_t* idx_out, void* zq_out,
+                               float* stats_out, int32_t* counts_out, int dtype, void* ws, size_t ws_bytes, hipStream_t stream) {
+  return frl_vq_assign_fwd_stats2(z, E, prep, N, K, d, idx_out, zq_out, stats_out, nullptr, counts_out, dtype, ws, ws_bytes, stream);
 }
 
 int frl_vq_assign_fwd(const void* z, const float* E, int64_t N, int K, int d, int32_t* idx_out, void* zq_out,
@@ -222,37 +284,15 @@
 int frl_vq_bwd(const void* g_out, const void* z, const void* zq, const float* E, const int32_t* idx, const int32_t* counts,
                const float* gscale, float beta, int64_t N, int K, int d, void* g_z_out, float* g_E_out,
                float* sums_out, int dtype, void* ws, size_t ws_bytes, hipStream_t stream) {
-  if (N <= 0 || K <= 0 || d <= 0) return frl_fail(-2, "vq_bwd: empty input");
-  if (dtype != FRL_F32 && dtype != FRL_BF16) return frl_fail(-2, "vq_bwd: bad dtype");
-  if (dtype == FRL_BF16 && d > 128) return frl_fail(-2, "vq_bwd: d > 128 unsupported in bf16");
-  if (ws_bytes < frl_vq_workspace_bytes(N, K, d)) return frl_fail(-4, "vq_bwd: workspace too small");
-  const int Kc = vq_bwd_chunk(K, d);
-  const size_t lds = (size_t)Kc * d * 4;
-  if (dtype == FRL_F32 && lds > 96 * 1024) return frl_fail(-2, "vq_bwd: one code row exceeds the LDS chunk");
-  const int64_t rows = (N + VQ_BWD_WGS - 1) / VQ_BWD_WGS;
-  const float cz = beta * 2.f / ((float)N * (float)d), ce = 2.f / ((float)N * (float)d);
-  float* slab = (float*)ws;
-  if (dtype == FRL_F32) {
-    auto kern = vq_bwd_kernel<float>;
-    if (lds > 64 * 1024) FRL_HIP(hipFuncSetAttribute((const void*)kern, hipFuncAttributeMaxDynamicSharedMemorySize, (int)lds));
-    FRL_LAUNCH_AS("vq_bwd_kernel", kern, dim3(VQ_BWD_WGS), dim3(256), lds, stream, (const float*)g_out, (const float*)z, E, idx, gscale,
-                       cz, N, K, d, Kc, rows, (float*)g_z_out, slab);
-    launch_slab_reduce_deferrable<float, CodeEpi>((const float*)slab, VQ_BWD_WGS, (int64_t)K * d, CodeEpi{E, counts, gscale, ce, d, 0, g_E_out, sums_out}, stream, sums_out == nullptr);
-  } else if (dtype == FRL_BF16) {
-    const int64_t rows64 = (rows + 63) / 64 * 64;
-    if (d <= 32) {
-      FRL_LAUNCH((vq_bwd_mfma_kernel<4, 2, 8>), dim3(VQ_BWD_WGS), dim3(512), (size_t)64 * 40 * 2 + 256, stream, (const bf16*)g_out, (const bf16*)z, (const bf16*)zq, E, idx,
-                 gscale, cz, N, K, d, rows64, (bf16*)g_z_out, slab);
-    } else if (d <= 64) {
-      FRL_LAUNCH((vq_bwd_mfma_kernel<4, 4, 8>), dim3(VQ_BWD_WGS), dim3(512), (size_t)64 * 72 * 2 + 256, stream, (const bf16*)g_out, (const bf16*)z, (const bf16*)zq, E, idx,
-                 gscale, cz, N, K, d, rows64, (bf16*)g_z_out, slab);
-    } else {
-      FRL_LAUNCH((vq_bwd_mfma_kernel<2, 8, 8>), dim3(VQ_BWD_WGS), dim3(512), (size_t)64 * 136 * 2 + 256, stream, (const bf16*)g_out, (const bf16*)z, (const bf16*)zq, E, idx,
-                 gscale, cz, N, K, d, rows64, (bf16*)g_z_out, slab);
-    }
-    launch_slab_reduce_deferrable<float, CodeEpi>((const float*)slab, VQ_BWD_WGS, (int64_t)K * d, CodeEpi{E, counts, gscale, ce, d, 1, g_E_out, sums_out}, stream, sums_out == nullptr);
-  } else return frl_fail(-2, "vq_bwd: bad dtype");
-  return frl_check_launch("vq_bwd");
+  return vq_bwd_impl(g_out, z, zq, E, idx, counts, gscale, gscale ? gscale + 1 : nullptr, 1.f, 1.f, beta, N, K, d, g_z_out, g_E_out, sums_out, dtype,
+                     ws, ws_bytes, stream);
+}
+
+int frl_vq_bwd_scalars(const void* g_out, const void* z, const void* zq, const float* E, const int32_t* idx, const int32_t* counts,
+                       const float* g_commit, const float* g_codebook, float beta, int64_t N, int K, int d, void* g_z_out, float* g_E_out,
+                       float* sums_out, int dtype, void* ws, size_t ws_bytes, hipStream_t stream) {
+  return vq_bwd_impl(g_out, z, zq, E, idx, counts, g_commit, g_codebook, g_commit ? 1.f : 0.f, g_codebook ? 1.f : 0.f, beta, N, K, d, g_z_out,
+                     g_E_out, sums_out, dtype, ws, ws_bytes, stream);
 }
 
 int frl_vq_ema_update(const float* sums, const int32_t* counts, int K, int d, float decay, float eps, float* ema_count,
diff --git a/vq-vae_amd/csrc/vq_assign_chunked.hpp b/vq-vae_amd/csrc/vq_assign_chunked.hpp
--- a/vq-vae_amd/csrc/vq_assign_chunked.hpp
+++ b/vq-vae_amd/csrc/vq_assign_chunked.hpp
@@ -256,7 +256,7 @@
 
 __global__ __launch_bounds__(256) void vq_finalize_kernel(const float* __restrict__ partial, int npartial, const VqHeader* __restrict__ hdr,
                                                           const int32_t* __restrict__ counts_acc, int32_t* __restrict__ counts, int K, int64_t N,
-                                                          int d, float* __restrict__ stats) {
+                                                          int d, float* __restrict__ stats, float* __restrict__ stats_copy ) {
   __shared__ double red[256];
   double s = 0.0;
   for (int i = threadIdx.x; i < npartial; i += 256) s += (double)partial[i];
@@ -280,5 +280,8 @@
     stats[1] = (float)exp(-red[0]);
     stats[2] = (float)hdr->namb;
     stats[3] = (float)(sq / ((double)N * (double)d));
+    if (stats_copy) {
+      for (int i = 0; i < 4; ++i) stats_copy[i] = stats[i];
+    }
   }
 }
diff --git a/vq-vae_amd/csrc/vq_assign_resident.hpp b/vq-vae_amd/csrc/vq_assign_resident.hpp
--- a/vq-vae_amd/csrc/vq_assign_resident.hpp
+++ b/vq-vae_amd/csrc/vq_assign_resident.hpp
@@ -7,7 +7,8 @@
 __global__ __launch_bounds__(NW * 64, (NW == 8 ? 4 : 1)) void vq_assign_resident_kernel(
     const T* __restrict__ Z, const float* __restrict__ E, const float* __restrict__ en_g, int64_t N, int K, int d, int Kc,
     int32_t* __restrict__ idx_out, T* __restrict__ zq_out, float* __restrict__ partial ,
-    const typename DT<T>::frag_t* __restrict__ pk, VqCtl* __restrict__ ctl, int32_t* __restrict__ counts_out, float* __restrict__ stats_out) {
+    const typename DT<T>::frag_t* __restrict__ pk, VqCtl* __restrict__ ctl, int32_t* __restrict__ counts_out, float* __restrict__ stats_out,
+    float* __restrict__ stats_copy ) {
   typedef typename DT<T>::frag_t frag_t;
   constexpr int FE = DT<T>::FE;
   constexpr int q = NF * FE;
@@ -376,7 +377,7 @@
   __syncthreads();
   const bool last = misc[17] != 0;
   __syncthreads();
-  if (last) vq_fold_stats<NW>(reinterpret_cast<double*>(smem), tidt, tidt & 63, tidt >> 6, partial, (int)gridDim.x * NW, ctl, K, N, d, counts_out, stats_out);
+  if (last) vq_fold_stats<NW>(reinterpret_cast<double*>(smem), tidt, tidt & 63, tidt >> 6, partial, (int)gridDim.x * NW, ctl, K, N, d, counts_out, stats_out, stats_copy);
 #ifdef VQ_STAMPS
   VQ_ST(6);
   __syncthreads();
diff --git a/vq-vae_amd/csrc/vq_assign_stream.hpp b/vq-vae_amd/csrc/vq_assign_stream.hpp
--- a/vq-vae_amd/csrc/vq_assign_stream.hpp
+++ b/vq-vae_amd/csrc/vq_assign_stream.hpp
@@ -98,7 +98,8 @@
 __global__ __launch_bounds__(VQS_NW * 64, 1) void vq_assign_stream_kernel(
     const bf16* __restrict__ Z, const float* __restrict__ en_g, int64_t N, int K, int Kc, int32_t* __restrict__ idx_out,
     bf16* __restrict__ zq_out, float* __restrict__ partial , const bf16x8* __restrict__ pk, VqCtl* __restrict__ ctl,
-    int32_t* __restrict__ counts_out, float* __restrict__ stats_out, unsigned* __restrict__ ovf_row , float* __restrict__ ovf_lim ) {
+    int32_t* __restrict__ counts_out, float* __restrict__ stats_out, unsigned* __restrict__ ovf_row , float* __restrict__ ovf_lim ,
+    float* __restrict__ stats_copy ) {
   constexpr int NF = 2, q = 16, d = 64, NW = VQS_NW;
   constexpr int BATCH = NW * NT * 16;
   static_assert(NW * VQS_CAP <= VQ_FAST_ROWS, "parked rows of a workgroup");
@@ -422,7 +423,7 @@
   __syncthreads();
   const bool last = misc[17] != 0;
   __syncthreads();
-  if (last) vq_fold_stats<NW>(reinterpret_cast<double*>(smem), tid, lane, wave, partial, (int)gridDim.x * NW, ctl, K, N, d, counts_out, stats_out);
+  if (last) vq_fold_stats<NW>(reinterpret_cast<double*>(smem), tid, lane, wave, partial, (int)gridDim.x * NW, ctl, K, N, d, counts_out, stats_out, stats_copy);
 #ifdef VQ_STAMPS
   VQ_ST(6);
   __syncthreads();
diff --git a/vq-vae_amd/csrc/vq_common.hpp b/vq-vae_amd/csrc/vq_common.hpp
--- a/vq-vae_amd/csrc/vq_common.hpp
+++ b/vq-vae_amd/csrc/vq_common.hpp
@@ -178,7 +178,7 @@
 
 template <int NW>
 __device__ __forceinline__ void vq_fold_stats(double* red, int tid, int lane, int wave, const float* partial, int npartial, VqCtl* ctl, int K, int64_t N, int d,
-                                              int32_t* __restrict__ counts_out, float* __restrict__ stats_out) {
+                                              int32_t* __restrict__ counts_out, float* __restrict__ stats_out, float* __restrict__ stats_copy) {
   int32_t* counts_acc = reinterpret_cast<int32_t*>(ctl + 1);
   double sp = 0.0;
   for (int i = tid; i < npartial; i += NW * 64) sp += (double)__hip_atomic_load(&partial[i], __ATOMIC_RELAXED, __HIP_MEMORY_SCOPE_AGENT);
@@ -196,10 +196,14 @@
   __syncthreads();
   if (tid == 0) {
     for (int w = 1; w < NW; ++w) { red[0] += red[w]; red[NW] += red[NW + w]; }
-    stats_out[0] = (float)red[0];
-    stats_out[1] = (float)exp(-red[NW]);
-    stats_out[2] = (float)__hip_atomic_load(&ctl->namb, __ATOMIC_RELAXED, __HIP_MEMORY_SCOPE_AGENT);
-    stats_out[3] = (float)(red[0] / ((double)N * (double)d));
+    const float st[4] = {(float)red[0], (float)exp(-red[NW]), (float)__hip_atomic_load(&ctl->namb, __ATOMIC_RELAXED, __HIP_MEMORY_SCOPE_AGENT),
+                         (float)(red[0] / ((double)N * (double)d))};
+#pragma unroll
+    for (int i = 0; i < 4; ++i) stats_out[i] = st[i];
+    if (stats_copy) {
+#pragma unroll
+      for (int i = 0; i < 4; ++i) stats_copy[i] = st[i];
+    }
     __hip_atomic_store(&ctl->namb, 0, __ATOMIC_RELAXED, __HIP_MEMORY_SCOPE_AGENT);
     __hip_atomic_store(&ctl->done, 0, __ATOMIC_RELAXED, __HIP_MEMORY_SCOPE_AGENT);
   }
diff --git a/vq-vae_amd/csrc/vq_prepare.hpp b/vq-vae_amd/csrc/vq_prepare.hpp
--- a/vq-vae_amd/csrc/vq_prepare.hpp
+++ b/vq-vae_amd/csrc/vq_prepare.hpp
@@ -1,29 +1,40 @@
 #pragma once
-#include "vq_common.hpp"
+#include "frl_common.hpp"
 
-template <typename T, int NF>
-__global__ void vq_prepare_kernel(const float* __restrict__ E, int K, int d, float* __restrict__ en, int kpad,
-                                  typename DT<T>::frag_t* __restrict__ pk, int total, int npack_blocks, int* __restrict__ ctl) {
-  constexpr int FE = DT<T>::FE;
-  constexpr int q = NF * FE;
-  if ((int)blockIdx.x >= npack_blocks) {
-    const int k = ((int)blockIdx.x - npack_blocks) * blockDim.x + threadIdx.x;
-    if (k >= kpad) return;
-    if (k < 64) ctl[k] = 0;
-    if (k < K) ctl[64 + k] = 0;
-    float s = 3.0e38f;
-    if (k < K) {
-      s = 0.f;
+
+template <typename T>
+__device__ __forceinline__ void vq_prepare_norm(const float* __restrict__ E, int K, int d, float* __restrict__ en, int kpad, int* __restrict__ ctl, int k) {
+  if (k >= kpad) return;
+  if (k < 64) ctl[k] = 0;
+  if (k < K) ctl[64 + k] = 0;
+  float s = 3.0e38f;
+  if (k < K) {
+    s = 0.f;
+    const float* row = E + (int64_t)k * d;
+    if ((d & 3) == 0 && (reinterpret_cast<uintptr_t>(E) & 15) == 0) {
+#pragma unroll 4
+      for (int j = 0; j < d; j += 4) {
+        const f32x4 r = *reinterpret_cast<const f32x4*>(row + j);
+#pragma unroll
+        for (int e = 0; e < 4; ++e) {
+          const float v = to_f32(from_f32<T>(r[e]));
+          s = fmaf(v, v, s);
+        }
+      }
+    } else {
       for (int j = 0; j < d; ++j) {
-        const float v = to_f32(from_f32<T>(E[(int64_t)k * d + j]));
+        const float v = to_f32(from_f32<T>(row[j]));
         s = fmaf(v, v, s);
       }
     }
-    en[k] = s;
-    return;
   }
-  const int i = blockIdx.x * blockDim.x + threadIdx.x;
-  if (i >= total) return;
+  en[k] = s;
+}
+
+template <typename T, int NF>
+__device__ __forceinline__ void vq_prepare_frag(const float* __restrict__ E, int K, int d, typename DT<T>::frag_t* __restrict__ pk, int i) {
+  constexpr int FE = DT<T>::FE;
+  constexpr int q = NF * FE;
   const int ln = i & 63, fs = i >> 6;
   const int s = fs % NF, mb = fs / NF;
   const int code = mb * 16 + (ln & 15), kq = ln >> 4;
@@ -40,3 +51,14 @@
     pk[i] = (code < K && ch < d) ? -2.f * E[(int64_t)code * d + ch] : 0.f;
   }
 }
+
+template <typename T, int NF>
+__global__ void vq_prepare_kernel(const float* __restrict__ E, int K, int d, float* __restrict__ en, int kpad,
+                                  typename DT<T>::frag_t* __restrict__ pk, int total, int npack_blocks, int* __restrict__ ctl) {
+  if ((int)blockIdx.x >= npack_blocks) {
+    vq_prepare_norm<T>(E, K, d, en, kpad, ctl, ((int)blockIdx.x - npack_blocks) * blockDim.x + threadIdx.x);
+    return;
+  }
+  const int i = blockIdx.x * blockDim.x + threadIdx.x;
+  if (i < total) vq_prepare_frag<T, NF>(E, K, d, pk, i);
+}
diff --git a/vq-vae_amd/frl_hip/_lib.py b/vq-vae_amd/frl_hip/_lib.py
--- a/vq-vae_amd/frl_hip/_lib.py
+++ b/vq-vae_amd/frl_hip/_lib.py
@@ -47,7 +47,10 @@
     "frl_vq_prepare": (c_int, [P, L, I, I, I, P, S, P]),
     "frl_vq_stream_tiles": (c_int, [I]),
     "frl_vq_assign_fwd_prepared": (c_int, [P, P, P, L, I, I, P, P, P, P, I, P, S, P]),
+    "frl_vq_assign_fwd_stats2": (c_int, [P, P, P, L, I, I, P, P, P, P, P, I, P, S, P]),
+    "frl_pack_cache_add_vq": (c_int, [I, P, I, I, I, P, S]),
     "frl_vq_bwd": (c_int, [P, P, P, P, P, P, P, F, L, I, I, P, P, P, I, P, S, P]),
+    "frl_vq_bwd_scalars": (c_int, [P, P, P, P, P, P, P, P, F, L, I, I, P, P, P, I, P, S, P]),
     "frl_vq_ema_update": (c_int, [P, P, I, I, F, F, P, P, P, P, P]),
     "frl_vq_revive_dead_codes": (c_int, [P, P, L, P, L, I, I, ctypes.c_uint64, P, P, P, I, P]),
     "frl_groupnorm_fwd": (c_int, [P, P, P, P, P, P, I, I, I, I, F, I, I, P]),
diff --git a/vq-vae_amd/frl_hip/functional.py b/vq-vae_amd/frl_hip/functional.py
--- a/vq-vae_amd/frl_hip/functional.py
+++ b/vq-vae_amd/frl_hip/functional.py
@@ -12,6 +12,10 @@
 
 def _c(t: Optional[torch.Tensor]):
     return None if t is None else (t if t.is_contiguous() else t.contiguous())
+
+
+def _lean() -> bool:
+    return ops.lean_enabled()
 
 
 def _wanted(ctx, first: int, grads):
@@ -112,11 +116,15 @@
         ctx.mults = mults
         ctx.promises = promises
         ctx.mark_non_differentiable(*res[1:])
+        if _lean():
+            ctx.set_materialize_grads(False)
         return res if aux_coefs is not None else res + (None,)
 
     @staticmethod
     @once_differentiable
     def backward(ctx, g, g_ok, g_aux):
+        if g is None:
+            return (None,) * (4 + len(ctx.coefs))
         gg = ops.scalar_fanout(g.reshape(1).float().contiguous(), ctx.coefs, ctx.mults, ctx.promises)
         return (None, None, None, None) + tuple(gg[i] for i in range(len(ctx.coefs)))
 
@@ -364,11 +372,15 @@
         z, gamma, beta = ops.film_fused_fwd(z_type, h, params)
         ctx.save_for_backward(h, z_type, *params)
         ctx.mark_non_differentiable(gamma, beta)
+        if _lean():
+            ctx.set_materialize_grads(False)
         return z, gamma, beta
 
     @staticmethod
     @once_differentiable
     def backward(ctx, dz, _dg, _db):
+        if dz is None:
+            return (None,) * len(ctx.saved_tensors)
         h, z_type, *params = ctx.saved_tensors
         dh, grads = ops.film_fused_bwd(z_type, h, _c(dz), params)
         return (dh if ctx.needs_input_grad[0] else None, None) + _wanted(ctx, 2, grads)
@@ -397,12 +409,13 @@
 
     @staticmethod
     def forward(ctx, z, codebook, prep=None):
-        idx, zq, stats, counts = ops.vq_assign(z, codebook, prep)
-        d = z.shape[-1]
-        n = z.numel() // d
+        if _lean():
+            idx, zq, stats, counts, st = ops.vq_assign(z, codebook, prep, stats_copy=True)
+        else:
+            idx, zq, stats, counts = ops.vq_assign(z, codebook, prep)
+            st = stats.clone()
         ctx.set_materialize_grads(False)
         ctx.save_for_backward(z, codebook, idx, counts, zq)
-        st = stats.clone()
         ctx.mark_non_differentiable(idx, counts, stats)
         return zq, st[3], st.narrow(0, 3, 1).reshape(()), st[1], idx, counts, stats
 
@@ -410,6 +423,14 @@
     @once_differentiable
     def backward(ctx, g_zq, g_cb, g_cm, g_perp, g_idx, g_counts, g_stats):
         z, codebook, idx, counts, zq = ctx.saved_tensors
+
+        def scalar_ok(g):
+            return g is None or (g.dtype == torch.float32 and g.numel() == 1 and g.device == z.device)
+
+        if _lean() and scalar_ok(g_cm) and scalar_ok(g_cb):
+            gz, ge, _ = ops.vq_bwd(_c(g_zq), z, codebook, idx, counts, None, 1.0, want_gz=ctx.needs_input_grad[0],
+                                   want_ge=ctx.needs_input_grad[1], zq=zq, scalars=(g_cm, g_cb))
+            return gz, ge, None
         if g_cm is not None and g_cb is not None:
             gs = torch.stack([g_cm.reshape(()).float(), g_cb.reshape(()).float()])
         else:
diff --git a/vq-vae_amd/frl_hip/models/vqvae.py b/vq-vae_amd/frl_hip/models/vqvae.py
--- a/vq-vae_amd/frl_hip/models/vqvae.py
+++ b/vq-vae_amd/frl_hip/models/vqvae.py
@@ -126,6 +126,7 @@
         self.fused_decoder = True
         self.onepass_decoder = True
         self.chain_xtype = True
+        self.lean_step = True
         self._grad_scale_dev = {}
         self.concurrent_phase = True
         self._side_stream = None
diff --git a/vq-vae_amd/frl_hip/ops.py b/vq-vae_amd/frl_hip/ops.py
--- a/vq-vae_amd/frl_hip/ops.py
+++ b/vq-vae_amd/frl_hip/ops.py
@@ -71,6 +71,24 @@
         if self.handle <= 0:
             check(self.handle, "frl_pack_cache_create")
         self._prev = 0
+        self._quantizers = {}
+
+    def add_quantizer(self, quantizer) -> bool:
+        prep = quantizer._prepared
+        if prep is None or prep[0][2] is None:
+            return False
+        dtype, buf, cb = prep[0][2], prep[1], quantizer.codebook
+        key = (id(quantizer), buf.data_ptr(), cb.data_ptr(), dtype)
+        if key not in self._quantizers:
+            if cb.dtype != torch.float32 or not cb.is_contiguous() or cb.device != self.arena.device:
+                return False
+            if any(k[1] == key[1] for k in self._quantizers):
+                return False
+            k, d = cb.shape
+            check(_lib.load().frl_pack_cache_add_vq(self.handle, _p(cb), k, d, BF16 if dtype == torch.bfloat16 else F32, _p(buf), buf.numel()),
+                  "frl_pack_cache_add_vq")
+            self._quantizers[key] = (quantizer, dtype, buf, cb)
+        return True
 
     def __enter__(self):
         self._prev = _lib.load().frl_pack_cache_activate(self.handle)
@@ -82,6 +100,11 @@
 
     def refresh(self) -> None:
         check(_lib.load().frl_pack_cache_refresh(self.handle, _stream()), "frl_pack_cache_refresh")
+        for qz, dtype, buf, cb in self._quantizers.values():
+            if qz._prepared is None or qz._prepared[1] is not buf:
+                continue
+            same = qz.codebook is cb or qz.codebook.data_ptr() == cb.data_ptr()
+            qz._prepared = ((cb.data_ptr(), qz.codebook._version, dtype) if same else (None, None, dtype), buf)
 
     @property
     def images(self) -> int:
@@ -367,7 +390,7 @@
 
 
 @_timed("vq_assign")
-def vq_assign(z: torch.Tensor, codebook: torch.Tensor, prep: Optional[torch.Tensor] = None):
+def vq_assign(z: torch.Tensor, codebook: torch.Tensor, prep: Optional[torch.Tensor] = None, stats_copy: bool = False):
     k, d = codebook.shape
     _chk_rows(z, d, "vq_assign.z")
     cb = _f32(codebook, "codebook")
@@ -380,6 +403,11 @@
     counts = torch.empty(k, dtype=torch.int32, device=z.device)
     if prep is not None and (prep.dtype != torch.uint8 or prep.device != z.device or prep.numel() < lib.frl_vq_prepared_bytes(k, d)):
         raise ValueError("vq_assign: prep is not a prepared-codebook image for this codebook")
+    if stats_copy:
+        stats2 = torch.empty(4, dtype=torch.float32, device=z.device)
+        check(lib.frl_vq_assign_fwd_stats2(_p(z), _p(cb), _p(prep), n, k, d, _p(idx), _p(zq), _p(stats), _p(stats2), _p(counts), _dt(z), _p(ws),
+                                           ws.numel(), _stream()), "frl_vq_assign_fwd")
+        return idx, zq, stats, counts, stats2
     check(lib.frl_vq_assign_fwd_prepared(_p(z), _p(cb), _p(prep), n, k, d, _p(idx), _p(zq), _p(stats), _p(counts), _dt(z), _p(ws),
                                          ws.numel(), _stream()), "frl_vq_assign_fwd")
     return idx, zq, stats, counts
@@ -388,7 +416,7 @@
 @_timed("vq_bwd")
 def vq_bwd(g_out: Optional[torch.Tensor], z: torch.Tensor, codebook: torch.Tensor, idx: torch.Tensor,
            counts: torch.Tensor, gscale: Optional[torch.Tensor], beta: float, want_gz: bool = True,
-           want_ge: bool = True, want_sums: bool = False, zq: Optional[torch.Tensor] = None):
+           want_ge: bool = True, want_sums: bool = False, zq: Optional[torch.Tensor] = None, scalars=None):
     if codebook.dim() != 2:
         raise ValueError(f"vq_bwd: codebook must be [K, d], got {tuple(codebook.shape)}")
     k, d = codebook.shape
@@ -410,6 +438,12 @@
         raise ValueError("vq_bwd.gscale: expected a contiguous float32 tensor of at least 2 elements on the device of z")
     if codebook.device != z.device:
         raise ValueError("vq_bwd: codebook and z live on different devices")
+    if scalars is not None:
+        if gscale is not None or len(scalars) != 2:
+            raise ValueError("vq_bwd: scalars is a pair (g_commit, g_codebook) and replaces gscale")
+        for s in scalars:
+            if s is not None and (s.dtype != torch.float32 or s.device != z.device or s.numel() != 1):
+                raise ValueError("vq_bwd.scalars: expected float32 scalars on the device of z (or None)")
     lib = _lib.load()
     ws = workspace(lib.frl_vq_workspace_bytes(n, k, d), z.device)
     gz = torch.empty_like(z) if want_gz else None
@@ -417,7 +451,11 @@
     sums = torch.empty(k, d, dtype=torch.float32, device=z.device) if want_sums else None
     cb32 = _f32(codebook, "codebook")
     if _DEFER["on"]:
-        _DEFER["keep"] += [t for t in (counts, gscale, cb32) if t is not None]
+        _DEFER["keep"] += [t for t in (counts, gscale, cb32) + tuple(scalars or ()) if t is not None]
+    if scalars is not None:
+        check(lib.frl_vq_bwd_scalars(_p(g_out), _p(z), _p(zq), _p(cb32), _p(idx), _p(counts), _p(scalars[0]), _p(scalars[1]), float(beta),
+                                     n, k, d, _p(gz), _p(ge), _p(sums), _dt(z), _p(ws), ws.numel(), _stream()), "frl_vq_bwd_scalars")
+        return gz, ge, sums
     check(lib.frl_vq_bwd(_p(g_out), _p(z), _p(zq), _p(cb32), _p(idx), _p(counts), _p(gscale), float(beta),
                          n, k, d, _p(gz), _p(ge), _p(sums), _dt(z), _p(ws), ws.numel(), _stream()), "frl_vq_bwd")
     return gz, ge, sums
@@ -1088,6 +1126,18 @@
                                                   b, h, w, c, rank, coarse_dilation, _dt(x), _stream()),
           "frl_edge_smooth_stencil_bwd")
     return dx, da, db
+
+
+_LEAN = {"on": True}
+
+
+def set_lean(on: bool) -> bool:
+    was, _LEAN["on"] = _LEAN["on"], bool(on)
+    return was
+
+
+def lean_enabled() -> bool:
+    return _LEAN["on"] and fusion_enabled("launches")
 
 
 def fusion_enabled(name: str) -> bool:
diff --git a/vq-vae_amd/frl_hip/training/trainer.py b/vq-vae_amd/frl_hip/training/trainer.py
--- a/vq-vae_amd/frl_hip/training/trainer.py
+++ b/vq-vae_amd/frl_hip/training/trainer.py
@@ -248,15 +248,38 @@
         return (out["loss"].detach().float() * 0.0 == 0.0).float().reshape(1)
 
     def _backward(self, loss):
+        seed = self._unit_gradient(loss)
         if self.defer_reductions and self.hip_opt and not (self.reducer is not None and self.reducer.active):
             from .. import ops
             with ops.deferred_reductions(self.opt.params):
-                loss.backward()
+                loss.backward(seed)
         else:
-            loss.backward()
+            loss.backward(seed)
+
+    def _unit_gradient(self, loss):
+        if not (self._lean() and loss.is_cuda and loss.dim() == 0 and loss.dtype == torch.float32):
+            return None
+        one = self.__dict__.setdefault("_unit_grads", {}).get(loss.device)
+        if one is None:
+            one = self._unit_grads[loss.device] = torch.ones((), dtype=torch.float32, device=loss.device)
+        return one
+
+    def _lean(self) -> bool:
+        on = bool(getattr(self.model, "lean_step", False)) and not (self.reducer is not None and self.reducer.active)
+        if self.hip_opt:
+            from .. import ops
+            ops.set_lean(not (self.reducer is not None and self.reducer.active))
+        return on
+
+    def _refresh_images_and_codebooks(self) -> None:
+        if self.pack_cache is not None and self._lean() and hasattr(self.model, "_quantizers"):
+            for qz in self.model._quantizers():
+                self.pack_cache.add_quantizer(qz)
+        self._images_refresh()
 
     def _step_body(self, tile, mask):
         self.model.train()
+        self._lean()
         self.opt.zero_grad(set_to_none=True)
         dp = self.reducer is not None and self.reducer.active
         if dp:
@@ -282,7 +305,7 @@
             grads = [fg[id(p)] if p.grad is not None else None for p in self.opt.params]
             ok = (self.reducer.flag_result() == 0).float()
         out["grad_norm"] = self.opt.step(self.max_norm, grads, ok)
-        self._images_refresh()
+        self._refresh_images_and_codebooks()
         if getattr(self.model, "defer_codebook_hooks", False):
             self.model.commit_codebook_hooks(ok)
         if hasattr(self.model, "_quantizers"):
@@ -362,6 +385,7 @@
             pass
         self._set_lambda_vq()
         self.model.train()
+        self._lean()
         self.opt.zero_grad(set_to_none=True)
         self._images_current()
         if self.pack_cache is not None:
@@ -401,7 +425,7 @@
                 if ok is not None:
                     ok = (self.reducer.flag_result() == 0).float()
             out["grad_norm"] = self.opt.step(self.max_norm, grads, ok)
-            self._images_refresh()
+            self._refresh_images_and_codebooks()
             if getattr(self.model, "defer_codebook_hooks", False):
                 self.model.commit_codebook_hooks(ok)
         else:
```
